# PJLab-ADG/neuralsim

Measured on AMD Instinct MI355X. Metric: training rays/sec (fwd+bwd) NeuS 800x800, higher is better.
Workload: dtype fp16

## Files before the change

### include/nsim.h

```cpp
#ifndef NSIM_H
#define NSIM_H
#include <stdint.h>

#ifdef __cplusplus
extern "C" {
#endif

#define NSIM_MAX_LEVELS 32
#define NSIM_LOTD_DENSE 0
#define NSIM_LOTD_HASH 1

typedef struct NsimLotdMeta {
  int32_t num_levels;
  int32_t n_feats;
  int32_t n_active_levels;
  int32_t res[NSIM_MAX_LEVELS][3];
  int32_t type[NSIM_MAX_LEVELS];
  uint32_t size[NSIM_MAX_LEVELS];
  int64_t offset[NSIM_MAX_LEVELS];
  float x_scale[3];
  float x_shift[3];
} NsimLotdMeta;

typedef struct NsimOccMeta {
  float aabb_min[3];
  float aabb_max[3];
  float scale[3];
  int32_t res[3];
} NsimOccMeta;

const char* nsim_strerror(int code);
int nsim_version(void);

int nsim_pack_infos_from_n(const int64_t* n, int64_t P, int64_t* pack_infos, int64_t* total, int64_t cap,
                           void* stream);
int nsim_pack_infos_from_n_notify(const int64_t* n, int64_t P, int64_t* pack_infos, int64_t* total, int64_t cap,
                                  int64_t* notify, int64_t seq, void* stream);
int nsim_live_rank(const int64_t* n, int64_t R, int C, int nf0, int nf1, int nf2, int nf3, int64_t* live_rank,
                   int64_t* live_idx, int64_t* cnts, int64_t* notify, int64_t seq, int64_t* pack_infos, int64_t* total,
                   int64_t cap, int64_t* notify_total, int64_t seq_total, void* stream);
int nsim_packed_sum(const float* x, int C, const int64_t* pack_infos, int64_t P, float* out, void* stream);
int nsim_packed_binary(const float* x, int C, const float* per_pack, int Cp, const int64_t* pack_infos,
                       int64_t P, int op, float* out, void* stream);
int nsim_packed_cmp(const float* x, const float* per_pack, const int64_t* pack_infos, int64_t P, int op,
                    uint8_t* out, void* stream);
int nsim_packed_matmul3(const float* x, const float* rot, const int64_t* pack_infos, int64_t P,
                        int transpose, float* out, void* stream);
int nsim_packed_sort(const float* x, const int64_t* pack_infos, int64_t P, float* sorted,
                     int64_t* indices, void* stream);
typedef struct NsimComposeSrc {
  const float* t;
  const int64_t* rays_inds;
  const int64_t* pack_infos;
  int64_t P;
  int64_t* dst;
} NsimComposeSrc;
int nsim_compose_collect_sort(const NsimComposeSrc* src, int32_t K, const int64_t* total_pack_infos, int64_t N,
                              float* t_sorted, void* stream);
int nsim_interleave_linstep(const int64_t* start, const int64_t* pack_infos, int64_t P, int64_t step,
                            int64_t* out, void* stream);
int nsim_merge_two_packs(const float* va, const int64_t* pia, const int64_t* slot_a, int64_t Pa,
                         const float* vb, const int64_t* pib, const int64_t* slot_b, int64_t Pb,
                         const int64_t* pack_infos_out, int64_t U, int64_t* pidx_a, int64_t* pidx_b,
                         void* stream);

int nsim_alpha_to_vw_fwd(const float* alpha, const int64_t* pack_infos, int64_t P, float* vw, float* trans,
                         void* stream);
int nsim_alpha_to_vw_bwd(const float* alpha, const float* trans, const float* vw, const float* dvw,
                         const int64_t* pack_infos, int64_t P, float* dalpha, void* stream);
int nsim_render_head(const float* sdf, const float* ln_inv_s, float ln_inv_s_factor, float forward_inv_s, const float* t,
                     const float* rgb, const float* nablas, const int64_t* pack_infos, int64_t P, int normalized_depth,
                     const float* gt, int64_t N, int64_t S, int64_t M, float w_eikonal, const int64_t* out_idx, float* alpha,
                     float* vw, float* trans, float* mask, float* depth, float* rgb_out, float* nrm_out, float* acc,
                     float* dalpha, float* dsdf, float* drgb, float* dnablas, float* d_ln_inv_s, void* stream);
int nsim_composite_fwd(const float* alpha, const float* t, const float* rgb, const float* nrm,
                       const int64_t* pack_infos, int64_t P, int normalized_depth, float* vw, float* trans,
                       float* mask, float* depth, float* rgb_out, float* nrm_out, const int64_t* out_idx,
                       void* stream);
int nsim_composite_bwd(const float* alpha, const float* trans, const float* vw, const float* t,
                       const float* rgb, const float* nrm, const int64_t* pack_infos, int64_t P,
                       int normalized_depth, const float* mask, const float* depth, const float* dmask,
                       const float* ddepth, const float* drgb_out, const float* dnrm_out,
                       const float* dvw_ext, float* dalpha, float* drgb, float* dnrm, const int64_t* out_idx,
                       void* stream);
int nsim_neus_alpha_fwd(const float* sdf, const int64_t* pack_infos, int64_t P, const float* ln_inv_s,
                        float ln_inv_s_factor, float forward_inv_s, float* alpha, void* stream);
int nsim_neus_alpha_bwd(const float* sdf, const float* dalpha, const int64_t* pack_infos, int64_t P,
                        const float* ln_inv_s, float ln_inv_s_factor, float forward_inv_s, float* dsdf,
                        float* d_ln_inv_s, void* stream);
int nsim_neus_composite_fwd(const float* sdf, const float* ln_inv_s, float ln_inv_s_factor, float forward_inv_s,
                            const float* t, const float* rgb, const float* nrm, const int64_t* pack_infos, int64_t P,
                            int normalized_depth, float* alpha, float* vw, float* trans, float* mask, float* depth,
                            float* rgb_out, float* nrm_out, const int64_t* out_idx, void* stream);

int nsim_raygen_pinhole(const float* xy, const int64_t* fidx, const float* intr ,
                        const float* c2w , const int64_t* WH , int64_t N, int snap,
                        float* rays_o, float* rays_d, void* stream);
int nsim_raygen_pinhole_bwd(const float* xy, const int64_t* fidx, const float* intr, const float* c2w,
                            const int64_t* WH, int64_t N, int snap, const float* d_rays_o, const float* d_rays_d,
                            float* d_c2w, void* stream);
int nsim_raygen_opencv(const float* xy, const int64_t* fidx, const float* intr, const float* distortion ,
                       int n_iters, const float* c2w, const int64_t* WH, int64_t N, int snap, float* rays_o,
                       float* rays_d, void* stream);
int nsim_raygen_opencv_bwd(const float* xy, const int64_t* fidx, const float* intr, const float* distortion, int n_iters,
                           const float* c2w, const int64_t* WH, int64_t N, int snap, const float* d_rays_o,
                           const float* d_rays_d, float* d_c2w, void* stream);
int nsim_raygen_fisheye(const float* xy, const int64_t* fidx, const float* intr, const float* distortion ,
                        int n_iters, const float* c2w, const int64_t* WH, int64_t N, int snap, float* rays_o,
                        float* rays_d, void* stream);
int nsim_raygen_fisheye_bwd(const float* xy, const int64_t* fidx, const float* intr, const float* distortion, int n_iters,
                            const float* c2w, const int64_t* WH, int64_t N, int snap, const float* d_rays_o,
                            const float* d_rays_d, float* d_c2w, void* stream);
int nsim_aabb_ray_test(const float* rays_o, const float* rays_d, int64_t N, const NsimOccMeta* meta,
                       float near, float far, float* near_out, float* far_out, uint8_t* hit, void* stream);

int nsim_occ_decay(float* val, int64_t nvox, float decay, void* stream);
int nsim_occ_update(float* val, const float* pts, const float* sdf, int64_t n, const NsimOccMeta* meta,
                    float inv_s, void* stream);
int nsim_occ_pack_bits(const float* val, int64_t nvox, float thre, uint32_t* bits, void* stream);
int nsim_occ_collect(float* val, const float* pts, const float* sdf, int64_t n, const int64_t* n_dev, int64_t n_add,
                     const NsimOccMeta* meta, float inv_s, void* stream);
int nsim_march_count(const float* rays_o, const float* rays_d, const float* near, const float* far,
                     const float* jitter, int64_t R, const uint32_t* bits, const int64_t* ray_word_off,
                     const NsimOccMeta* meta, float step, int max_steps, int64_t* counts, void* stream);
int nsim_march_emit(const float* rays_o, const float* rays_d, const float* near, const float* far,
                    const float* jitter, int64_t R, const uint32_t* bits, const int64_t* ray_word_off,
                    const NsimOccMeta* meta, float step, int max_steps, const int64_t* pack_infos, float* t_out,
                    void* stream);
int nsim_coarse_depths(const float* near, const float* far, const float* jitter_c, int64_t R, int C,
                       float* out, const int64_t* live_rank, void* stream);
int nsim_upsample_stage(const float* t, const float* sdf, const int64_t* pack_infos, int64_t R, float inv_s,
                        int n_fine, int use_estimate_alpha, float* scratch, float* t_new, const float* rays_o,
                        const float* rays_d, float* x_new, const int64_t* live_rank, void* stream);
int nsim_merge_sorted(const float* t_a, const float* v_a, const int64_t* pack_infos_a, const float* t_b,
                      const float* v_b, int64_t R, int nb, float* t_out, float* v_out,
                      int64_t* pack_infos_out, int64_t* ridx_out, const float* rays_o, const float* rays_d,
                      float* x_out, const int64_t* live_rank, void* stream);
int nsim_merge_upsample(const float* t_a, const float* v_a, const int64_t* pack_infos_a, const float* t_b, const float* v_b,
                        int64_t R, int nb, float* t_out, float* v_out, int64_t* pack_infos_out, int64_t* ridx_out, float inv_s,
                        int n_fine, int use_estimate_alpha, float* scratch, float* t_new, const float* rays_o,
                        const float* rays_d, float* x_new, const int64_t* live_rank, void* stream);

int nsim_compress_count(const float* sdf, const int64_t* pack_infos, int64_t R, const float* ln_inv_s,
                        float ln_inv_s_factor, float forward_inv_s, float thre, int64_t* counts, void* stream);
int nsim_compress_emit(const float* sdf, const float* t, const int64_t* pack_infos, int64_t R, const float* ln_inv_s,
                       float ln_inv_s_factor, float forward_inv_s, float thre, const int64_t* pack_infos_out,
                       float* t_out, int64_t* ridx_out, int64_t tail_n, void* stream);

int nsim_lotd_fwd(const float* x, const void* grid_f16, const NsimLotdMeta* meta, int64_t S, float* out,
                  float* dydx, void* stream);
int nsim_lotd_bwd(const float* x, const float* dL_dout, const float* dL_ddydx, const NsimLotdMeta* meta,
                  int64_t S, float* dgrid, void* stream);

typedef struct NsimPermutoMeta {
  int32_t in_dim;
  int32_t num_levels;
  int32_t n_feats;
  uint32_t hashmap_size;
  float scale[NSIM_MAX_LEVELS][8];
  float shift[NSIM_MAX_LEVELS][8];
} NsimPermutoMeta;
int nsim_permuto_fwd(const NsimPermutoMeta* meta, const void* grid_f16, const float* x, int64_t S, float* out, float* dydx,
                     void* stream);
int nsim_permuto_bwd(const NsimPermutoMeta* meta, const float* x, int64_t S, const float* dL_dout, float* dgrid,
                     void* stream);
int nsim_permuto_gather(const NsimPermutoMeta* meta, const void* grid_f16, const float* x, const float* rays_o,
                        const float* rays_d, const float* t, const int64_t* ridx, const float* z, int64_t S,
                        const int64_t* n_dev, int64_t n_add, void* feat_planes, int feat_f32, float* h_planes,
                        void* J_planes, void* stream);
int nsim_permuto_scatter(const NsimPermutoMeta* meta, const float* x, const float* rays_o, const float* rays_d,
                         const float* t, const int64_t* ridx, const float* z, int64_t S, const float* dh_planes,
                         const float* g_planes, const float* gn, float* dgrid, void* stream);
int nsim_permuto_dz(const NsimPermutoMeta* meta, const void* grid_f16, const float* x, const float* rays_o,
                    const float* rays_d, const float* t, const int64_t* ridx, const float* z, int64_t S,
                    const float* dh_planes, float* dz, void* stream);

typedef struct NsimFieldMeta {
  NsimLotdMeta lotd;
  int32_t sdf_D;
  int32_t precision;
  float softplus_beta;
  int32_t embed_E;
} NsimFieldMeta;

int64_t nsim_field_wpack_bytes(const NsimFieldMeta* meta);
int nsim_field_pack_weights(const NsimFieldMeta* meta, const float* sdf_w, const float* sdf_b,
                            const float* rad_w, const float* rad_b, void* wpack, void* stream);
int nsim_field_pack_weights2(const NsimFieldMeta* meta_a, void* wpack_a, const NsimFieldMeta* meta_b, void* wpack_b,
                             const float* sdf_w, const float* sdf_b, const float* rad_w, const float* rad_b, void* stream);
int nsim_field_sdf(const NsimFieldMeta* meta, const void* grid_f16, const void* wpack, const float* x,
                   const float* rays_o, const float* rays_d, const float* t, const int64_t* ridx,
                   const int64_t* ray_goff, int64_t S, const int64_t* n_dev, int64_t n_add, float* sdf,
                   const void* feat_planes, float* occ_val, const NsimOccMeta* occ_meta, float occ_inv_s, void* stream);
int nsim_lotd_gather_lm(const NsimFieldMeta* meta, const void* grid_f16, const float* x, const float* rays_o,
                        const float* rays_d, const float* t, const int64_t* ridx, const int64_t* ray_goff, int64_t S,
                        const int64_t* n_dev, int64_t n_add, void* feat_planes, void* stream);
#define NSIM_PLANE_PITCH(S) ((((int64_t)(S)) + 31) & ~(int64_t)31)
int nsim_field_fwd(const NsimFieldMeta* meta, const void* grid_f16, const void* wpack, const float* x,
                   const float* rays_o, const float* rays_d, const float* t, const int64_t* ridx,
                   const int64_t* ray_goff, const float* h_appear, int64_t S, float* sdf, float* nablas, float* rgb,
                   float* h_planes, void* J_planes, const int64_t* n_dev, int64_t n_add, void* stream);
int nsim_jplane_elem_bytes(const NsimFieldMeta* meta);
int nsim_set_grad_scratch(float* buf, int64_t floats, void* stream);
int nsim_field_bwd_rad(const NsimFieldMeta* meta, const void* wpack, const float* nablas_fwd, const float* rgb_fwd,
                       const float* x, const float* rays_o, const float* rays_d, const float* t, const int64_t* ridx,
                       const float* h_appear, int64_t S, const float* dnablas, const float* drgb, float* gn_out,
                       float* drad_w, float* drad_b, float* dh_appear, float* dx, float* dv, void* stream);
int nsim_field_bwd_sdf(const NsimFieldMeta* meta, const void* wpack, const float* h_planes, const void* J_planes,
                       int64_t S, const float* dsdf, const float* gn, float* dh_planes, float* g_planes,
                       float* dsdf_w, float* dsdf_b, float* dx, int64_t plane_pitch, void* stream);
int nsim_wide_sdf(const NsimFieldMeta* meta, int32_t n_freq, const float* sdf_w, const float* sdf_b, const float* x,
                  const float* rays_o, const float* rays_d, const float* t, const int64_t* ridx, int64_t S,
                  const int64_t* n_dev, int64_t n_add, const float* feat_planes, float* sdf, void* stream);
int nsim_wide_bwd_sdf(const NsimFieldMeta* meta, const void* wpack, const float* x, const float* rays_o,
                      const float* rays_d, const float* t, const int64_t* ridx, int64_t S, const float* h_planes,
                      const void* J_planes, int64_t plane_pitch, const float* dsdf, const float* gn, float* dh_planes,
                      float* g_planes, float* dsdf_w, float* dsdf_b, void* stream);
int nsim_lotd_scatter(const NsimLotdMeta* meta, const float* x, const float* rays_o, const float* rays_d,
                      const float* t, const int64_t* ridx, const int64_t* ray_goff, int64_t S,
                      const float* dh_planes, const float* g_planes, const float* gn, float* dgrid, int level_begin,
                      int level_count, void* stream);
int nsim_lotd_hess_dx(const NsimLotdMeta* meta, const void* grid_f16, const float* x, const float* rays_o,
                      const float* rays_d, const float* t, const int64_t* ridx, const int64_t* ray_goff, int64_t S,
                      const float* g_planes, const float* gn, float* dx, void* stream);
int nsim_ray_grad_reduce(const float* dx, const float* dv, const float* t, const int64_t* ridx, int64_t S,
                         float* d_rays_o, float* d_rays_d, void* stream);

typedef struct NsimLotd4Meta {
  int32_t num_levels;
  int32_t res_xyz[16];
  int32_t res_w[16];
  int32_t type[16];
  uint32_t size[16];
  int64_t offset[16];
  int32_t res_y[16];
  int32_t res_z[16];
} NsimLotd4Meta;

typedef struct NsimDistantMeta {
  NsimLotd4Meta lotd;
  int32_t precision;
} NsimDistantMeta;

int64_t nsim_distant_wpack_bytes(const NsimDistantMeta* meta);
int nsim_distant_pack_weights(const NsimDistantMeta* meta, const float* den_w, const float* den_b, const float* rad_w,
                              const float* rad_b, void* wpack, void* stream);
int nsim_distant_shells(const float* rays_o, const float* rays_d, const float* near, const float* jitter, int64_t N,
                        int K, const float* aabb, float r_min, float r_max, float* t, float* u4, uint8_t* valid,
                        void* stream);
int nsim_density_alpha_fwd(const float* sigma, const float* t, const uint8_t* valid, int64_t N, int K,
                           int include_inf_distance, float* alpha, void* stream);
int nsim_density_alpha_bwd(const float* sigma, const float* t, const uint8_t* valid, const float* dalpha, int64_t N,
                           int K, int include_inf_distance, float* dsigma, void* stream);
int nsim_distant_fwd(const NsimDistantMeta* meta, const void* grid_f16, const void* wpack, const float* u4,
                     const float* rays_d, const float* h_appear, int64_t S, int K, float* sigma, float* rgb,
                     float* h_planes, void* stream);
int nsim_distant_bwd(const NsimDistantMeta* meta, const void* wpack, const float* h_planes, const float* sigma_fwd,
                     const float* rgb_fwd, const float* rays_d, const float* h_appear, const uint8_t* valid,
                     int64_t S, int K, const float* dsigma, const float* drgb, float* dh_planes, float* dden_w,
                     float* dden_b, float* drad_w, float* drad_b, float* dh_appear, void* stream);
int nsim_lotd4_scatter(const NsimLotd4Meta* meta, const float* u4, const uint8_t* valid, int64_t S,
                       const float* dh_planes, float* dgrid, void* stream);

typedef struct NsimSkyMeta {
  int32_t n_frequencies;
  int32_t n_appear;
  int32_t precision;
} NsimSkyMeta;

int64_t nsim_sky_wpack_bytes(const NsimSkyMeta* meta);
int64_t nsim_sky_plane_pitch(int64_t N);
int nsim_sky_pack_weights(const NsimSkyMeta* meta, const float* w, const float* b, void* wpack, void* stream);
int nsim_sky_fwd(const NsimSkyMeta* meta, const void* wpack, const float* v, const float* h_appear, int64_t N,
                 float* rgb, float* planes_fwd, void* stream);
int nsim_sky_bwd(const NsimSkyMeta* meta, const void* wpack, const float* rgb_fwd, const float* drgb, int64_t N,
                 const float* planes_fwd, float* planes_bwd, float* dw, float* db, float* dh_appear, void* stream);

int nsim_eikonal_loss_fwd(const float* nablas, int64_t S, float* out, void* stream);
int nsim_eikonal_loss_bwd(const float* nablas, int64_t S, const float* gout, float* dnablas, void* stream);
int nsim_mse_loss_fwd(const float* pred, const float* gt, int64_t n, float* out, void* stream);
int nsim_mse_loss_bwd(const float* pred, const float* gt, int64_t n, const float* gout, float* dpred, void* stream);
int nsim_rows_scatter_add(const float* g, const int64_t* idx, int64_t n, int C, int64_t rows, float* out, void* stream);
int nsim_rows_gather(const float* table, const int64_t* idx, int64_t n, int C, int64_t rows, int64_t tail, float* out,
                     void* stream);
int nsim_train_loss_head(const float* pred, const float* gt, int64_t n_img, const float* nablas, int64_t S, int64_t M,
                         float w_eikonal, float* acc, float* d_pred, float* d_nablas, void* stream);
int nsim_gather_rays(const float* rays_o, const float* rays_d, const float* near, const float* far, const int64_t* idx,
                     int64_t R, float* o_out, float* d_out, float* near_out, float* far_out, void* stream);
int nsim_sphere_image(const float* rays_o, const float* rays_d, int64_t N, float radius, float* rgb, void* stream);

int nsim_adam_step(float* p, void* p16, float* grad, float* m, float* v, int64_t n, float lr, float beta1,
                   float beta2, float eps, float bias1, float bias2, float grad_scale, int zero_grad,
                   void* stream);

#define NSIM_ADAM_MULTI_MAX 12
typedef struct {
  float* p;
  void* p16;
  float* grad;
  float* m;
  float* v;
  int64_t n;
  float beta1, beta2, bias1, bias2, lr_scale;
} NsimAdamTensor;
int nsim_adam_multi(const NsimAdamTensor* tensors, int n_tensors, float lr, float eps, float grad_scale, int zero_grad,
                    void* stream);

int nsim_mc_count(const float* lat, int64_t nx, int64_t ny, int64_t nzs, float level, int32_t* cnt_v, int32_t* cnt_t,
                  void* stream);
int nsim_mc_scan(int32_t* cnt_v, int32_t* cnt_t, int64_t nx, int64_t ny, int64_t nzs, int32_t* totals, void* stream);
int nsim_mc_emit_verts(const float* lat, const float* below, const float* above, int64_t nx, int64_t ny, int64_t nzs,
                       float level, float bx, float by, float bz, float h, int64_t k0, int64_t vbase, int emit_top,
                       const int32_t* off_v, int32_t* vid, float* verts, float* normals, void* stream);
int nsim_mc_emit_tris(const float* lat, int64_t nx, int64_t ny, int64_t nzs, float level, const int32_t* off_t,
                      const int32_t* vid, int32_t* faces, void* stream);

int nsim_nn_brute(const float* x, int64_t N, const float* y, int64_t M, const int32_t* qlist, const int32_t* nq, int64_t nsplit,
                  float* part_d2, int32_t* part_idx, float* d2, int32_t* idx, void* stream);
int nsim_nn_grid_count(const float* y, int64_t M, float target_occ, int64_t max_cells, int32_t* hdr, int32_t* cell_cnt,
                       int32_t* cell_of, int32_t* rank, void* stream);
int nsim_nn_grid_scan(const int32_t* hdr, int32_t* cell_cnt, void* stream);
int nsim_nn_grid_fill(const float* y, int64_t M, const int32_t* cell_off, const int32_t* cell_of, const int32_t* rank, float* rec,
                      void* stream);
int nsim_nn_grid_query(const float* x, int64_t N, const float* rec, const int32_t* cell_off, int32_t* hdr, int max_rings, float* d2,
                       int32_t* idx, int32_t* left_list, void* stream);

int nsim_selftest_mfma(const float* a, const float* b, float* d, int use_f32, void* stream);

#ifdef __cplusplus
}
#endif
#endif
```

### neuralsim_amd/_lib.py

```python
import ctypes as C
import os
from pathlib import Path

import torch

NSIM_MAX_LEVELS = 32
_HERE = Path(__file__).resolve().parent
LIB_PATH = _HERE / "csrc" / "libnsim_hip.so"


class LotdMeta(C.Structure):
    _fields_ = [("num_levels", C.c_int32), ("n_feats", C.c_int32), ("n_active_levels", C.c_int32),
                ("res", (C.c_int32 * 3) * NSIM_MAX_LEVELS),
                ("type", C.c_int32 * NSIM_MAX_LEVELS), ("size", C.c_uint32 * NSIM_MAX_LEVELS),
                ("offset", C.c_int64 * NSIM_MAX_LEVELS), ("x_scale", C.c_float * 3), ("x_shift", C.c_float * 3)]


class OccMeta(C.Structure):
    _fields_ = [("aabb_min", C.c_float * 3), ("aabb_max", C.c_float * 3), ("scale", C.c_float * 3),
                ("res", C.c_int32 * 3)]


class Lotd4Meta(C.Structure):
    _fields_ = [("num_levels", C.c_int32), ("res_xyz", C.c_int32 * 16), ("res_w", C.c_int32 * 16),
                ("type", C.c_int32 * 16), ("size", C.c_uint32 * 16), ("offset", C.c_int64 * 16),
                ("res_y", C.c_int32 * 16), ("res_z", C.c_int32 * 16)]


class PermutoMeta(C.Structure):
    _fields_ = [("in_dim", C.c_int32), ("num_levels", C.c_int32), ("n_feats", C.c_int32), ("hashmap_size", C.c_uint32),
                ("scale", (C.c_float * 8) * NSIM_MAX_LEVELS), ("shift", (C.c_float * 8) * NSIM_MAX_LEVELS)]


class DistantMeta(C.Structure):
    _fields_ = [("lotd", Lotd4Meta), ("precision", C.c_int32)]


class SkyMeta(C.Structure):
    _fields_ = [("n_frequencies", C.c_int32), ("n_appear", C.c_int32), ("precision", C.c_int32)]


class AdamTensor(C.Structure):
    _fields_ = [("p", C.c_void_p), ("p16", C.c_void_p), ("grad", C.c_void_p), ("m", C.c_void_p), ("v", C.c_void_p),
                ("n", C.c_int64), ("beta1", C.c_float), ("beta2", C.c_float), ("bias1", C.c_float), ("bias2", C.c_float),
                ("lr_scale", C.c_float)]


ADAM_MULTI_MAX = 12


def plane_pitch(S: int) -> int:
    return (int(S) + 31) & ~31


def jplane_dtype(fm):
    import torch
    return torch.float16 if int(get_lib().nsim_jplane_elem_bytes(fm)) == 2 else torch.float32


class FieldMeta(C.Structure):
    _fields_ = [("lotd", LotdMeta), ("sdf_D", C.c_int32), ("precision", C.c_int32), ("softplus_beta", C.c_float),
                ("embed_E", C.c_int32)]


class ComposeSrc(C.Structure):
    _fields_ = [("t", C.c_void_p), ("rays_inds", C.c_void_p), ("pack_infos", C.c_void_p), ("P", C.c_int64), ("dst", C.c_void_p)]


_P = C.c_void_p
_I64 = C.c_int64
_I = C.c_int
_F = C.c_float

SIGNATURES = {
    "nsim_pack_infos_from_n": [_P, _I64, _P, _P, _I64],
    "nsim_pack_infos_from_n_notify": [_P, _I64, _P, _P, _I64, _P, _I64],
    "nsim_live_rank": [_P, _I64, _I, _I, _I, _I, _I, _P, _P, _P, _P, _I64, _P, _P, _I64, _P, _I64],
    "nsim_packed_sum": [_P, _I, _P, _I64, _P],
    "nsim_packed_binary": [_P, _I, _P, _I, _P, _I64, _I, _P],
    "nsim_packed_cmp": [_P, _P, _P, _I64, _I, _P],
    "nsim_packed_matmul3": [_P, _P, _P, _I64, _I, _P],
    "nsim_packed_sort": [_P, _P, _I64, _P, _P],
    "nsim_interleave_linstep": [_P, _P, _I64, _I64, _P],
    "nsim_merge_two_packs": [_P, _P, _P, _I64, _P, _P, _P, _I64, _P, _I64, _P, _P],
    "nsim_alpha_to_vw_fwd": [_P, _P, _I64, _P, _P],
    "nsim_alpha_to_vw_bwd": [_P, _P, _P, _P, _P, _I64, _P],
    "nsim_composite_fwd": [_P, _P, _P, _P, _P, _I64, _I, _P, _P, _P, _P, _P, _P, _P],
    "nsim_neus_composite_fwd": [_P, _P, _F, _F, _P, _P, _P, _P, _I64, _I, _P, _P, _P, _P, _P, _P, _P, _P],
    "nsim_render_head": [_P, _P, _F, _F, _P, _P, _P, _P, _I64, _I, _P, _I64, _I64, _I64, _F, _P] + [_P] * 13,
    "nsim_composite_bwd": [_P, _P, _P, _P, _P, _P, _P, _I64, _I, _P, _P, _P, _P, _P, _P, _P, _P, _P, _P, _P],
    "nsim_neus_alpha_fwd": [_P, _P, _I64, _P, _F, _F, _P],
    "nsim_neus_alpha_bwd": [_P, _P, _P, _I64, _P, _F, _F, _P, _P],
    "nsim_raygen_pinhole": [_P, _P, _P, _P, _P, _I64, _I, _P, _P],
    "nsim_raygen_pinhole_bwd": [_P, _P, _P, _P, _P, _I64, _I, _P, _P, _P],
    "nsim_raygen_opencv": [_P, _P, _P, _P, _I, _P, _P, _I64, _I, _P, _P],
    "nsim_raygen_opencv_bwd": [_P, _P, _P, _P, _I, _P, _P, _I64, _I, _P, _P, _P],
    "nsim_raygen_fisheye": [_P, _P, _P, _P, _I, _P, _P, _I64, _I, _P, _P],
    "nsim_raygen_fisheye_bwd": [_P, _P, _P, _P, _I, _P, _P, _I64, _I, _P, _P, _P],
    "nsim_aabb_ray_test": [_P, _P, _I64, C.POINTER(OccMeta), _F, _F, _P, _P, _P],
    "nsim_occ_decay": [_P, _I64, _F],
    "nsim_occ_update": [_P, _P, _P, _I64, C.POINTER(OccMeta), _F],
    "nsim_occ_pack_bits": [_P, _I64, _F, _P],
    "nsim_occ_collect": [_P, _P, _P, _I64, _P, _I64, C.POINTER(OccMeta), _F],
    "nsim_march_count": [_P, _P, _P, _P, _P, _I64, _P, _P, C.POINTER(OccMeta), _F, _I, _P],
    "nsim_march_emit": [_P, _P, _P, _P, _P, _I64, _P, _P, C.POINTER(OccMeta), _F, _I, _P, _P],
    "nsim_coarse_depths": [_P, _P, _P, _I64, _I, _P, _P],
    "nsim_upsample_stage": [_P, _P, _P, _I64, _F, _I, _I, _P, _P, _P, _P, _P, _P],
    "nsim_merge_sorted": [_P, _P, _P, _P, _P, _I64, _I, _P, _P, _P, _P, _P, _P, _P, _P],
    "nsim_merge_upsample": [_P, _P, _P, _P, _P, _I64, _I, _P, _P, _P, _P, _F, _I, _I, _P, _P, _P, _P, _P, _P],
    "nsim_compress_count": [_P, _P, _I64, _P, _F, _F, _F, _P],
    "nsim_compress_emit": [_P, _P, _P, _I64, _P, _F, _F, _F, _P, _P, _P, _I64],
    "nsim_lotd_fwd": [_P, _P, C.POINTER(LotdMeta), _I64, _P, _P],
    "nsim_lotd_bwd": [_P, _P, _P, C.POINTER(LotdMeta), _I64, _P],
    "nsim_field_pack_weights": [C.POINTER(FieldMeta), _P, _P, _P, _P, _P],
    "nsim_field_sdf": [C.POINTER(FieldMeta), _P, _P, _P, _P, _P, _P, _P, _P, _I64, _P, _I64, _P, _P, _P, C.POINTER(OccMeta), _F],
    "nsim_lotd_gather_lm": [C.POINTER(FieldMeta), _P, _P, _P, _P, _P, _P, _P, _I64, _P, _I64, _P],
    "nsim_field_fwd": [C.POINTER(FieldMeta), _P, _P, _P, _P, _P, _P, _P, _P, _P, _I64, _P, _P, _P, _P, _P, _P, _I64],
    "nsim_compose_collect_sort": [_P, _I, _P, _I64, _P],
    "nsim_wide_sdf": [C.POINTER(FieldMeta), _I, _P, _P, _P, _P, _P, _P, _P, _I64, _P, _I64, _P, _P],
    "nsim_wide_bwd_sdf": [C.POINTER(FieldMeta), _P, _P, _P, _P, _P, _P, _I64, _P, _P, _I64, _P, _P, _P, _P, _P, _P],
    "nsim_set_grad_scratch": [_P, _I64],
    "nsim_permuto_fwd": [C.POINTER(PermutoMeta), _P, _P, _I64, _P, _P],
    "nsim_permuto_bwd": [C.POINTER(PermutoMeta), _P, _I64, _P, _P],
    "nsim_permuto_gather": [C.POINTER(PermutoMeta), _P, _P, _P, _P, _P, _P, _P, _I64, _P, _I64, _P, _I, _P, _P],
    "nsim_permuto_scatter": [C.POINTER(PermutoMeta), _P, _P, _P, _P, _P, _P, _I64, _P, _P, _P, _P],
    "nsim_permuto_dz": [C.POINTER(PermutoMeta), _P, _P, _P, _P, _P, _P, _P, _I64, _P, _P],
    "nsim_field_bwd_rad": [C.POINTER(FieldMeta), _P, _P, _P, _P, _P, _P, _P, _P, _P, _I64, _P, _P, _P, _P, _P, _P, _P, _P],
    "nsim_field_bwd_sdf": [C.POINTER(FieldMeta), _P, _P, _P, _I64, _P, _P, _P, _P, _P, _P, _P, _I64],
    "nsim_lotd_hess_dx": [C.POINTER(LotdMeta), _P, _P, _P, _P, _P, _P, _P, _I64, _P, _P, _P],
    "nsim_ray_grad_reduce": [_P, _P, _P, _P, _I64, _P, _P],
    "nsim_lotd_scatter": [C.POINTER(LotdMeta), _P, _P, _P, _P, _P, _P, _I64, _P, _P, _P, _P, _I, _I],
    "nsim_distant_pack_weights": [C.POINTER(DistantMeta), _P, _P, _P, _P, _P],
    "nsim_distant_shells": [_P, _P, _P, _P, _I64, _I, C.POINTER(C.c_float * 6), _F, _F, _P, _P, _P],
    "nsim_density_alpha_fwd": [_P, _P, _P, _I64, _I, _I, _P],
    "nsim_density_alpha_bwd": [_P, _P, _P, _P, _I64, _I, _I, _P],
    "nsim_distant_fwd": [C.POINTER(DistantMeta), _P, _P, _P, _P, _P, _I64, _I, _P, _P, _P],
    "nsim_distant_bwd": [C.POINTER(DistantMeta), _P, _P, _P, _P, _P, _P, _P, _I64, _I, _P, _P, _P, _P, _P, _P, _P, _P],
    "nsim_lotd4_scatter": [C.POINTER(Lotd4Meta), _P, _P, _I64, _P, _P],
    "nsim_sky_pack_weights": [C.POINTER(SkyMeta), _P, _P, _P],
    "nsim_sky_fwd": [C.POINTER(SkyMeta), _P, _P, _P, _I64, _P, _P],
    "nsim_sky_bwd": [C.POINTER(SkyMeta), _P, _P, _P, _I64, _P, _P, _P, _P, _P],
    "nsim_eikonal_loss_fwd": [_P, _I64, _P],
    "nsim_eikonal_loss_bwd": [_P, _I64, _P, _P],
    "nsim_mse_loss_fwd": [_P, _P, _I64, _P],
    "nsim_train_loss_head": [_P, _P, _I64, _P, _I64, _I64, _F, _P, _P, _P],
    "nsim_mse_loss_bwd": [_P, _P, _I64, _P, _P],
    "nsim_rows_scatter_add": [_P, _P, _I64, _I, _I64, _P],
    "nsim_rows_gather": [_P, _P, _I64, _I, _I64, _I64, _P],
    "nsim_field_pack_weights2": [C.POINTER(FieldMeta), _P, C.POINTER(FieldMeta), _P, _P, _P, _P, _P],
    "nsim_gather_rays": [_P, _P, _P, _P, _P, _I64, _P, _P, _P, _P],
    "nsim_sphere_image": [_P, _P, _I64, _F, _P],
    "nsim_adam_step": [_P, _P, _P, _P, _P, _I64, _F, _F, _F, _F, _F, _F, _F, _I],
    "nsim_adam_multi": [C.POINTER(AdamTensor), _I, _F, _F, _F, _I],
    "nsim_selftest_mfma": [_P, _P, _P, _I],
    "nsim_mc_count": [_P, _I64, _I64, _I64, _F, _P, _P],
    "nsim_mc_scan": [_P, _P, _I64, _I64, _I64, _P],
    "nsim_mc_emit_verts": [_P, _P, _P, _I64, _I64, _I64, _F, _F, _F, _F, _F, _I64, _I64, _I, _P, _P, _P, _P],
    "nsim_mc_emit_tris": [_P, _I64, _I64, _I64, _F, _P, _P, _P],
    "nsim_nn_brute": [_P, _I64, _P, _I64, _P, _P, _I64, _P, _P, _P, _P],
    "nsim_nn_grid_count": [_P, _I64, _F, _I64, _P, _P, _P, _P],
    "nsim_nn_grid_scan": [_P, _P],
    "nsim_nn_grid_fill": [_P, _I64, _P, _P, _P, _P],
    "nsim_nn_grid_query": [_P, _I64, _P, _P, _P, _I, _P, _P, _P],
}
NOSTREAM = {
    "nsim_strerror": ([_I], C.c_char_p),
    "nsim_version": ([], _I),
    "nsim_field_wpack_bytes": ([C.POINTER(FieldMeta)], _I64),
    "nsim_jplane_elem_bytes": ([C.POINTER(FieldMeta)], _I),
    "nsim_distant_wpack_bytes": ([C.POINTER(DistantMeta)], _I64),
    "nsim_sky_wpack_bytes": ([C.POINTER(SkyMeta)], _I64),
    "nsim_sky_plane_pitch": ([_I64], _I64),
}


def bind(cdll):
    for name, args in SIGNATURES.items():
        fn = getattr(cdll, name)
        fn.argtypes = list(args) + [_P]
        fn.restype = _I
    for name, (args, res) in NOSTREAM.items():
        fn = getattr(cdll, name)
        fn.argtypes = list(args)
        fn.restype = res
    return cdll


_LIB = None


def get_lib():
    global _LIB
    if _LIB is None:
        if not LIB_PATH.exists():
            raise RuntimeError(
                f"neuralsim_amd: {LIB_PATH} is missing. This package has no CPU fallback -- build the HIP "
                f"extension with `python -m neuralsim_amd.csrc.build` (needs hipcc, --offload-arch=gfx950).")
        _LIB = bind(C.CDLL(str(LIB_PATH)))
    return _LIB


def stream_handle() -> int:
    return torch._C._cuda_getCurrentRawStream(torch._C._cuda_getDevice())


def require_device(t: torch.Tensor, name: str = "tensor"):
    if not t.is_cuda:
        raise RuntimeError(f"neuralsim_amd: {name} must live on a HIP device (got {t.device}); there is no CPU path")


def ptr(t, dtype=None, name="tensor"):
    if t is not None and dtype is not None and t.dtype != dtype:
        raise TypeError(f"neuralsim_amd: {name} must be {dtype}, got {t.dtype}")
    return t


class HostNotify:

    def __init__(self, slots: int = 2):
        buf = torch.zeros([slots, 2], dtype=torch.long)
        self.buf = buf.pin_memory() if torch.cuda.is_available() else buf
        self.view = self.buf.numpy()
        self.seq = 0

    def __deepcopy__(self, memo):
        return HostNotify(self.buf.shape[0])

    def __reduce__(self):
        return (HostNotify, (self.buf.shape[0],))

    def arm(self, slot: int):
        self.seq += 1
        return self.buf.data_ptr() + 16 * slot, self.seq

    def wait(self, slot: int, seq: int, timeout_s: float = 10.0):
        v = self.view
        n = 0
        t0 = None
        while int(v[slot, 1]) != seq:
            n += 1
            if n & 1023 == 0:
                import time
                now = time.perf_counter()
                t0 = now if t0 is None else t0
                if now - t0 > timeout_s:
                    return None
        return int(v[slot, 0])


class KernelTimer:

    def __init__(self, only=None):
        self.events = {}
        self.units = {}
        self.only = set(only) if only is not None else None

    def note_units(self, name, n):
        self.units[name] = self.units.get(name, 0) + int(n)

    def summary(self):
        torch.cuda.synchronize()
        out = {}
        for name, evs in self.events.items():
            ms = [a.elapsed_time(b) for a, b in evs]
            out[name] = dict(calls=len(ms), total_ms=sum(ms), avg_ms=sum(ms) / max(1, len(ms)),
                             units=self.units.get(name, 0))
        return out


TIMER = None


_Tensor = torch.Tensor


def _marshal(args):
    out = []
    ap = out.append
    for a in args:
        if isinstance(a, _Tensor):
            if not a.is_cuda:
                require_device(a)
            if not a.is_contiguous():
                raise ValueError("neuralsim_amd: tensor arguments must be contiguous")
            ap(a.data_ptr())
        else:
            ap(a)
    return out


_GRAD_SCRATCH = {}
_GRAD_SCRATCH_USERS = ("nsim_field_bwd_rad", "nsim_field_bwd_sdf")
GRAD_SCRATCH_FLOATS = 16 * 8448


def ensure_grad_scratch(device):
    key = (str(device), stream_handle())
    if key not in _GRAD_SCRATCH:
        buf = torch.zeros([GRAD_SCRATCH_FLOATS], dtype=torch.float32, device=device)
        _GRAD_SCRATCH[key] = buf
        call("nsim_set_grad_scratch", buf, buf.numel())
    return _GRAD_SCRATCH[key]


CALL_COUNT = None
class _Arena:
    __slots__ = ("buf", "off", "cap", "demand", "device", "stream")


_ARENA = None
_ARENA_DEMAND = {}


def arena_begin(device):
    global _ARENA
    if os.environ.get("NSIM_ZERO_ARENA", "0") != "1":
        _ARENA = None
        return
    a = _Arena()
    a.device, a.off, a.demand = device, 0, 0
    want = _ARENA_DEMAND.get(str(device), 0)
    a.cap = (int(want * 1.125) + 1024) if want else 0
    a.buf = torch.zeros([a.cap], dtype=torch.float32, device=device) if a.cap else None
    a.stream = stream_handle() if device.type == "cuda" else 0
    _ARENA = a


def arena_end():
    global _ARENA
    a = _ARENA
    if a is not None:
        _ARENA_DEMAND[str(a.device)] = a.demand
    _ARENA = None


def zeros(shape, dtype=torch.float32, device=None):
    a = _ARENA
    if a is None or dtype != torch.float32 or device != a.device:
        return torch.zeros(shape, dtype=dtype, device=device)
    n = 1
    for d_ in shape:
        n *= int(d_)
    pad = (n + 3) & ~3
    a.demand += pad
    if a.off + pad > a.cap or (a.device.type == "cuda" and stream_handle() != a.stream):
        return torch.zeros(shape, dtype=dtype, device=device)
    v = a.buf[a.off:a.off + n].view(shape)
    a.off += pad
    return v


HOST_WAIT = None


def call(name: str, *args):
    global CALL_COUNT
    if CALL_COUNT is not None:
        CALL_COUNT += 1
    lib = get_lib()
    if name in _GRAD_SCRATCH_USERS:
        for a_ in args:
            if isinstance(a_, _Tensor):
                ensure_grad_scratch(a_.device)
                break
    cargs = _marshal(args)
    if TIMER is not None and (TIMER.only is None or name in TIMER.only):
        e0, e1 = torch.cuda.Event(enable_timing=True), torch.cuda.Event(enable_timing=True)
        e0.record()
        rc = getattr(lib, name)(*cargs, stream_handle())
        e1.record()
        TIMER.events.setdefault(name, []).append((e0, e1))
    else:
        rc = getattr(lib, name)(*cargs, stream_handle())
    if rc != 0:
        msg = lib.nsim_strerror(rc)
        raise RuntimeError(f"{name} failed with code {rc}: {msg.decode() if msg else '?'}")
```

### neuralsim_amd/csrc/build.py

```python
import hashlib
import os
import subprocess
import sys
from pathlib import Path

HERE = Path(__file__).resolve().parent
SOURCES = ["pack_ops.hip", "sampling.hip", "lotd.hip", "field.hip", "wide_field.hip", "permuto.hip", "nerf_field.hip", "sky.hip", "loss_ops.hip", "optim.hip", "misc.hip"]
HEADERS = ["nsim_common.h", "nsim_prims.h", "lotd_dev.h", "mfma_mlp.h", "occ_dev.h", "../../include/nsim.h"]
LIB = HERE / "libnsim_hip.so"
BUILD = HERE / "_build"

HIPCC_FLAGS = ["--offload-arch=gfx950", "-O3", "-std=c++17", "-fPIC", "-ffp-contract=off", f"-I{HERE}",
               "-munsafe-fp-atomics", "-Wno-unused-result"] + os.environ.get("NSIM_EXTRA_HIPCC_FLAGS", "").split()


def _hipcc():
    for c in (os.environ.get("HIPCC"), "/opt/rocm/bin/hipcc", "hipcc"):
        if c and (os.path.isabs(c) and os.path.exists(c) or not os.path.isabs(c)):
            return c
    raise RuntimeError("hipcc not found")


def _digest():
    h = hashlib.sha256()
    for f in SOURCES + HEADERS:
        h.update((HERE / f).read_bytes())
    h.update(" ".join(HIPCC_FLAGS).encode())
    return h.hexdigest()


def build(force: bool = False, verbose: bool = True) -> Path:
    BUILD.mkdir(exist_ok=True)
    stamp = BUILD / "stamp"
    dig = _digest()
    if not force and LIB.exists() and stamp.exists() and stamp.read_text() == dig:
        return LIB
    hipcc = _hipcc()
    procs = []
    objs = []
    for src in SOURCES:
        obj = BUILD / (src + ".o")
        objs.append(str(obj))
        cmd = [hipcc, *HIPCC_FLAGS, "-c", str(HERE / src), "-o", str(obj)]
        if verbose:
            print("[nsim build]", " ".join(cmd), flush=True)
        procs.append((src, subprocess.Popen(cmd, stdout=subprocess.PIPE, stderr=subprocess.STDOUT, text=True)))
    failed = False
    for src, p in procs:
        out, _ = p.communicate()
        if p.returncode != 0:
            failed = True
            sys.stderr.write(f"[nsim build] FAILED {src}\n{out}\n")
        elif verbose and out.strip():
            print(out)
    if failed:
        raise RuntimeError("hipcc failed")
    cmd = [hipcc, "--offload-arch=gfx950", "-shared", "-fPIC", *objs, "-o", str(LIB)]
    if verbose:
        print("[nsim build]", " ".join(cmd), flush=True)
    subprocess.check_call(cmd)
    stamp.write_text(dig)
    return LIB


if __name__ == "__main__":
    build(force="--force" in sys.argv)
    print(LIB)
```

### neuralsim_amd/csrc/pack_ops.hip

```cpp
#include "nsim_common.h"

#define PACK_WAVES_PER_BLOCK 4
#define PACK_BLOCK (64 * PACK_WAVES_PER_BLOCK)

__device__ __forceinline__ int64_t pack_wave_id() {
  return (int64_t)blockIdx.x * PACK_WAVES_PER_BLOCK + (threadIdx.x >> 6);
}
static inline dim3 pack_grid(int64_t P) { return dim3(nsim_blocks(P, PACK_WAVES_PER_BLOCK)); }

#define PI_THREADS 1024
#define PI_PER 8
__global__ void __launch_bounds__(PI_THREADS) k_pack_infos_from_n(const int64_t* __restrict__ n, int64_t P,
                                                                    int64_t* __restrict__ pi,
                                                                    int64_t* __restrict__ total, int64_t cap,
                                                                    int64_t* notify, int64_t seq) {
  __shared__ int64_t wtot[PI_THREADS / 64];
  const int tid = threadIdx.x, lane = nsim_lane(), wave = tid >> 6;
  int64_t carry = 0;
  for (int64_t base = 0; base < P; base += (int64_t)PI_THREADS * PI_PER) {
    const int64_t i0 = base + (int64_t)tid * PI_PER;
    int64_t v[PI_PER];
    int64_t mine = 0;
#pragma unroll
    for (int k = 0; k < PI_PER; ++k) {
      v[k] = (i0 + k) < P ? n[i0 + k] : 0;
      mine += v[k];
    }
    const int64_t incl = wave_incl_sum(mine);
    if (lane == 63) wtot[wave] = incl;
    __syncthreads();
    int64_t before = 0, chunk = 0;
#pragma unroll
    for (int w = 0; w < PI_THREADS / 64; ++w) {
      const int64_t x = wtot[w];
      before += (w < wave) ? x : 0;
      chunk += x;
    }
    int64_t run = carry + before + incl - mine;
#pragma unroll
    for (int k = 0; k < PI_PER; ++k) {
      const int64_t i = i0 + k;
      if (i < P) {
        const bool over = cap >= 0 && run + v[k] > cap;
        pi[2 * i] = (cap >= 0 && run > cap) ? cap : run;
        pi[2 * i + 1] = over ? 0 : v[k];
      }
      run += v[k];
    }
    carry += chunk;
    __syncthreads();
  }
  if (tid == 0 && total) total[0] = carry;
  if (tid == 0 && notify) {
    nsim_store_system(notify, carry, false);
    nsim_store_system(notify + 1, seq, true);
  }
}

struct LiveArgs {
  int C;
  int nf[4];
};
__global__ void __launch_bounds__(PI_THREADS) k_live_rank(const int64_t* __restrict__ n, int64_t R, LiveArgs la,
                                                           int64_t* __restrict__ live_rank, int64_t* __restrict__ live_idx,
                                                           int64_t* __restrict__ cnts, int64_t* notify, int64_t seq,
                                                           int64_t* __restrict__ pi, int64_t* __restrict__ total, int64_t cap,
                                                           int64_t* notify_total, int64_t seq_total) {
  __shared__ int64_t wtot[PI_THREADS / 64];
  __shared__ int wlive[PI_THREADS / 64];
  const int tid = threadIdx.x, lane = nsim_lane(), wave = tid >> 6;
  int64_t carry = 0, carry_live = 0;
  for (int64_t base = 0; base < R; base += (int64_t)PI_THREADS * PI_PER) {
    const int64_t i0 = base + (int64_t)tid * PI_PER;
    int64_t v[PI_PER];
    int64_t mine = 0;
    int mine_live = 0;
#pragma unroll
    for (int k = 0; k < PI_PER; ++k) {
      v[k] = (i0 + k) < R ? n[i0 + k] : 0;
      mine += v[k];
      mine_live += v[k] > 0 ? 1 : 0;
    }
    const int64_t incl = wave_incl_sum(mine);
    const int incl_live = wave_incl_sum(mine_live);
    if (lane == 63) {
      wtot[wave] = incl;
      wlive[wave] = incl_live;
    }
    __syncthreads();
    int64_t before = 0, chunk = 0;
    int before_live = 0, chunk_live = 0;
#pragma unroll
    for (int w = 0; w < PI_THREADS / 64; ++w) {
      const int64_t x = wtot[w];
      const int y = wlive[w];
      before += (w < wave) ? x : 0;
      chunk += x;
      before_live += (w < wave) ? y : 0;
      chunk_live += y;
    }
    int64_t run = carry + before + incl - mine;
    int64_t q = carry_live + before_live + incl_live - mine_live;
#pragma unroll
    for (int k = 0; k < PI_PER; ++k) {
      const int64_t i = i0 + k;
      if (i < R) {
        const bool live = v[k] > 0;
        live_rank[i] = live ? q : ~q;
        if (live && live_idx) live_idx[q] = i;
        if (pi) {
          const bool over = cap >= 0 && run + v[k] > cap;
          pi[2 * i] = (cap >= 0 && run > cap) ? cap : run;
          pi[2 * i + 1] = over ? 0 : v[k];
        }
        q += live ? 1 : 0;
      }
      run += v[k];
    }
    carry += chunk;
    carry_live += chunk_live;
    __syncthreads();
  }
  const int64_t Rl = carry_live, M = carry;
  if (live_idx)
    for (int64_t i = Rl + tid; i < R; i += PI_THREADS) live_idx[i] = 0;
  if (tid == 0) {
    cnts[0] = Rl;
    cnts[1] = M + Rl * la.C;
#pragma unroll
    for (int k = 0; k < 4; ++k) cnts[2 + k] = Rl * la.nf[k];
    cnts[6] = M;
    cnts[7] = 0;
    if (total) total[0] = M;
    if (notify) {
      nsim_store_system(notify, Rl, false);
      nsim_store_system(notify + 1, seq, true);
    }
    if (notify_total) {
      nsim_store_system(notify_total, M, false);
      nsim_store_system(notify_total + 1, seq_total, true);
    }
  }
}

__global__ void __launch_bounds__(PACK_BLOCK) k_packed_sum(const float* __restrict__ x, int C,
                                                             const int64_t* __restrict__ pi, int64_t P,
                                                             float* __restrict__ out) {
  const int64_t p = pack_wave_id();
  if (p >= P) return;
  const int lane = nsim_lane();
  const int64_t st = pi[2 * p], n = pi[2 * p + 1];
  for (int c = 0; c < C; ++c) {
    float acc = 0.f;
    for (int64_t i = lane; i < n; i += 64) acc += x[(st + i) * C + c];
    acc = wave_sum(acc);
    if (lane == 0) out[p * C + c] = acc;
  }
}

__global__ void __launch_bounds__(PACK_BLOCK) k_packed_binary(const float* __restrict__ x, int C,
                                                                const float* __restrict__ pp, int Cp,
                                                                const int64_t* __restrict__ pi, int64_t P,
                                                                int op, float* __restrict__ out) {
  const int64_t p = pack_wave_id();
  if (p >= P) return;
  const int lane = nsim_lane();
  const int64_t st = pi[2 * p], n = pi[2 * p + 1];
  const int64_t tot = n * C;
  for (int64_t j = lane; j < tot; j += 64) {
    const int c = (int)(j % C);
    const float b = pp[p * Cp + (Cp == 1 ? 0 : c)];
    const float a = x ? x[st * C + j] : 1.0f;
    float r;
    if (op == 0) r = a * b;
    else if (op == 1) r = a / b;
    else if (op == 2) r = a + b;
    else r = a - b;
    out[st * C + j] = r;
  }
}

__global__ void __launch_bounds__(PACK_BLOCK) k_packed_cmp(const float* __restrict__ x,
                                                             const float* __restrict__ pp,
                                                             const int64_t* __restrict__ pi, int64_t P, int op,
                                                             uint8_t* __restrict__ out) {
  const int64_t p = pack_wave_id();
  if (p >= P) return;
  const int lane = nsim_lane();
  const int64_t st = pi[2 * p], n = pi[2 * p + 1];
  const float b = pp[p];
  for (int64_t i = lane; i < n; i += 64) {
    const float a = x[st + i];
    bool r = (op == 0) ? (a >= b) : (op == 1) ? (a <= b) : (op == 2) ? (a < b) : (a > b);
    out[st + i] = r ? 1 : 0;
  }
}

__global__ void __launch_bounds__(PACK_BLOCK) k_packed_matmul3(const float* __restrict__ x,
                                                                 const float* __restrict__ rot,
                                                                 const int64_t* __restrict__ pi, int64_t P,
                                                                 int transpose, float* __restrict__ out) {
  const int64_t p = pack_wave_id();
  if (p >= P) return;
  const int lane = nsim_lane();
  const int64_t st = pi[2 * p], n = pi[2 * p + 1];
  float r[9];
  for (int k = 0; k < 9; ++k) r[k] = rot[p * 9 + k];
  for (int64_t i = lane; i < n; i += 64) {
    const float a = x[(st + i) * 3 + 0], b = x[(st + i) * 3 + 1], c = x[(st + i) * 3 + 2];
    float o0, o1, o2;
    if (!transpose) {
      o0 = r[0] * a + r[1] * b + r[2] * c;
      o1 = r[3] * a + r[4] * b + r[5] * c;
      o2 = r[6] * a + r[7] * b + r[8] * c;
    } else {
      o0 = r[0] * a + r[3] * b + r[6] * c;
      o1 = r[1] * a + r[4] * b + r[7] * c;
      o2 = r[2] * a + r[5] * b + r[8] * c;
    }
    out[(st + i) * 3 + 0] = o0;
    out[(st + i) * 3 + 1] = o1;
    out[(st + i) * 3 + 2] = o2;
  }
}

__global__ void __launch_bounds__(PACK_BLOCK) k_interleave_linstep(const int64_t* __restrict__ start,
                                                                     const int64_t* __restrict__ pi,
                                                                     int64_t P, int64_t step,
                                                                     int64_t* __restrict__ out) {
  const int64_t p = pack_wave_id();
  if (p >= P) return;
  const int lane = nsim_lane();
  const int64_t st = pi[2 * p], n = pi[2 * p + 1], s0 = start[p];
  for (int64_t i = lane; i < n; i += 64) out[st + i] = s0 + i * step;
}

#define PSORT_CAP 1024
#define PSORT_RUNS 16
__device__ __forceinline__ int lds_upper_bound(const float* a, int n, float v) {
  int lo = 0, hi = n;
  while (lo < hi) {
    const int mid = (lo + hi) >> 1;
    if (a[mid] <= v) lo = mid + 1; else hi = mid;
  }
  return lo;
}
__device__ __forceinline__ int lds_lower_bound(const float* a, int n, float v) {
  int lo = 0, hi = n;
  while (lo < hi) {
    const int mid = (lo + hi) >> 1;
    if (a[mid] < v) lo = mid + 1; else hi = mid;
  }
  return lo;
}
template <class Emit>
__device__ __forceinline__ void psort_staged(const float* sx, int* srun, int nn, int lane, Emit emit) {
  int nrun = 0;
  for (int i0 = 0; i0 < nn; i0 += 64) {
    const int i = i0 + lane;
    const bool head = i < nn && (i == 0 || sx[i] < sx[i - 1]);
    const unsigned long long m = wave_ballot(head);
    if (head) {
      const int pos = nrun + __popcll(m & ((1ull << lane) - 1ull));
      if (pos < PSORT_RUNS) srun[pos] = i;
    }
    nrun += __popcll(m);
  }
  if (nrun <= 1) {
    for (int i = lane; i < nn; i += 64) emit(i, i, sx[i]);
    return;
  }
  if (nrun <= PSORT_RUNS) {
    if (lane == 0) srun[nrun] = nn;
    wave_sync_lds();
    for (int i = lane; i < nn; i += 64) {
      const float xi = sx[i];
      int rank = 0;
      for (int r = 0; r < nrun; ++r) {
        const int b = srun[r], e = srun[r + 1];
        if (e <= i) rank += lds_upper_bound(&sx[b], e - b, xi);
        else if (b > i) rank += lds_lower_bound(&sx[b], e - b, xi);
        else rank += i - b;
      }
      emit(i, rank, xi);
    }
    return;
  }
  for (int i0 = 0; i0 < nn; i0 += 256) {
    float xi[4];
    int ii[4], rank[4];
#pragma unroll
    for (int k = 0; k < 4; ++k) {
      ii[k] = i0 + lane + 64 * k;
      xi[k] = ii[k] < nn ? sx[ii[k]] : 0.f;
      rank[k] = 0;
    }
    for (int j = 0; j < nn; ++j) {
      const float xj = sx[j];
#pragma unroll
      for (int k = 0; k < 4; ++k) rank[k] += (xj < xi[k] || (xj == xi[k] && j < ii[k])) ? 1 : 0;
    }
#pragma unroll
    for (int k = 0; k < 4; ++k)
      if (ii[k] < nn) emit(ii[k], rank[k], xi[k]);
  }
}

__global__ void __launch_bounds__(PACK_BLOCK) k_packed_sort(const float* __restrict__ x,
                                                              const int64_t* __restrict__ pi, int64_t P,
                                                              float* __restrict__ sorted,
                                                              int64_t* __restrict__ indices) {
  __shared__ float sx[PACK_WAVES_PER_BLOCK][PSORT_CAP];
  __shared__ int srun[PACK_WAVES_PER_BLOCK][PSORT_RUNS + 1];
  const int64_t p = pack_wave_id();
  if (p >= P) return;
  const int lane = nsim_lane();
  const int w = (int)(threadIdx.x >> 6);
  const int64_t st = pi[2 * p], n = pi[2 * p + 1];
  if (n <= PSORT_CAP) {
    for (int64_t i = lane; i < n; i += 64) sx[w][i] = x[st + i];
    wave_sync_lds();
    psort_staged(sx[w], srun[w], (int)n, lane, [&](int i, int rank, float xi) {
      sorted[st + rank] = xi;
      indices[st + rank] = st + i;
    });
    return;
  }
  for (int64_t i = lane; i < n; i += 64) {
    const float xi = x[st + i];
    int64_t rank = 0;
    for (int64_t j = 0; j < n; ++j) {
      const float xj = x[st + j];
      rank += (xj < xi || (xj == xi && j < i)) ? 1 : 0;
    }
    sorted[st + rank] = xi;
    indices[st + rank] = st + i;
  }
}

#define COMPOSE_MAX_SRC 64
struct ComposeSrcDev {
  const float* t;
  const int64_t *ric, *pi;
  int64_t P;
  int64_t* dst;
};
struct ComposeArgs {
  int K;
  ComposeSrcDev src[COMPOSE_MAX_SRC];
  const int64_t* total_pi;
  int64_t N;
  float* t_sorted;
};

__global__ void __launch_bounds__(PACK_BLOCK) k_compose_collect_sort(ComposeArgs a) {
  __shared__ float sx[PACK_WAVES_PER_BLOCK][PSORT_CAP];
  __shared__ int srun[PACK_WAVES_PER_BLOCK][PSORT_RUNS + 1];
  __shared__ int s_off[PACK_WAVES_PER_BLOCK][COMPOSE_MAX_SRC + 1];
  __shared__ int64_t s_stg[PACK_WAVES_PER_BLOCK][COMPOSE_MAX_SRC];
  const int64_t r = pack_wave_id();
  if (r >= a.N) return;
  const int lane = nsim_lane();
  const int w = (int)(threadIdx.x >> 6);
  const int64_t st = a.total_pi[2 * r], n = a.total_pi[2 * r + 1];
  if (n <= 0) return;
  int64_t my_st = 0;
  int my_n = 0;
  if (lane < a.K) {
    const ComposeSrcDev& sk = a.src[lane];
    int64_t lo = 0, hi = sk.P;
    while (lo < hi) {
      const int64_t mid = (lo + hi) >> 1;
      if (sk.ric[mid] < r) lo = mid + 1; else hi = mid;
    }
    if (lo < sk.P && sk.ric[lo] == r) {
      my_st = sk.pi[2 * lo];
      my_n = (int)sk.pi[2 * lo + 1];
    }
  }
  const int incl = wave_incl_sum(my_n);
  s_off[w][lane] = incl - my_n;
  if (lane == 63) s_off[w][64] = incl;
  s_stg[w][lane] = my_st;
  wave_sync_lds();
  const int K = a.K;
  auto source_of = [&](int j) -> int {
    int lo = 0, hi = K - 1;
    while (lo < hi) {
      const int mid = (lo + hi + 1) >> 1;
      if (s_off[w][mid] <= j) lo = mid; else hi = mid - 1;
    }
    return lo;
  };
  if (n <= PSORT_CAP) {
    for (int k = 0; k < K; ++k) {
      const int ok = s_off[w][k], nk = s_off[w][k + 1] - ok;
      const float* tk = a.src[k].t + s_stg[w][k];
      for (int i = lane; i < nk; i += 64) sx[w][ok + i] = tk[i];
    }
    wave_sync_lds();
    psort_staged(sx[w], srun[w], (int)n, lane, [&](int i, int rank, float xi) {
      a.t_sorted[st + rank] = xi;
      const int k = source_of(i);
      a.src[k].dst[s_stg[w][k] + (i - s_off[w][k])] = st + rank;
    });
    return;
  }
  for (int64_t i = lane; i < n; i += 64) {
    const int ki = source_of((int)i);
    const float xi = a.src[ki].t[s_stg[w][ki] + (i - s_off[w][ki])];
    int64_t rank = 0;
    for (int k = 0; k < K; ++k) {
      const int ok = s_off[w][k], nk = s_off[w][k + 1] - ok;
      const float* tk = a.src[k].t + s_stg[w][k];
      for (int jj = 0; jj < nk; ++jj) {
        const float xj = tk[jj];
        const int64_t j = ok + jj;
        rank += (xj < xi || (xj == xi && j < i)) ? 1 : 0;
      }
    }
    a.t_sorted[st + rank] = xi;
    a.src[ki].dst[s_stg[w][ki] + (i - s_off[w][ki])] = st + rank;
  }
}

__device__ __forceinline__ int64_t seg_lower_bound(const float* a, int64_t n, float v) {
  int64_t lo = 0, hi = n;
  while (lo < hi) {
    const int64_t mid = (lo + hi) >> 1;
    if (a[mid] < v) lo = mid + 1; else hi = mid;
  }
  return lo;
}
__device__ __forceinline__ int64_t seg_upper_bound(const float* a, int64_t n, float v) {
  int64_t lo = 0, hi = n;
  while (lo < hi) {
    const int64_t mid = (lo + hi) >> 1;
    if (a[mid] <= v) lo = mid + 1; else hi = mid;
  }
  return lo;
}

__global__ void __launch_bounds__(PACK_BLOCK) k_merge_two_packs(
    const float* __restrict__ vs, const int64_t* __restrict__ pis, const int64_t* __restrict__ slot_s,
    int64_t Ps, const float* __restrict__ vo, const int64_t* __restrict__ pio,
// ... 711 lines not shown
```

### neuralsim_amd/csrc/sampling.hip

```cpp
#include "nsim_common.h"
#include "occ_dev.h"

#define SMP_WAVES_PER_BLOCK 4
#define SMP_BLOCK (64 * SMP_WAVES_PER_BLOCK)
#define SMP_LDS_FLOATS 512

__device__ __forceinline__ int64_t smp_wave_id() {
  return (int64_t)blockIdx.x * SMP_WAVES_PER_BLOCK + (threadIdx.x >> 6);
}
static inline dim3 smp_grid(int64_t R) { return dim3(nsim_blocks(R, SMP_WAVES_PER_BLOCK)); }

__device__ __forceinline__ bool smp_live(const int64_t* __restrict__ live_rank, int64_t r, int64_t& q) {
  if (!live_rank) {
    q = r;
    return true;
  }
  const int64_t e = live_rank[r];
  q = e >= 0 ? e : ~e;
  return e >= 0;
}

__device__ __forceinline__ void raygen_lift_fisheye(const float* K, const float* dist, int n_iters, float w, float h, float l[3]) {
  const float xd = (w - K[2]) / K[0], yd = (h - K[5]) / K[4];
  const float td = sqrtf(xd * xd + yd * yd);
  const float k1 = dist[0], k2 = dist[1], k3 = dist[2], k4 = dist[3];
  float th = td;
  for (int it = 0; it < n_iters; ++it) {
    const float t2 = th * th;
    const float f = th * (1.0f + (((k4 * t2 + k3) * t2 + k2) * t2 + k1) * t2) - td;
    const float fp = 1.0f + (((9.0f * k4 * t2 + 7.0f * k3) * t2 + 5.0f * k2) * t2 + 3.0f * k1) * t2;
    th = th - f / fp;
  }
  const float sc = td > 1e-8f ? sinf(th) / td : 1.0f;
  l[0] = xd * sc;
  l[1] = yd * sc;
  l[2] = cosf(th);
}

__device__ __forceinline__ void raygen_lift(const float* K, const float* dist, int n_iters, float w, float h, float l[3]) {
  if (n_iters < 0) {
    raygen_lift_fisheye(K, dist, -n_iters, w, h, l);
    return;
  }
  const float x0 = (w - K[2]) / K[0], y0 = (h - K[5]) / K[4];
  float x = x0, y = y0;
  if (dist) {
    const float k1 = dist[0], k2 = dist[1], p1 = dist[2], p2 = dist[3], k3 = dist[4];
    for (int it = 0; it < n_iters; ++it) {
      const float r2 = x * x + y * y;
      const float icd = 1.0f / (1.0f + ((k3 * r2 + k2) * r2 + k1) * r2);
      const float dx = 2.0f * p1 * x * y + p2 * (r2 + 2.0f * x * x);
      const float dy = p1 * (r2 + 2.0f * y * y) + 2.0f * p2 * x * y;
      x = (x0 - dx) * icd;
      y = (y0 - dy) * icd;
    }
  }
  l[0] = x;
  l[1] = y;
  l[2] = 1.0f;
}

__global__ void __launch_bounds__(256) k_raygen_pinhole(const float* __restrict__ xy,
                                                         const int64_t* __restrict__ fidx,
                                                         const float* __restrict__ intr,
                                                         const float* __restrict__ c2w,
                                                         const int64_t* __restrict__ WH, int64_t N, int snap,
                                                         float* __restrict__ rays_o, float* __restrict__ rays_d,
                                                         const float* __restrict__ dist, int n_iters) {
  const int64_t i = (int64_t)blockIdx.x * blockDim.x + threadIdx.x;
  if (i >= N) return;
  const int64_t f = fidx[i];
  const float W = (float)WH[2 * f], H = (float)WH[2 * f + 1];
  float w = xy[2 * i] * W, h = xy[2 * i + 1] * H;
  if (snap) {
    float wi = truncf(w), hi = truncf(h);
    wi = fminf(fmaxf(wi, 0.f), W - 1.f);
    hi = fminf(fmaxf(hi, 0.f), H - 1.f);
    w = wi + 0.5f;
    h = hi + 0.5f;
  }
  float l[3];
  raygen_lift(intr + f * 9, dist ? dist + f * (n_iters < 0 ? 4 : 5) : nullptr, n_iters, w, h, l);
  const float dx = l[0], dy = l[1], dz = l[2];
  const float* M = c2w + f * 16;
  float d0 = M[0] * dx + M[1] * dy + M[2] * dz;
  float d1 = M[4] * dx + M[5] * dy + M[6] * dz;
  float d2 = M[8] * dx + M[9] * dy + M[10] * dz;
  const float nrm = fmaxf(sqrtf(d0 * d0 + d1 * d1 + d2 * d2), 1e-12f);
  rays_d[3 * i + 0] = d0 / nrm;
  rays_d[3 * i + 1] = d1 / nrm;
  rays_d[3 * i + 2] = d2 / nrm;
  rays_o[3 * i + 0] = M[3];
  rays_o[3 * i + 1] = M[7];
  rays_o[3 * i + 2] = M[11];
}

__global__ void __launch_bounds__(256) k_raygen_pinhole_bwd(const float* __restrict__ xy,
                                                             const int64_t* __restrict__ fidx,
                                                             const float* __restrict__ intr,
                                                             const float* __restrict__ c2w,
                                                             const int64_t* __restrict__ WH, int64_t N, int snap,
                                                             const float* __restrict__ d_o,
                                                             const float* __restrict__ d_d,
                                                             float* __restrict__ d_c2w,
                                                             const float* __restrict__ dist, int n_iters) {
  const int64_t i = (int64_t)blockIdx.x * blockDim.x + threadIdx.x;
  if (i >= N) return;
  const int64_t f = fidx[i];
  const float W = (float)WH[2 * f], H = (float)WH[2 * f + 1];
  float w = xy[2 * i] * W, h = xy[2 * i + 1] * H;
  if (snap) {
    float wi = truncf(w), hi = truncf(h);
    wi = fminf(fmaxf(wi, 0.f), W - 1.f);
    hi = fminf(fmaxf(hi, 0.f), H - 1.f);
    w = wi + 0.5f;
    h = hi + 0.5f;
  }
  float l[3];
  raygen_lift(intr + f * 9, dist ? dist + f * (n_iters < 0 ? 4 : 5) : nullptr, n_iters, w, h, l);
  const float* M = c2w + f * 16;
  float dw[3];
#pragma unroll
  for (int r = 0; r < 3; ++r) dw[r] = M[4 * r] * l[0] + M[4 * r + 1] * l[1] + M[4 * r + 2] * l[2];
  const float nrm = fmaxf(sqrtf(dw[0] * dw[0] + dw[1] * dw[1] + dw[2] * dw[2]), 1e-12f);
  float* G = d_c2w + f * 16;
  if (d_d) {
    const float u[3] = {dw[0] / nrm, dw[1] / nrm, dw[2] / nrm};
    const float g[3] = {d_d[3 * i], d_d[3 * i + 1], d_d[3 * i + 2]};
    const float dot = g[0] * u[0] + g[1] * u[1] + g[2] * u[2];
#pragma unroll
    for (int r = 0; r < 3; ++r) {
      const float gr = (g[r] - dot * u[r]) / nrm;
#pragma unroll
      for (int c = 0; c < 3; ++c) atomicAdd(&G[4 * r + c], gr * l[c]);
    }
  }
  if (d_o) {
#pragma unroll
    for (int r = 0; r < 3; ++r) atomicAdd(&G[4 * r + 3], d_o[3 * i + r]);
  }
}

__global__ void __launch_bounds__(256) k_aabb_ray_test(const float* __restrict__ rays_o,
                                                        const float* __restrict__ rays_d, int64_t N, OccDev m,
                                                        float near, float far, float* __restrict__ near_out,
                                                        float* __restrict__ far_out, uint8_t* __restrict__ hit) {
  const int64_t i = (int64_t)blockIdx.x * blockDim.x + threadIdx.x;
  if (i >= N) return;
  float tmin = -INFINITY, tmax = INFINITY;
#pragma unroll
  for (int a = 0; a < 3; ++a) {
    const float o = rays_o[3 * i + a];
    float d = rays_d[3 * i + a];
    if (fabsf(d) < 1e-12f) d = (d < 0.f) ? -1e-12f : 1e-12f;
    const float inv = 1.0f / d;
    const float t1 = (m.mn[a] - o) * inv, t2 = (m.mx[a] - o) * inv;
    tmin = fmaxf(tmin, fminf(t1, t2));
    tmax = fminf(tmax, fmaxf(t1, t2));
  }
  const float n = fmaxf(tmin, near);
  const float f = (far >= 0.f) ? fminf(tmax, far) : tmax;
  near_out[i] = n;
  far_out[i] = f;
  hit[i] = (f > n) ? 1 : 0;
}

__global__ void __launch_bounds__(256) k_occ_decay(float* __restrict__ val, int64_t n, float decay) {
  const int64_t i = (int64_t)blockIdx.x * blockDim.x + threadIdx.x;
  if (i < n) val[i] = val[i] * decay;
}

__global__ void __launch_bounds__(256) k_occ_update(float* __restrict__ val, const float* __restrict__ pts,
                                                     const float* __restrict__ sdf, int64_t n, OccDev m,
                                                     float inv_s, const int64_t* __restrict__ n_dev, int64_t n_add) {
  const int64_t i = (int64_t)blockIdx.x * blockDim.x + threadIdx.x;
  if (n_dev) {
    const int64_t nd = n_dev[0] + n_add;
    n = nd <= n ? nd : 0;
  }
  const bool ok = i < n;
  occ_collect_wave(val, m, ok, ok ? pts[3 * i] : 0.f, ok ? pts[3 * i + 1] : 0.f, ok ? pts[3 * i + 2] : 0.f, ok ? sdf[i] : 0.f,
                   inv_s);
}

__global__ void __launch_bounds__(256) k_occ_pack_bits(const float* __restrict__ val, int64_t nvox, float thre,
                                                        uint32_t* __restrict__ bits) {
  const int64_t w = (int64_t)blockIdx.x * blockDim.x + threadIdx.x;
  const int64_t nwords = (nvox + 31) / 32;
  if (w >= nwords) return;
  uint32_t b = 0;
  for (int k = 0; k < 32; ++k) {
    const int64_t v = w * 32 + k;
    if (v < nvox && val[v] > thre) b |= (1u << k);
  }
  bits[w] = b;
}

struct MarchRay {
  float o[3], d[3], near, far, jit;
  int K;
};

__device__ __forceinline__ MarchRay march_load(const float* rays_o, const float* rays_d, const float* near,
                                               const float* far, const float* jitter, int64_t r, float step,
                                               int max_steps) {
  MarchRay m;
  for (int a = 0; a < 3; ++a) {
    m.o[a] = rays_o[3 * r + a];
    m.d[a] = rays_d[3 * r + a];
  }
  m.near = near[r];
  m.far = far[r];
  m.jit = jitter ? jitter[r] : 0.5f;
  float kf = ceilf((m.far - m.near) / step);
  kf = fminf(fmaxf(kf, 0.f), (float)max_steps);
  m.K = (int)kf;
  return m;
}

__device__ __forceinline__ bool march_test(const MarchRay& m, const OccDev& occ, const uint32_t* bits, int k,
                                           float step, float& t) {
  t = m.near + ((float)k + m.jit) * step;
  if (k >= m.K || !(t < m.far)) return false;
  const float px = m.o[0] + t * m.d[0], py = m.o[1] + t * m.d[1], pz = m.o[2] + t * m.d[2];
  int64_t flat;
  if (!occ_voxel(occ, px, py, pz, flat)) return false;
  return (bits[flat >> 5] >> (flat & 31)) & 1u;
}

__global__ void __launch_bounds__(SMP_BLOCK) k_march_count(
    const float* __restrict__ rays_o, const float* __restrict__ rays_d, const float* __restrict__ near,
    const float* __restrict__ far, const float* __restrict__ jitter, int64_t R, const uint32_t* __restrict__ bits,
    const int64_t* __restrict__ ray_word_off, OccDev occ, float step, int max_steps, int64_t* __restrict__ counts) {
  const int64_t r = smp_wave_id();
  if (r >= R) return;
  const int lane = nsim_lane();
  if (ray_word_off) bits += ray_word_off[r];
  const MarchRay m = march_load(rays_o, rays_d, near, far, jitter, r, step, max_steps);
  int cnt = 0;
  for (int base = 0; base < m.K; base += 64) {
    float t;
    const bool hit = march_test(m, occ, bits, base + lane, step, t);
    cnt += __popcll(wave_ballot(hit));
  }
  if (lane == 0) counts[r] = cnt;
}

__global__ void __launch_bounds__(SMP_BLOCK) k_march_emit(
    const float* __restrict__ rays_o, const float* __restrict__ rays_d, const float* __restrict__ near,
    const float* __restrict__ far, const float* __restrict__ jitter, int64_t R, const uint32_t* __restrict__ bits,
    const int64_t* __restrict__ ray_word_off, OccDev occ, float step, int max_steps, const int64_t* __restrict__ pi,
    float* __restrict__ t_out) {
  const int64_t r = smp_wave_id();
  if (r >= R) return;
  const int lane = nsim_lane();
  if (ray_word_off) bits += ray_word_off[r];
  if (pi[2 * r + 1] == 0) return;
  const MarchRay m = march_load(rays_o, rays_d, near, far, jitter, r, step, max_steps);
  const int64_t st = pi[2 * r];
  int cnt = 0;
  for (int base = 0; base < m.K; base += 64) {
    float t;
    const bool hit = march_test(m, occ, bits, base + lane, step, t);
    const unsigned long long mask = wave_ballot(hit);
    if (hit) {
      const int before = __popcll(mask & ((1ull << lane) - 1ull));
      t_out[st + cnt + before] = t;
    }
    cnt += __popcll(mask);
  }
}

__global__ void __launch_bounds__(256) k_coarse_depths(const float* __restrict__ near, const float* __restrict__ far,
                                                        const float* __restrict__ jc, int64_t R, int C,
                                                        float* __restrict__ out, const int64_t* __restrict__ live_rank) {
  const int64_t j = (int64_t)blockIdx.x * blockDim.x + threadIdx.x;
  if (j >= R * C) return;
  const int64_t r = j / C;
  const int i = (int)(j % C);
  int64_t q;
  if (!smp_live(live_rank, r, q)) return;
  const float u = jc ? jc[j] : 0.5f;
  out[q * C + i] = near[r] + (far[r] - near[r]) * (((float)i + u) / (float)C);
}

__device__ __forceinline__ float smp_sigmoid(float x) { return 1.0f / (1.0f + expf(-x)); }

__device__ __forceinline__ float upsample_alpha(const float* t, const float* sdf, int64_t i, float inv_s,
                                                int use_est) {
  const float s0 = sdf[i], s1 = sdf[i + 1];
  if (use_est) {
    const float t0 = t[i], t1 = t[i + 1];
    const float dist = t1 - t0;
    float cs = (s1 - s0) / (dist + 1e-5f);
    float prev = 0.f;
    if (i > 0) prev = (s0 - sdf[i - 1]) / ((t0 - t[i - 1]) + 1e-5f);
    cs = fminf(prev, cs);
    cs = fminf(fmaxf(cs, -1e3f), 0.f);
    const float mid = (s0 + s1) * 0.5f;
    const float half = cs * dist * 0.5f;
    const float pc = smp_sigmoid((mid - half) * inv_s), nc = smp_sigmoid((mid + half) * inv_s);
    return (pc - nc + 1e-5f) / (pc + 1e-5f);
  } else {
    const float c0 = smp_sigmoid(s0 * inv_s), c1 = smp_sigmoid(s1 * inv_s);
    const float a = (c0 - c1 + 1e-5f) / (c0 + 1e-5f);
    return fminf(fmaxf(a, 0.f), 1.f);
  }
}

__device__ __forceinline__ void upsample_ray(const float* tt, const float* ss, int64_t n, int64_t r, int64_t q, float inv_s, int n_fine,
                                             int use_est, float* lds, float* cs_glob, float* __restrict__ t_new,
                                             const float* __restrict__ rays_o, const float* __restrict__ rays_d,
                                             float* __restrict__ x_new) {
  const int lane = nsim_lane();
  const int64_t ni = n - 1;
  float ro[3] = {0.f, 0.f, 0.f}, rd[3] = {0.f, 0.f, 0.f};
  if (x_new) {
#pragma unroll
    for (int c = 0; c < 3; ++c) {
      ro[c] = rays_o[3 * r + c];
      rd[c] = rays_d[3 * r + c];
    }
  }
  auto body = [&](auto cs) {
    float carry_T = 1.0f, carry_S = 0.f;
    for (int64_t base = 0; base < ni; base += 64) {
      const int64_t i = base + lane;
      const bool valid = i < ni;
      const float a = valid ? upsample_alpha(tt, ss, i, inv_s, use_est) : 0.f;
      const float f = valid ? (1.0f - a + 1e-7f) : 1.0f;
      const float incl = wave_incl_prod(f);
      float excl = wave_shfl(incl, lane - 1);
      if (lane == 0) excl = 1.0f;
      const float T = carry_T * excl;
      carry_T = carry_T * wave_shfl(incl, 63);
      const float w = valid ? (a * T + 1e-5f) : 0.f;
      const float ws = wave_incl_sum(w);
      if (valid) cs[i] = carry_S + ws;
      carry_S = carry_S + wave_shfl(ws, 63);
    }
    nsim_wave_fence();
    const float wsum = carry_S;
    for (int kb = 0; kb < n_fine; kb += 64) {
      const int k = kb + lane;
      if (k >= n_fine) continue;
      float tn = (n > 0) ? tt[0] : 0.f;
      if (ni > 0) {
        const float u = ((float)k + 0.5f) / (float)n_fine;
        int64_t lo = 0, hi = ni;
        while (lo < hi) {
          const int64_t mid = (lo + hi) >> 1;
          if (cs[mid] / wsum <= u) lo = mid + 1; else hi = mid;
        }
        if (lo > ni - 1) lo = ni - 1;
        const float c_lo = (lo == 0) ? 0.f : cs[lo - 1] / wsum;
        const float c_hi = cs[lo] / wsum;
        float den = c_hi - c_lo;
        if (den < 1e-5f) den = 1.0f;
        float frac = (u - c_lo) / den;
        frac = fminf(fmaxf(frac, 0.f), 1.f);
        const float b_lo = tt[lo], b_hi = tt[lo + 1];
        tn = b_lo + frac * (b_hi - b_lo);
      }
      t_new[q * n_fine + k] = tn;
      if (x_new) {
#pragma unroll
        for (int c = 0; c < 3; ++c) x_new[(q * n_fine + k) * 3 + c] = ro[c] + tn * rd[c];
      }
    }
  };
  if (ni <= SMP_LDS_FLOATS) body(lds);
  else body(cs_glob);
}

__global__ void __launch_bounds__(SMP_BLOCK) k_upsample_stage(const float* __restrict__ t,
                                                                const float* __restrict__ sdf,
                                                                const int64_t* __restrict__ pi, int64_t R,
                                                                float inv_s, int n_fine, int use_est,
                                                                float* __restrict__ csum,
                                                                float* __restrict__ t_new,
                                                                const float* __restrict__ rays_o,
                                                                const float* __restrict__ rays_d,
                                                                float* __restrict__ x_new,
                                                                const int64_t* __restrict__ live_rank) {
  __shared__ float smp_lds[SMP_WAVES_PER_BLOCK][SMP_LDS_FLOATS];
  const int64_t r = smp_wave_id();
  if (r >= R) return;
  int64_t q;
  if (!smp_live(live_rank, r, q)) return;
  const int64_t st = pi[2 * r], n = pi[2 * r + 1];
  upsample_ray(t + st, sdf + st, n, r, q, inv_s, n_fine, use_est, &smp_lds[threadIdx.x >> 6][0], csum + st, t_new, rays_o, rays_d,
               x_new);
}

__device__ __forceinline__ int64_t smp_lower_bound(const float* a, int64_t n, float v) {
  int64_t lo = 0, hi = n;
  while (lo < hi) {
    const int64_t mid = (lo + hi) >> 1;
    if (a[mid] < v) lo = mid + 1; else hi = mid;
  }
  return lo;
}
__device__ __forceinline__ int64_t smp_upper_bound(const float* a, int64_t n, float v) {
  int64_t lo = 0, hi = n;
  while (lo < hi) {
    const int64_t mid = (lo + hi) >> 1;
    if (a[mid] <= v) lo = mid + 1; else hi = mid;
  }
  return lo;
}

__device__ __forceinline__ void merge_ray(const float* __restrict__ t_a, const float* __restrict__ v_a, int64_t sa, int64_t na,
                                          const float* __restrict__ t_b, const float* __restrict__ v_b, int64_t r, int64_t q, int nb,
                                          int64_t so, float* lds, float* __restrict__ t_out, float* __restrict__ v_out,
                                          int64_t* __restrict__ ridx_out, const float* __restrict__ rays_o,
                                          const float* __restrict__ rays_d, float* __restrict__ x_out) {
  const int lane = nsim_lane();
  float ro[3] = {0.f, 0.f, 0.f}, rd[3] = {0.f, 0.f, 0.f};
  if (x_out) {
#pragma unroll
    for (int c = 0; c < 3; ++c) {
      ro[c] = rays_o[3 * r + c];
      rd[c] = rays_d[3 * r + c];
    }
  }
  const bool in_lds = na + nb <= SMP_LDS_FLOATS;
  float* la = lds;
  float* lb = la + na;
  if (in_lds) {
    for (int64_t i = lane; i < na; i += 64) la[i] = t_a[sa + i];
    for (int64_t j = lane; j < nb; j += 64) lb[j] = t_b[q * (int64_t)nb + j];
    nsim_wave_fence();
  }
  auto body = [&](auto a, auto b) {
    for (int64_t i = lane; i < na; i += 64) {
      const float v = a[i];
      const int64_t pos = i + smp_lower_bound(b, nb, v);
      t_out[so + pos] = v;
      if (v_out) v_out[so + pos] = v_a ? v_a[sa + i] : 0.f;
      if (ridx_out) ridx_out[so + pos] = r;
      if (x_out) {
#pragma unroll
        for (int c = 0; c < 3; ++c) x_out[(so + pos) * 3 + c] = ro[c] + v * rd[c];
      }
    }
    for (int64_t j = lane; j < nb; j += 64) {
      const float v = b[j];
      const int64_t pos = j + smp_upper_bound(a, na, v);
      t_out[so + pos] = v;
      if (v_out) v_out[so + pos] = v_b ? v_b[q * (int64_t)nb + j] : 0.f;
      if (ridx_out) ridx_out[so + pos] = r;
      if (x_out) {
#pragma unroll
        for (int c = 0; c < 3; ++c) x_out[(so + pos) * 3 + c] = ro[c] + v * rd[c];
      }
    }
  };
  if (in_lds) body((const float*)la, (const float*)lb);
  else body(t_a + sa, t_b + q * (int64_t)nb);
}

__global__ void __launch_bounds__(SMP_BLOCK) k_merge_sorted(const float* __restrict__ t_a,
                                                              const float* __restrict__ v_a,
                                                              const int64_t* __restrict__ pia,
                                                              const float* __restrict__ t_b,
                                                              const float* __restrict__ v_b, int64_t R, int nb,
                                                              float* __restrict__ t_out, float* __restrict__ v_out,
                                                              int64_t* __restrict__ pio, int64_t* __restrict__ ridx_out,
                                                              const float* __restrict__ rays_o,
                                                              const float* __restrict__ rays_d,
                                                              float* __restrict__ x_out,
                                                              const int64_t* __restrict__ live_rank) {
  __shared__ float smp_lds[SMP_WAVES_PER_BLOCK][SMP_LDS_FLOATS];
  const int64_t r = smp_wave_id();
  if (r >= R) return;
  int64_t q;
  const bool live = smp_live(live_rank, r, q);
  const int64_t sa = pia[2 * r], na = live ? pia[2 * r + 1] : 0;
  const int64_t so = sa + q * (int64_t)nb;
  const int nb_r = live ? nb : 0;
  if (nsim_lane() == 0) {
    pio[2 * r] = so;
    pio[2 * r + 1] = na + nb_r;
  }
  if (!live) return;
  merge_ray(t_a, v_a, sa, na, t_b, v_b, r, q, nb, so, &smp_lds[threadIdx.x >> 6][0], t_out, v_out, ridx_out, rays_o, rays_d, x_out);
}

__global__ void __launch_bounds__(SMP_BLOCK) k_merge_upsample(const float* __restrict__ t_a, const float* __restrict__ v_a,
                                                                const int64_t* __restrict__ pia, const float* __restrict__ t_b,
                                                                const float* __restrict__ v_b, int64_t R, int nb,
                                                                float* __restrict__ t_out, float* __restrict__ v_out,
                                                                int64_t* __restrict__ pio, int64_t* __restrict__ ridx_out,
                                                                float inv_s, int n_fine, int use_est, float* __restrict__ csum,
                                                                float* __restrict__ t_new, const float* __restrict__ rays_o,
                                                                const float* __restrict__ rays_d, float* __restrict__ x_new,
                                                                const int64_t* __restrict__ live_rank) {
  __shared__ float smp_lds[SMP_WAVES_PER_BLOCK][SMP_LDS_FLOATS];
  const int64_t r = smp_wave_id();
  if (r >= R) return;
  int64_t q;
  const bool live = smp_live(live_rank, r, q);
  const int64_t sa = pia[2 * r], na = live ? pia[2 * r + 1] : 0;
  const int64_t so = sa + q * (int64_t)nb;
  const int nb_r = live ? nb : 0;
  if (nsim_lane() == 0) {
    pio[2 * r] = so;
    pio[2 * r + 1] = na + nb_r;
  }
  if (!live) return;
  float* lds = &smp_lds[threadIdx.x >> 6][0];
  merge_ray(t_a, v_a, sa, na, t_b, v_b, r, q, nb, so, lds, t_out, v_out, ridx_out, nullptr, nullptr, nullptr);
  nsim_wave_fence();
  upsample_ray(t_out + so, v_out + so, na + nb, r, q, inv_s, n_fine, use_est, lds, csum + so, t_new, rays_o, rays_d, x_new);
}

__device__ __forceinline__ float compress_alpha(const float* sdf, int64_t i, int64_t n, float s) {
  if (i + 1 >= n) return 0.f;
  const float c0 = smp_sigmoid(sdf[i] * s), c1 = smp_sigmoid(sdf[i + 1] * s);
  const float a = (c0 - c1 + 1e-5f) / (c0 + 1e-5f);
  return fminf(fmaxf(a, 0.f), 1.f);
}

template <bool EMIT>
__global__ void __launch_bounds__(SMP_BLOCK) k_compress(const float* __restrict__ sdf, const float* __restrict__ t,
                                                         const int64_t* __restrict__ pi, int64_t R,
                                                         const float* __restrict__ ln_inv_s, float factor,
                                                         float forward_inv_s, float thre, int64_t* __restrict__ counts,
                                                         const int64_t* __restrict__ pi_out, float* __restrict__ t_out,
                                                         int64_t* __restrict__ ridx_out, int64_t tail_n) {
  const int64_t r = smp_wave_id();
  if (r >= R) return;
  const int lane = nsim_lane();
  if (EMIT && tail_n > 0) {
    const int64_t S = pi_out[2 * (R - 1)] + pi_out[2 * (R - 1) + 1];
    for (int64_t i = r * 64 + lane; i < tail_n; i += R * 64) {
      t_out[S + i] = 0.f;
      ridx_out[S + i] = R + i;
    }
  }
  const int64_t st = pi[2 * r], n = pi[2 * r + 1];
  const float s = forward_inv_s > 0.f ? forward_inv_s : expf(ln_inv_s[0] * factor);
  const float* ss = sdf + st;
  float carry = 1.0f;
  bool prev_sig = false;
  int cnt = 0;
  const int64_t ost = EMIT ? pi_out[2 * r] : 0;
  for (int64_t base = 0; base < n; base += 64) {
    const int64_t i = base + lane;
    const bool valid = i < n;
    const float a = valid ? compress_alpha(ss, i, n, s) : 0.f;
    const float f = valid ? (1.0f - a + 1e-10f) : 1.0f;
    const float incl = wave_incl_prod(f);
    float excl = wave_shfl(incl, lane - 1);
    if (lane == 0) excl = 1.0f;
    const float vw = a * (carry * excl);
    carry = carry * wave_shfl(incl, 63);
    const bool sig = valid && (vw > thre);
    int psig = wave_shfl((int)sig, lane - 1);
    if (lane == 0) psig = prev_sig ? 1 : 0;
    prev_sig = wave_shfl((int)sig, 63) != 0;
    const bool keep = valid && (sig || psig != 0);
    const unsigned long long m = wave_ballot(keep);
    if (EMIT && keep) {
      const int before = __popcll(m & ((1ull << lane) - 1ull));
      t_out[ost + cnt + before] = t[st + i];
      ridx_out[ost + cnt + before] = r;
    }
    cnt += __popcll(m);
  }
  if (!EMIT && lane == 0) counts[r] = cnt;
}

extern "C" {

int nsim_raygen_pinhole(const float* xy, const int64_t* fidx, const float* intr, const float* c2w,
                        const int64_t* WH, int64_t N, int snap, float* rays_o, float* rays_d, void* stream) {
  if (N <= 0) return 0;
  hipLaunchKernelGGL(k_raygen_pinhole, dim3(nsim_blocks(N, 256)), dim3(256), 0, (hipStream_t)stream, xy, fidx, intr, c2w,
                     WH, N, snap, rays_o, rays_d, (const float*)nullptr, 0);
  NSIM_CHECK_LAUNCH();
  return 0;
}

int nsim_raygen_opencv(const float* xy, const int64_t* fidx, const float* intr, const float* distortion, int n_iters,
                       const float* c2w, const int64_t* WH, int64_t N, int snap, float* rays_o, float* rays_d,
                       void* stream) {
  if (N <= 0) return 0;
  if (!distortion || n_iters < 0 || n_iters > 64) return 4;
  hipLaunchKernelGGL(k_raygen_pinhole, dim3(nsim_blocks(N, 256)), dim3(256), 0, (hipStream_t)stream, xy, fidx, intr, c2w,
                     WH, N, snap, rays_o, rays_d, distortion, n_iters);
  NSIM_CHECK_LAUNCH();
  return 0;
}

int nsim_raygen_fisheye(const float* xy, const int64_t* fidx, const float* intr, const float* distortion, int n_iters,
                        const float* c2w, const int64_t* WH, int64_t N, int snap, float* rays_o, float* rays_d,
                        void* stream) {
  if (N <= 0) return 0;
  if (!distortion || n_iters < 1 || n_iters > 64) return 4;
  hipLaunchKernelGGL(k_raygen_pinhole, dim3(nsim_blocks(N, 256)), dim3(256), 0, (hipStream_t)stream, xy, fidx, intr, c2w,
                     WH, N, snap, rays_o, rays_d, distortion, -n_iters);
  NSIM_CHECK_LAUNCH();
  return 0;
}

int nsim_raygen_fisheye_bwd(const float* xy, const int64_t* fidx, const float* intr, const float* distortion, int n_iters,
                            const float* c2w, const int64_t* WH, int64_t N, int snap, const float* d_rays_o,
                            const float* d_rays_d, float* d_c2w, void* stream) {
  if (N <= 0) return 0;
  if (!d_c2w || !distortion || n_iters < 1 || n_iters > 64) return 4;
  hipLaunchKernelGGL(k_raygen_pinhole_bwd, dim3(nsim_blocks(N, 256)), dim3(256), 0, (hipStream_t)stream, xy, fidx, intr,
                     c2w, WH, N, snap, d_rays_o, d_rays_d, d_c2w, distortion, -n_iters);
  NSIM_CHECK_LAUNCH();
  return 0;
}

int nsim_raygen_pinhole_bwd(const float* xy, const int64_t* fidx, const float* intr, const float* c2w,
                            const int64_t* WH, int64_t N, int snap, const float* d_rays_o, const float* d_rays_d,
                            float* d_c2w, void* stream) {
  if (N <= 0) return 0;
  if (!d_c2w) return 4;
  hipLaunchKernelGGL(k_raygen_pinhole_bwd, dim3(nsim_blocks(N, 256)), dim3(256), 0, (hipStream_t)stream, xy, fidx, intr,
                     c2w, WH, N, snap, d_rays_o, d_rays_d, d_c2w, (const float*)nullptr, 0);
  NSIM_CHECK_LAUNCH();
  return 0;
}

int nsim_raygen_opencv_bwd(const float* xy, const int64_t* fidx, const float* intr, const float* distortion, int n_iters,
                           const float* c2w, const int64_t* WH, int64_t N, int snap, const float* d_rays_o,
                           const float* d_rays_d, float* d_c2w, void* stream) {
  if (N <= 0) return 0;
  if (!d_c2w || !distortion || n_iters < 0 || n_iters > 64) return 4;
  hipLaunchKernelGGL(k_raygen_pinhole_bwd, dim3(nsim_blocks(N, 256)), dim3(256), 0, (hipStream_t)stream, xy, fidx, intr,
                     c2w, WH, N, snap, d_rays_o, d_rays_d, d_c2w, distortion, n_iters);
  NSIM_CHECK_LAUNCH();
  return 0;
}

int nsim_aabb_ray_test(const float* rays_o, const float* rays_d, int64_t N, const NsimOccMeta* meta, float near,
                       float far, float* near_out, float* far_out, uint8_t* hit, void* stream) {
  if (N <= 0) return 0;
  if (!meta) return 5;
  hipLaunchKernelGGL(k_aabb_ray_test, dim3(nsim_blocks(N, 256)), dim3(256), 0, (hipStream_t)stream, rays_o, rays_d, N,
                     occ_dev(meta), near, far, near_out, far_out, hit);
  NSIM_CHECK_LAUNCH();
  return 0;
}

int nsim_occ_decay(float* val, int64_t nvox, float decay, void* stream) {
  if (nvox <= 0) return 0;
  hipLaunchKernelGGL(k_occ_decay, dim3(nsim_blocks(nvox, 256)), dim3(256), 0, (hipStream_t)stream, val, nvox, decay);
  NSIM_CHECK_LAUNCH();
  return 0;
}

int nsim_occ_update(float* val, const float* pts, const float* sdf, int64_t n, const NsimOccMeta* meta,
                    float inv_s, void* stream) {
  if (n <= 0) return 0;
  if (!meta) return 5;
  hipLaunchKernelGGL(k_occ_update, dim3(nsim_blocks(n, 256)), dim3(256), 0, (hipStream_t)stream, val, pts, sdf, n,
                     occ_dev(meta), inv_s, (const int64_t*)nullptr, (int64_t)0);
  NSIM_CHECK_LAUNCH();
  return 0;
}

int nsim_occ_collect(float* val, const float* pts, const float* sdf, int64_t n, const int64_t* n_dev, int64_t n_add,
                     const NsimOccMeta* meta, float inv_s, void* stream) {
  if (n <= 0) return 0;
  if (!meta) return 5;
  hipLaunchKernelGGL(k_occ_update, dim3(nsim_blocks(n, 256)), dim3(256), 0, (hipStream_t)stream, val, pts, sdf, n,
                     occ_dev(meta), inv_s, n_dev, n_add);
  NSIM_CHECK_LAUNCH();
  return 0;
}

int nsim_occ_pack_bits(const float* val, int64_t nvox, float thre, uint32_t* bits, void* stream) {
  if (nvox <= 0) return 0;
  hipLaunchKernelGGL(k_occ_pack_bits, dim3(nsim_blocks((nvox + 31) / 32, 256)), dim3(256), 0, (hipStream_t)stream, val,
                     nvox, thre, bits);
  NSIM_CHECK_LAUNCH();
  return 0;
}

int nsim_march_count(const float* rays_o, const float* rays_d, const float* near, const float* far,
                     const float* jitter, int64_t R, const uint32_t* bits, const int64_t* ray_word_off,
                     const NsimOccMeta* meta, float step, int max_steps, int64_t* counts, void* stream) {
  if (R <= 0) return 0;
  if (!meta || !(step > 0.f)) return 5;
  hipLaunchKernelGGL(k_march_count, smp_grid(R), dim3(SMP_BLOCK), 0, (hipStream_t)stream, rays_o, rays_d, near, far,
                     jitter, R, bits, ray_word_off, occ_dev(meta), step, max_steps, counts);
  NSIM_CHECK_LAUNCH();
  return 0;
}

int nsim_march_emit(const float* rays_o, const float* rays_d, const float* near, const float* far,
                    const float* jitter, int64_t R, const uint32_t* bits, const int64_t* ray_word_off,
                    const NsimOccMeta* meta, float step, int max_steps, const int64_t* pack_infos, float* t_out,
                    void* stream) {
  if (R <= 0) return 0;
  if (!meta || !(step > 0.f)) return 5;
  hipLaunchKernelGGL(k_march_emit, smp_grid(R), dim3(SMP_BLOCK), 0, (hipStream_t)stream, rays_o, rays_d, near, far, jitter,
                     R, bits, ray_word_off, occ_dev(meta), step, max_steps, pack_infos, t_out);
  NSIM_CHECK_LAUNCH();
  return 0;
}

int nsim_coarse_depths(const float* near, const float* far, const float* jitter_c, int64_t R, int C, float* out,
                       const int64_t* live_rank, void* stream) {
  if (R <= 0 || C <= 0) return 0;
  hipLaunchKernelGGL(k_coarse_depths, dim3(nsim_blocks(R * C, 256)), dim3(256), 0, (hipStream_t)stream, near, far,
                     jitter_c, R, C, out, live_rank);
  NSIM_CHECK_LAUNCH();
  return 0;
}

int nsim_upsample_stage(const float* t, const float* sdf, const int64_t* pack_infos, int64_t R, float inv_s,
                        int n_fine, int use_estimate_alpha, float* scratch, float* t_new, const float* rays_o,
                        const float* rays_d, float* x_new, const int64_t* live_rank, void* stream) {
  if (R <= 0 || n_fine <= 0) return 0;
  if (x_new && !(rays_o && rays_d)) return 24;
  hipLaunchKernelGGL(k_upsample_stage, smp_grid(R), dim3(SMP_BLOCK), 0, (hipStream_t)stream, t, sdf, pack_infos, R, inv_s,
                     n_fine, use_estimate_alpha, scratch, t_new, rays_o, rays_d, x_new, live_rank);
  NSIM_CHECK_LAUNCH();
  return 0;
}

int nsim_merge_sorted(const float* t_a, const float* v_a, const int64_t* pack_infos_a, const float* t_b,
                      const float* v_b, int64_t R, int nb, float* t_out, float* v_out, int64_t* pack_infos_out,
                      int64_t* ridx_out, const float* rays_o, const float* rays_d, float* x_out, const int64_t* live_rank,
                      void* stream) {
  if (R <= 0) return 0;
  if (x_out && !(rays_o && rays_d)) return 24;
  hipLaunchKernelGGL(k_merge_sorted, smp_grid(R), dim3(SMP_BLOCK), 0, (hipStream_t)stream, t_a, v_a, pack_infos_a, t_b, v_b,
                     R, nb, t_out, v_out, pack_infos_out, ridx_out, rays_o, rays_d, x_out, live_rank);
  NSIM_CHECK_LAUNCH();
  return 0;
}

int nsim_merge_upsample(const float* t_a, const float* v_a, const int64_t* pack_infos_a, const float* t_b, const float* v_b,
                        int64_t R, int nb, float* t_out, float* v_out, int64_t* pack_infos_out, int64_t* ridx_out, float inv_s,
                        int n_fine, int use_estimate_alpha, float* scratch, float* t_new, const float* rays_o,
                        const float* rays_d, float* x_new, const int64_t* live_rank, void* stream) {
  if (R <= 0) return 0;
  if (n_fine <= 0 || !v_a || !v_b || !v_out || !scratch || !t_new) return 4;
  if (x_new && !(rays_o && rays_d)) return 24;
  hipLaunchKernelGGL(k_merge_upsample, smp_grid(R), dim3(SMP_BLOCK), 0, (hipStream_t)stream, t_a, v_a, pack_infos_a, t_b, v_b, R,
                     nb, t_out, v_out, pack_infos_out, ridx_out, inv_s, n_fine, use_estimate_alpha, scratch, t_new, rays_o,
                     rays_d, x_new, live_rank);
  NSIM_CHECK_LAUNCH();
  return 0;
}

int nsim_compress_count(const float* sdf, const int64_t* pack_infos, int64_t R, const float* ln_inv_s,
                        float ln_inv_s_factor, float forward_inv_s, float thre, int64_t* counts, void* stream) {
  if (R <= 0) return 0;
  hipLaunchKernelGGL((k_compress<false>), smp_grid(R), dim3(SMP_BLOCK), 0, (hipStream_t)stream, sdf, nullptr, pack_infos, R,
                     ln_inv_s, ln_inv_s_factor, forward_inv_s, thre, counts, nullptr, nullptr, nullptr, (int64_t)0);
  NSIM_CHECK_LAUNCH();
  return 0;
}

int nsim_compress_emit(const float* sdf, const float* t, const int64_t* pack_infos, int64_t R, const float* ln_inv_s,
                       float ln_inv_s_factor, float forward_inv_s, float thre, const int64_t* pack_infos_out,
                       float* t_out, int64_t* ridx_out, int64_t tail_n, void* stream) {
  if (R <= 0) return 0;
  hipLaunchKernelGGL((k_compress<true>), smp_grid(R), dim3(SMP_BLOCK), 0, (hipStream_t)stream, sdf, t, pack_infos, R,
                     ln_inv_s, ln_inv_s_factor, forward_inv_s, thre, nullptr, pack_infos_out, t_out, ridx_out, tail_n);
  NSIM_CHECK_LAUNCH();
  return 0;
}

}
```

### neuralsim_amd/fields/neus.py

```python
import ctypes
import math
import os
import time
from typing import Dict, Optional, Sequence

import torch
import torch.nn as nn

from .. import _lib
from ..grid_encodings.lotd import LoTDConfig, LoTDEncoding
from ..graphics import pack_ops as po
from ..model_base import ModelMixin
from ..spatial import AABBSpace, aabb_ray_test

def C_memmove(dst, src):
    ctypes.memmove(ctypes.byref(dst), ctypes.byref(src), ctypes.sizeof(src))


DEFAULT_LOD_RES = [16, 23, 31, 43, 59, 81, 112, 154, 213, 295, 407, 562, 777, 1073, 1483, 2048]
RAD_IN = 26


def _flat_sizes(D: int, L: int = 16, E: int = 0):
    n_sdf_w = 64 * (2 * L + E) + (64 * 64 if D == 2 else 0) + 64
    n_sdf_b = 64 * D + 1
    n_rad_w = 64 * RAD_IN + 64 * 64 + 3 * 64
    n_rad_b = 131
    return n_sdf_w, n_sdf_b, n_rad_w, n_rad_b


def append_extra_points(model, rays_o, rays_d, t, ridx, h_appear, extra_x):
    dev = rays_o.device
    R, M = rays_o.shape[0], extra_x.shape[0]
    xe = extra_x.detach().float().reshape(-1, 3)
    ck = (M, str(dev))
    cache = getattr(model, "_extra_cache", None)
    if cache is None or cache[0] != ck:
        ez = torch.zeros([M, 3], dtype=torch.float32, device=dev)
        ez[:, 2] = 1.0
        cache = model._extra_cache = (ck, ez, torch.zeros([M], dtype=torch.float32, device=dev),
                                      torch.zeros([M, 4], dtype=torch.float32, device=dev))
    _, ez, tz, hz = cache
    rays_o, rays_d = torch.cat([rays_o, xe]), torch.cat([rays_d, ez])
    t = torch.cat([t, tz])
    ridx = torch.cat([ridx, torch.arange(R, R + M, device=dev)])
    if h_appear is not None:
        hz = hz if h_appear.shape[1] == 4 else hz.new_zeros([M, h_appear.shape[1]])
        h_appear = torch.cat([h_appear.detach().float(), hz])
    return rays_o, rays_d, t, ridx, h_appear


def fine_list(qp: dict):
    nf = qp.get("num_fine", [8, 8, 32])
    if isinstance(nf, (list, tuple)):
        return [int(n) for n in nf]
    k = max(len(qp.get("upsample_inv_s_factors", [1, 4, 16])), 1)
    return [max(int(nf) // k, 1)] * k


def marched_only(qp: dict) -> bool:
    v = qp.get("upsample_on_marched_only", None)
    if v is None:
        return os.environ.get("NSIM_UPSAMPLE_ON_MARCHED_ONLY", "1") == "1"
    return bool(v)




_SPEC_FORWARD = os.environ.get("NSIM_SPEC_FORWARD", "1") == "1"
_EVAL_PLANES = os.environ.get("NSIM_EVAL_PLANES", "0") == "1"
_SDF_FUSED_BELOW = int(os.environ.get("NSIM_SDF_FUSED_BELOW", "0"))
_FUSE_MERGE_UPSAMPLE = os.environ.get("NSIM_FUSE_MERGE_UPSAMPLE", "1") == "1"


class _FieldFn(torch.autograd.Function):

    @staticmethod
    def forward(ctx, model, grid, sdf_w, sdf_b, rad_w, rad_b, h_appear, x, rays_o, rays_d, t, ridx, with_rgb,
                goff=None, extra_x=None, pre=None):
        dev = grid.device
        M = 0
        ctx.PS = 0
        if pre is not None:
            M = pre["M"]
            rays_o, rays_d, t, ridx, ha = pre["rays_o"], pre["rays_d"], pre["t"], pre["ridx"], pre["ha"]
            S = t.shape[0]
            sdf, nablas, rgb = pre["sdf"][:S], pre["nablas"][:S], (pre["rgb"][:S] if with_rgb else None)
            h_pl, J_pl, ctx.PS = pre["h_pl"], pre["J_pl"], pre["PS"]
            if _lib.TIMER is not None:
                _lib.TIMER.note_units("nsim_field_fwd", S)
            ctx.model, ctx.S, ctx.with_rgb, ctx.M = model, S, with_rgb, M
            ctx.enc_state = pre.get("enc_state")
            ctx.grid_numel = grid.numel()
            ctx.grid16 = None
            ctx.x_shape = None
            ctx.save_for_backward(None, rays_o, rays_d, t, ridx, ha, nablas, rgb, h_pl, J_pl)
            ctx.goff = None
            ctx.ha_shape = ha.shape if ha is not None else None
            ctx.set_materialize_grads(False)
            if M == 0:
                return (sdf, nablas, rgb) if with_rgb else (sdf, nablas)
            Sm = S - M
            return (sdf[:Sm], nablas[:Sm]) + ((rgb[:Sm],) if with_rgb else ()) + (sdf[Sm:], nablas[Sm:])
        if extra_x is not None:
            assert x is None and goff is None, "extra points ride on a ray-mode query of a single-instance model"
            M = extra_x.shape[0]
            rays_o, rays_d, t, ridx, h_appear = append_extra_points(model, rays_o, rays_d, t, ridx, h_appear, extra_x)
        S = x.shape[0] if x is not None else t.shape[0]
        grid16, wpack = model._shadow()
        sdf = torch.empty([S], dtype=torch.float32, device=dev)
        nablas = torch.empty([S, 3], dtype=torch.float32, device=dev)
        rgb = torch.empty([S, 3], dtype=torch.float32, device=dev) if with_rgb else None
        ha = h_appear.detach().float().contiguous() if h_appear is not None else None
        need_bwd = any(ctx.needs_input_grad)
        NLP = model.plane_levels
        need_pl = need_bwd or NLP > 16 or model.planes_always or _EVAL_PLANES
        PS = _lib.plane_pitch(S)
        h_pl = torch.empty([NLP, PS, 2], dtype=torch.float32, device=dev) if need_pl else None
        J_pl = torch.empty([NLP, PS, 2, 3], dtype=_lib.jplane_dtype(model.field_meta), device=dev) if need_pl else None
        ctx.enc_state = model._enc_field_fwd(grid16, wpack, x, rays_o, rays_d, t, ridx, goff, ha, S, sdf, nablas, rgb, h_pl, J_pl,
                                             None, 0)
        if _lib.TIMER is not None:
            _lib.TIMER.note_units("nsim_field_fwd", S)
        ctx.model, ctx.S, ctx.with_rgb, ctx.M = model, S, with_rgb, M
        ctx.grid_numel = grid.numel()
        ctx.grid16 = grid16
        ctx.x_shape = x.shape if x is not None else None
        ctx.save_for_backward(x, rays_o, rays_d, t, ridx, ha, nablas, rgb, h_pl, J_pl)
        ctx.goff = goff
        ctx.ha_shape = ha.shape if ha is not None else None
        ctx.set_materialize_grads(False)
        if M == 0:
            return (sdf, nablas, rgb) if with_rgb else (sdf, nablas)
        Sm = S - M
        outs = (sdf[:Sm], nablas[:Sm]) + ((rgb[:Sm],) if with_rgb else ()) + (sdf[Sm:], nablas[Sm:])
        return outs

    @staticmethod
    def backward(ctx, *grads):
        model = ctx.model
        x, rays_o, rays_d, t, ridx, ha, nab_fwd, rgb_fwd, h_pl, J_pl = ctx.saved_tensors
        S, M = ctx.S, ctx.M
        dev = nab_fwd.device
        g_sdf, g_nab = grads[0], grads[1]
        g_rgb = grads[2] if ctx.with_rgb else None
        if M > 0:
            Sm = S - M
            ge_s, ge_n = grads[-2], grads[-1]

            def join(a, b, tail):
                if a is None and b is None:
                    return None
                a = a.float() if a is not None else _lib.zeros([Sm, *tail], device=dev)
                b = b.float() if b is not None else _lib.zeros([M, *tail], device=dev)
                return torch.cat([a, b])
            g_sdf, g_nab = join(g_sdf, ge_s, ()), join(g_nab, ge_n, (3,))
            if g_rgb is not None:
                g_rgb = join(g_rgb, None, (3,))
        grid16 = ctx.grid16 if ctx.grid16 is not None else model._table16()
        wpack = model._weight_pack()
        n_sdf_w, n_sdf_b, n_rad_w, n_rad_b = _flat_sizes(model.sdf_D, model.encoding.cfg.num_levels, model.pos_embed_E)
        need = ctx.needs_input_grad
        dgrid = _lib.zeros([ctx.grid_numel], device=dev) if need[1] else None
        dsdf_w, dsdf_b, drad_w, drad_b = _lib.zeros([n_sdf_w + n_sdf_b + n_rad_w + n_rad_b],
                                                    device=dev).split([n_sdf_w, n_sdf_b, n_rad_w, n_rad_b])
        dha = _lib.zeros(list(ctx.ha_shape), device=dev) if (ha is not None and need[6]) else None
        gs = g_sdf.float().contiguous() if g_sdf is not None else None
        gn = g_nab.float().contiguous() if g_nab is not None else None
        gr = g_rgb.float().contiguous() if (ctx.with_rgb and g_rgb is not None) else None
        fm = model.field_meta
        gn_total = gn
        need_x, need_o, need_d = need[7] and x is not None, need[8] and x is None, need[9] and x is None
        need_dx = need_x or need_o or need_d
        dx = dv = None
        if need_dx:
            dx = (torch.empty if gr is not None else torch.zeros)([S, 3], dtype=torch.float32, device=dev)
            dv = torch.empty([S, 3], dtype=torch.float32, device=dev) if (gr is not None and need_d) else None
        if gr is not None:
            gn_total = torch.empty([S, 3], dtype=torch.float32, device=dev)
            _lib.call("nsim_field_bwd_rad", fm, _lib.ptr(wpack), _lib.ptr(nab_fwd.detach()), _lib.ptr(rgb_fwd.detach()),
                      _lib.ptr(x), _lib.ptr(rays_o), _lib.ptr(rays_d), _lib.ptr(t), _lib.ptr(ridx), _lib.ptr(ha), S,
                      _lib.ptr(gn), _lib.ptr(gr), _lib.ptr(gn_total), _lib.ptr(drad_w), _lib.ptr(drad_b), _lib.ptr(dha),
                      _lib.ptr(dx), _lib.ptr(dv))
        NLP = model.plane_levels
        need_pl = dgrid is not None or (need_dx and gn_total is not None)
        dh_pl = torch.empty([NLP, S, 2], dtype=torch.float32, device=dev) if need_pl else None
        g_pl = torch.empty([NLP, S, 2], dtype=torch.float32, device=dev) if need_pl else None
        if model.pos_embed_E:
            if need_dx:
                raise NotImplementedError("pose refinement through a model with extra_pos_embed_cfg (nsim_wide_bwd_sdf has no "
                                          "dL/dx output)")
            _lib.call("nsim_wide_bwd_sdf", fm, _lib.ptr(wpack), _lib.ptr(x), _lib.ptr(rays_o), _lib.ptr(rays_d), _lib.ptr(t),
                      _lib.ptr(ridx), S, _lib.ptr(h_pl), _lib.ptr(J_pl), int(ctx.PS), _lib.ptr(gs), _lib.ptr(gn_total),
                      _lib.ptr(dh_pl), _lib.ptr(g_pl), _lib.ptr(dsdf_w), _lib.ptr(dsdf_b))
        else:
            _lib.call("nsim_field_bwd_sdf", fm, _lib.ptr(wpack), _lib.ptr(h_pl), _lib.ptr(J_pl), S, _lib.ptr(gs),
                      _lib.ptr(gn_total), _lib.ptr(dh_pl), _lib.ptr(g_pl), _lib.ptr(dsdf_w), _lib.ptr(dsdf_b), _lib.ptr(dx),
                      int(ctx.PS))
        d_x = d_o = d_d = None
        if need_dx:
            if gn_total is not None:
                model._enc_hess_dx(grid16, x, rays_o, rays_d, t, ridx, ctx.goff, S, g_pl, gn_total, dx)
            if need_x:
                d_x = dx.reshape(ctx.x_shape)
            else:
                Rt = rays_o.shape[0]
                d_o = torch.zeros([Rt, 3], dtype=torch.float32, device=dev) if need_o else None
                d_d = torch.zeros([Rt, 3], dtype=torch.float32, device=dev) if need_d else None
                _lib.call("nsim_ray_grad_reduce", _lib.ptr(dx), _lib.ptr(dv), _lib.ptr(t), _lib.ptr(ridx), S,
                          _lib.ptr(d_o), _lib.ptr(d_d))
                if M > 0:
                    d_o = d_o[:Rt - M] if d_o is not None else None
                    d_d = d_d[:Rt - M] if d_d is not None else None
        if dgrid is not None:
            model._enc_scatter(x, rays_o, rays_d, t, ridx, ctx.goff, S, dh_pl, g_pl, gn_total, dgrid, enc_state=ctx.enc_state)
        if _lib.TIMER is not None:
            _lib.TIMER.note_units("nsim_field_bwd_sdf", S)
            if dgrid is not None:
                _lib.TIMER.note_units("nsim_lotd_scatter", S)
            if gr is not None:
                _lib.TIMER.note_units("nsim_field_bwd_rad", S)
        if model.sdf_scale != 1.0:
            dsdf_w[-64:] /= model.sdf_scale
            dsdf_b[-1:] /= model.sdf_scale
        if dha is not None and M > 0:
            dha = dha[:dha.shape[0] - M]
        if gr is None:
            drad_w = drad_b = dha = None
        return (None, dgrid, dsdf_w, dsdf_b, drad_w, drad_b, dha, d_x, d_o, d_d, None, None, None, None, None, None)


class _NeusAlphaFn(torch.autograd.Function):
    @staticmethod
    def forward(ctx, sdf, ln_inv_s, pack_infos, factor, forward_inv_s):
        sdf = sdf.float().contiguous()
        alpha = torch.empty_like(sdf)
        _lib.call("nsim_neus_alpha_fwd", _lib.ptr(sdf), _lib.ptr(pack_infos), pack_infos.shape[0], _lib.ptr(ln_inv_s),
                  float(factor), float(forward_inv_s), _lib.ptr(alpha))
        ctx.save_for_backward(sdf, ln_inv_s, pack_infos)
        ctx.factor, ctx.fis = float(factor), float(forward_inv_s)
        return alpha

    @staticmethod
    def backward(ctx, g):
        sdf, ln_inv_s, pack_infos = ctx.saved_tensors
        dsdf = torch.empty_like(sdf)
        dln = _lib.zeros(list(ln_inv_s.shape), device=ln_inv_s.device) if ln_inv_s.dtype == torch.float32 else torch.zeros_like(ln_inv_s)
        _lib.call("nsim_neus_alpha_bwd", _lib.ptr(sdf), _lib.ptr(g.float().contiguous()), _lib.ptr(pack_infos),
                  pack_infos.shape[0], _lib.ptr(ln_inv_s), ctx.factor, ctx.fis, _lib.ptr(dsdf), _lib.ptr(dln))
        return dsdf, dln, None, None, None


class _CompositeFn(torch.autograd.Function):

    @staticmethod
    def forward(ctx, alpha, t, rgb, nrm, pack_infos, normalized_depth, out_idx=None, N=None):
        alpha = alpha.float().contiguous()
        t = t.float().contiguous()
        rgbc = rgb.float().contiguous() if rgb is not None else None
        nrmc = nrm.float().contiguous() if nrm is not None else None
        P = pack_infos.shape[0]
        dev = alpha.device
        vw = torch.empty_like(alpha)
        trans = torch.empty_like(alpha)
        f32 = dict(dtype=torch.float32, device=dev)
        if out_idx is None:
            mask, depth = torch.empty([P], **f32), torch.empty([P], **f32)
            rgb_o = (torch.empty if rgbc is not None else torch.zeros)([P, 3], **f32)
            nrm_o = (torch.empty if nrmc is not None else torch.zeros)([P, 3], **f32)
        else:
            sc = _lib.zeros([2, N], device=dev)
            mask, depth = sc[0], sc[1]
            vec = _lib.zeros([2, N, 3], device=dev)
            rgb_o, nrm_o = vec[0], vec[1]
            out_idx = out_idx.contiguous()
        _lib.call("nsim_composite_fwd", _lib.ptr(alpha), _lib.ptr(t), _lib.ptr(rgbc), _lib.ptr(nrmc),
                  _lib.ptr(pack_infos), P, int(normalized_depth), _lib.ptr(vw), _lib.ptr(trans), _lib.ptr(mask),
                  _lib.ptr(depth), _lib.ptr(rgb_o), _lib.ptr(nrm_o), _lib.ptr(out_idx))
        ctx.save_for_backward(alpha, trans, vw, t, rgbc, nrmc, pack_infos, mask, depth, out_idx)
        ctx.nd = int(normalized_depth)
        ctx.mark_non_differentiable(trans)
        ctx.set_materialize_grads(False)
        return vw, mask, depth, rgb_o, nrm_o, trans

    @staticmethod
    def backward(ctx, g_vw, g_mask, g_depth, g_rgb, g_nrm, _g_trans):
        alpha, trans, vw, t, rgbc, nrmc, pack_infos, mask, depth, out_idx = ctx.saved_tensors
        P = pack_infos.shape[0]

        def c(g):
            return g.float().contiguous() if g is not None else None
        dalpha = torch.empty_like(alpha)
        drgb = torch.empty_like(rgbc) if rgbc is not None else None
        dnrm = torch.empty_like(nrmc) if nrmc is not None else None
        _lib.call("nsim_composite_bwd", _lib.ptr(alpha), _lib.ptr(trans), _lib.ptr(vw), _lib.ptr(t), _lib.ptr(rgbc),
                  _lib.ptr(nrmc), _lib.ptr(pack_infos), P, ctx.nd, _lib.ptr(mask), _lib.ptr(depth), _lib.ptr(c(g_mask)),
                  _lib.ptr(c(g_depth)), _lib.ptr(c(g_rgb)), _lib.ptr(c(g_nrm)), _lib.ptr(c(g_vw)), _lib.ptr(dalpha),
                  _lib.ptr(drgb), _lib.ptr(dnrm), _lib.ptr(out_idx))
        return dalpha, None, drgb, dnrm, None, None, None, None


def volume_integration(alpha, t, rgb, nablas, pack_infos, depth_use_normalized_vw=False, rays_inds=None,
                       num_rays: int = None) -> Dict[str, torch.Tensor]:
    vw, mask, depth, rgb_o, nrm_o, trans = _CompositeFn.apply(alpha, t, rgb, nablas, pack_infos, depth_use_normalized_vw,
                                                             rays_inds, num_rays)
    out = dict(vw=vw, mask_volume=mask, depth_volume=depth, trans=trans)
    if rgb is not None:
        out["rgb_volume"] = rgb_o
    if nablas is not None:
        out["normals_volume"] = nrm_o
    return out


class OccGridAccel(nn.Module):

    def __init__(self, aabb: torch.Tensor, resolution=(64, 64, 64), occ_thre=0.3, ema_decay=0.95, inv_s=256.0,
                 num_steps=4, num_pts=2 ** 20, n_steps_between_update=16, n_steps_warmup=256, device=None,
                 update_from_samples_cfg: Optional[dict] = None, init_cfg: Optional[dict] = None):
        super().__init__()
        self.init_cfg = dict(init_cfg or {})
        self.update_from_samples_cfg = None if update_from_samples_cfg is None else dict(update_from_samples_cfg)
        self.collect_armed = False
        self.sync_values = None
        self.resolution = [int(r) for r in resolution]
        self.occ_thre, self.ema_decay, self.inv_s = float(occ_thre), float(ema_decay), float(inv_s)
        self.num_steps, self.num_pts = int(num_steps), int(num_pts)
        self.n_steps_between_update, self.n_steps_warmup = n_steps_between_update, n_steps_warmup
        nvox = self.resolution[0] * self.resolution[1] * self.resolution[2]
        self.register_buffer("aabb", aabb.float().reshape(2, 3).clone())
        self.register_buffer("occ_val", torch.zeros(nvox, dtype=torch.float32))
        self.register_buffer("occ_bits", torch.full([(nvox + 31) // 32], -1, dtype=torch.int32))
        if device is not None:
            self.to(device)
        self.meta = self._make_meta()

    def _make_meta(self):
        m = _lib.OccMeta()
        a = self.aabb.detach().cpu()
        res = torch.tensor(self.resolution, dtype=torch.float32)
        scale = res / (a[1] - a[0])
        for i in range(3):
            m.aabb_min[i] = float(a[0, i])
            m.aabb_max[i] = float(a[1, i])
            m.scale[i] = float(scale[i])
            m.res[i] = self.resolution[i]
        return m

    @property
    def occ_grid(self) -> torch.Tensor:
        r = self.resolution
        return (self.occ_val > self.occ_thre).view(r[2], r[1], r[0]).permute(2, 1, 0)

    def frac_occupied(self) -> float:
        return float((self.occ_val > self.occ_thre).float().mean())

    def set_all_occupied(self):
        self.occ_val.fill_(1.0)
        self.pack_bits()

    def pack_bits(self):
        _lib.call("nsim_occ_pack_bits", _lib.ptr(self.occ_val), self.occ_val.shape[0], self.occ_thre,
                  _lib.ptr(self.occ_bits))

    @torch.no_grad()
    def draw_points(self, n: int, generator=None) -> torch.Tensor:
        dev = self.occ_val.device
        lo, hi = self.aabb[0], self.aabb[1]
        if os.environ.get("NSIM_OCC_IID", "0") == "1":
            return lo + torch.rand([n, 3], device=dev, generator=generator) * (hi - lo)
        rx, ry, rz = self.resolution
        nvox = rx * ry * rz
        sweep = getattr(self, "_sweep", 0) % nvox
        self._sweep = (sweep + n) % nvox
        key = (n, sweep, str(dev), self.aabb._version)
        cache = getattr(self, "_corner_cache", None)
# ... 361 lines not shown
            return
        C_memmove(fs, fm)
        fs.precision = code[sp]
        lib = _lib.get_lib()
        if a[1].numel() != int(lib.nsim_field_wpack_bytes(fm)) or b[1].numel() != int(lib.nsim_field_wpack_bytes(fs)):
            return
        _lib.call("nsim_field_pack_weights2", fm, _lib.ptr(a[1]), fs, _lib.ptr(b[1]), _lib.ptr(self.sdf_w.detach()),
                  _lib.ptr(self.sdf_b.detach()), _lib.ptr(self.rad_w.detach()), _lib.ptr(self.rad_b.detach()))
        object.__setattr__(self, "_wpack_slot", (va, a[1]))
        object.__setattr__(self, "_wpack_slot_s", (vb, b[1]))

    def _sampling_ctx(self):
        sp = self.sampling_precision
        fm = self.field_meta
        code = {"fp16": 0, "f32": 1, "split": 2}
        if sp is None or code[sp] == fm.precision or (sp == "split" and fm.precision == 1):
            return fm, self._shadow()[1]
        fs = getattr(self, "_field_meta_s", None)
        if fs is None:
            fs = _lib.FieldMeta()
            object.__setattr__(self, "_field_meta_s", fs)
        C_memmove(fs, fm)
        fs.precision = code[sp]
        self._shadow()
        return fs, self._pack_for(fs, "_wpack_slot_s")

    @torch.no_grad()
    def geometric_init_sphere(self, radius: float = 0.5, noise_scale: float = 0.25, inside_out: bool = None,
                              level: int = None):
        cfg = self.encoding.cfg
        lv = max(l for l, t in enumerate(cfg.lod_types) if t == "Dense") if level is None else int(level)
        assert cfg.lod_types[lv] == "Dense", "the sphere is written to a dense level"
        Rx, Ry, Rz = cfg.lod_res3[lv]
        zz, yy, xx = torch.meshgrid(torch.linspace(-1.0, 1.0, Rz), torch.linspace(-1.0, 1.0, Ry),
                                    torch.linspace(-1.0, 1.0, Rx), indexing="ij")
        sdf = (torch.sqrt(xx ** 2 + yy ** 2 + zz ** 2) - radius).reshape(-1)
        if self.inside_out if inside_out is None else inside_out:
            sdf = -sdf
        sdf = sdf * self.sdf_scale
        lvl = self.encoding.flattened_params.data[cfg.lod_offsets[lv]: cfg.lod_offsets[lv] + cfg.lod_sizes[lv] * 2].view(-1, 2)
        lvl[:, 0] = sdf.half().float().to(lvl.device)
        D = self.sdf_D
        F1 = 2 * cfg.num_levels + self.pos_embed_E
        w1 = self.sdf_w.data[:64 * F1].view(64, F1)
        w1.mul_(noise_scale)
        w1[0].zero_()
        w1[1].zero_()
        w1[0, 2 * lv], w1[1, 2 * lv] = 1.0, -1.0
        self.sdf_b.data[:64].mul_(noise_scale)
        self.sdf_b.data[0:2] = 0.0
        if D == 2:
            w2 = self.sdf_w.data[64 * F1:64 * F1 + 4096].view(64, 64)
            w2.mul_(noise_scale)
            w2[0].zero_()
            w2[1].zero_()
            w2[0, 0], w2[0, 1], w2[1, 0], w2[1, 1] = 1.0, -1.0, -1.0, 1.0
            self.sdf_b.data[64:128].mul_(noise_scale)
            self.sdf_b.data[64:66] = 0.0
        wh = self.sdf_w.data[-64:]
        wh.mul_(noise_scale * 0.05)
        wh[0], wh[1] = 1.0, -1.0
        self.sdf_b.data[-1] = 0.0
        self.encoding.flattened_params.add_(0)
        self.sdf_w.add_(0)
        return self

    @property
    def implicit_surface(self):
        return self

    @torch.no_grad()
    def geometric_init_fn(self, sdf_fn, noise_scale: float = 0.25, level: int = None):
        self.geometric_init_sphere(0.5, noise_scale=noise_scale, inside_out=False, level=level)
        cfg = self.encoding.cfg
        lv = max(l for l, t in enumerate(cfg.lod_types) if t == "Dense") if level is None else int(level)
        Rx, Ry, Rz = cfg.lod_res3[lv]
        zz, yy, xx = torch.meshgrid(torch.linspace(-1.0, 1.0, Rz), torch.linspace(-1.0, 1.0, Ry),
                                    torch.linspace(-1.0, 1.0, Rx), indexing="ij")
        a = self.accel.aabb.detach().cpu()
        xn = torch.stack([xx.reshape(-1), yy.reshape(-1), zz.reshape(-1)], dim=-1)
        x_obj = a[0] + (xn + 1.0) * 0.5 * (a[1] - a[0])
        sdf = sdf_fn(x_obj).reshape(-1).float() * self.sdf_scale
        lvl = self.encoding.flattened_params.data[cfg.lod_offsets[lv]: cfg.lod_offsets[lv] + cfg.lod_sizes[lv] * 2].view(-1, 2)
        lvl[:, 0] = sdf.half().float().to(lvl.device)
        self.encoding.flattened_params.add_(0)
        return self

    def set_var_ctrl(self, ctrl_type: Optional[str] = "mix_linear", start_it: int = 0, stop_it: int = 1,
                     final_inv_s: float = 2000.0):
        assert ctrl_type in (None, "mix_linear")
        self._var_ctrl = None if ctrl_type is None else dict(start_it=int(start_it), stop_it=int(stop_it),
                                                             final_inv_s=float(final_inv_s))
        self._ctrl_mix = 0.0

    def training_before_per_step(self, it: int, logger=None):
        if self.accel is not None and self.accel.update_from_samples_cfg is not None:
            self.accel.collect_armed = True
        vc = getattr(self, "_var_ctrl", None)
        if vc is not None:
            span = max(vc["stop_it"] - vc["start_it"], 1)
            self._ctrl_mix = min(max((int(it) - vc["start_it"]) / span, 0.0), 1.0)
        post = getattr(self, "_reference_post", None)
        if post is not None:
            if post.get("anneal") is not None:
                self.anneal_levels(int(it), **post["anneal"])
            self.accel.cur_batch__step(int(it), self.query_sdf, generator=getattr(self, "refresh_generator", None))

    def training_after_per_step(self, it: int, logger=None):
        """After ``optimizer.step`` (app/resources/asset_bank.py:300-308): nothing to do -- the fp16 table shadow and
        the packed MFMA weight fragments refresh lazily from the parameter versions."""

    def rendering_before_per_view(self, renderer=None, observer=None, per_frame_info: dict = None):
        """app/resources/asset_bank.py:310-318: no per-view state."""

    def model_setup(self):
        self._shadow()

    def _ln_inv_s_eff(self) -> torch.Tensor:
        a = getattr(self, "_ctrl_mix", 0.0)
        if a <= 0.0 or getattr(self, "_var_ctrl", None) is None:
            return self.ln_inv_s
        inv_s = (1.0 - a) * torch.exp(self.ln_inv_s * self.ln_inv_s_factor) + a * self._var_ctrl["final_inv_s"]
        return torch.log(inv_s) / self.ln_inv_s_factor

    def forward_inv_s(self) -> torch.Tensor:
        return torch.exp(self._ln_inv_s_eff() * self.ln_inv_s_factor)

    planes_always = False

    def _wide_weights(self):
        sw, sb = self.sdf_w.detach(), self.sdf_b.detach()
        if self.sdf_scale != 1.0:
            sw, sb = sw.clone(), sb.clone()
            sw[-64:] /= self.sdf_scale
            sb[-1:] /= self.sdf_scale
        return sw.contiguous(), sb.contiguous()

    def _enc_field_fwd(self, grid16, wpack, x, rays_o, rays_d, t, ridx, goff, ha, S, sdf, nablas, rgb, h_pl, J_pl, n_dev,
                       n_add):
        _lib.call("nsim_field_fwd", self.field_meta, _lib.ptr(grid16), _lib.ptr(wpack), _lib.ptr(x), _lib.ptr(rays_o),
                  _lib.ptr(rays_d), _lib.ptr(t), _lib.ptr(ridx), _lib.ptr(goff), _lib.ptr(ha), S, _lib.ptr(sdf),
                  _lib.ptr(nablas), _lib.ptr(rgb), _lib.ptr(h_pl), _lib.ptr(J_pl), _lib.ptr(n_dev), int(n_add))

    def _enc_gather_feat(self, fm, grid16, x, rays_o, rays_d, t, ridx, goff, S, n_dev, n_add, planes):
        _lib.call("nsim_lotd_gather_lm", fm, _lib.ptr(grid16), _lib.ptr(x), _lib.ptr(rays_o), _lib.ptr(rays_d),
                  _lib.ptr(t), _lib.ptr(ridx), _lib.ptr(goff), S, _lib.ptr(n_dev), int(n_add), _lib.ptr(planes))

    def _enc_scatter(self, x, rays_o, rays_d, t, ridx, goff, S, dh_pl, g_pl, gn_total, dgrid, enc_state=None):
        _lib.call("nsim_lotd_scatter", self.encoding.cfg.meta, _lib.ptr(x), _lib.ptr(rays_o), _lib.ptr(rays_d),
                  _lib.ptr(t), _lib.ptr(ridx), _lib.ptr(goff), S, _lib.ptr(dh_pl), _lib.ptr(g_pl),
                  _lib.ptr(gn_total), _lib.ptr(dgrid), 0, 0)

    def _enc_hess_dx(self, grid16, x, rays_o, rays_d, t, ridx, goff, S, g_pl, gn_total, dx):
        _lib.call("nsim_lotd_hess_dx", self.encoding.cfg.meta, _lib.ptr(grid16), _lib.ptr(x), _lib.ptr(rays_o),
                  _lib.ptr(rays_d), _lib.ptr(t), _lib.ptr(ridx), _lib.ptr(goff), S, _lib.ptr(g_pl),
                  _lib.ptr(gn_total), _lib.ptr(dx))

    def _sdf_query(self, grid16, wpack, x, rays_o, rays_d, t, ridx, S: int, dev, goff=None, n_dev=None,
                   n_add: int = 0, collect: bool = False, fm=None) -> torch.Tensor:
        sdf = torch.empty([S], dtype=torch.float32, device=dev)
        if S == 0:
            return sdf
        fm = self.field_meta if fm is None else fm
        if self.pos_embed_E:
            return self._sdf_query_wide(grid16, x, rays_o, rays_d, t, ridx, S, dev, goff, n_dev, n_add, collect, sdf)
        planes = None
        small = (_SDF_FUSED_BELOW > 0 and S <= _SDF_FUSED_BELOW and x is not None and goff is None and self.plane_levels == 16
                 and type(self)._enc_gather_feat is LoTDNeuSModel._enc_gather_feat)
        if not self._sdf_fused and not small:
            planes = torch.empty([self.plane_levels * _lib.plane_pitch(S) * (1 if fm.precision == 0 else 2)],
                                 dtype=torch.float32, device=dev)
            self._enc_gather_feat(fm, grid16, x, rays_o, rays_d, t, ridx, goff, S, n_dev, n_add, planes)
        acc = self.accel if collect else None
        _lib.call("nsim_field_sdf", fm, _lib.ptr(grid16), _lib.ptr(wpack), _lib.ptr(x), _lib.ptr(rays_o),
                  _lib.ptr(rays_d), _lib.ptr(t), _lib.ptr(ridx), _lib.ptr(goff), S, _lib.ptr(n_dev), int(n_add),
                  _lib.ptr(sdf), _lib.ptr(planes), _lib.ptr(acc.occ_val) if acc is not None else None,
                  acc.meta if acc is not None else None, float(acc.inv_s) if acc is not None else 0.0)
        if _lib.TIMER is not None and n_dev is None:
            _lib.TIMER.note_units("nsim_field_sdf", S)
            if planes is not None:
                _lib.TIMER.note_units("nsim_lotd_gather_lm", S)
        return sdf

    def _sdf_query_wide(self, grid16, x, rays_o, rays_d, t, ridx, S, dev, goff, n_dev, n_add, collect, sdf):
        fm32 = getattr(self, "_field_meta_f32", None)
        if fm32 is None:
            fm32 = _lib.FieldMeta()
            object.__setattr__(self, "_field_meta_f32", fm32)
        C_memmove(fm32, self.field_meta)
        fm32.precision = 1
        planes = torch.empty([self.plane_levels * _lib.plane_pitch(S) * 2], dtype=torch.float32, device=dev)
        self._enc_gather_feat(fm32, grid16, x, rays_o, rays_d, t, ridx, goff, S, n_dev, n_add, planes)
        sw, sb = self._wide_weights()
        _lib.call("nsim_wide_sdf", fm32, int(self.pos_embed_n), _lib.ptr(sw), _lib.ptr(sb), _lib.ptr(x), _lib.ptr(rays_o),
                  _lib.ptr(rays_d), _lib.ptr(t), _lib.ptr(ridx), S, _lib.ptr(n_dev), int(n_add), _lib.ptr(planes), _lib.ptr(sdf))
        if collect:
            pts = x if x is not None else torch.addcmul(rays_o[ridx], t.unsqueeze(-1), rays_d[ridx])
            self.accel.collect(pts.contiguous(), sdf, n_dev, n_add)
        return sdf

    @torch.no_grad()
    def query_sdf(self, x: torch.Tensor) -> torch.Tensor:
        shape = x.shape[:-1]
        x = x.detach().float().reshape(-1, 3).contiguous()
        grid16, wpack = self._shadow()
        sdf = self._sdf_query(grid16, wpack, x, None, None, None, None, x.shape[0], x.device)
        return sdf.reshape(shape)

    @torch.no_grad()
    def _query_sdf_rays(self, rays_o, rays_d, t, ridx, goff=None, n_dev=None, n_add=0):
        grid16, wpack = self._shadow()
        return self._sdf_query(grid16, wpack, None, rays_o, rays_d, t, ridx, t.shape[0], t.device, goff=goff,
                               n_dev=n_dev, n_add=n_add)

    def _object_coords(self, x: torch.Tensor, input_normalized: bool) -> torch.Tensor:
        return self.space.unnormalize_coords(x) if input_normalized else x

    def forward_sdf_nablas(self, x: torch.Tensor, nablas_has_grad: bool = True, *,
                           input_normalized: bool = False) -> Dict[str, torch.Tensor]:
        shape = x.shape[:-1]
        x = self._object_coords(x, input_normalized)
        xf = (x if x.requires_grad else x.detach()).float().reshape(-1, 3).contiguous()
        sdf, nablas = _FieldFn.apply(self, self._table(), self.sdf_w, self.sdf_b, self.rad_w,
                                     self.rad_b, None, xf, None, None, None, None, False)
        if not nablas_has_grad:
            nablas = nablas.detach()
        return dict(sdf=sdf.reshape(shape), nablas=nablas.reshape(*shape, 3))

    def forward_sdf(self, x: torch.Tensor, *, input_normalized: bool = False) -> Dict[str, torch.Tensor]:
        return dict(sdf=self.forward_sdf_nablas(self._object_coords(x, input_normalized), nablas_has_grad=False)["sdf"])

    def forward(self, x: torch.Tensor, v: torch.Tensor, *, with_rgb: bool = True, with_normal: bool = False,
                input_normalized: bool = False, h_appear: torch.Tensor = None) -> Dict[str, torch.Tensor]:
        shape = x.shape[:-1]
        o = self._object_coords(x, input_normalized).detach().float().reshape(-1, 3).contiguous()
        d = v.detach().float().reshape(-1, 3).contiguous()
        n = o.shape[0]
        t = torch.zeros([n], dtype=torch.float32, device=o.device)
        ridx = torch.arange(n, device=o.device)
        ha = h_appear.reshape(n, -1) if h_appear is not None else None
        outs = _FieldFn.apply(self, self._table(), self.sdf_w, self.sdf_b, self.rad_w, self.rad_b, ha, None, o, d, t, ridx,
                              bool(with_rgb))
        ret = dict(sdf=outs[0].reshape(shape))
        if with_rgb:
            ret["rgb"] = outs[2].reshape(*shape, 3)
        if with_normal:
            ret["nablas"] = outs[1].reshape(*shape, 3)
        return ret

    def sample_pts_uniform(self, num_pts: int, generator=None) -> Dict[str, torch.Tensor]:
        lo, hi = self.accel.aabb[0], self.accel.aabb[1]
        x = lo + torch.rand([num_pts, 3], device=self.device, generator=generator) * (hi - lo)
        ret = self.forward_sdf_nablas(x)
        ret["net_x"] = x
        return ret

    def sample_pts_in_occupied(self, num_pts: int, generator=None) -> Dict[str, torch.Tensor]:
        acc = self.accel
        occ_idx = (acc.occ_val > acc.occ_thre).nonzero()[:, 0]
        if occ_idx.numel() == 0:
            return self.sample_pts_uniform(num_pts, generator=generator)
        dev = self.device
        pick = occ_idx[torch.randint(0, occ_idx.numel(), [num_pts], device=dev, generator=generator)]
        rx, ry = acc.resolution[0], acc.resolution[1]
        vox = torch.stack([pick % rx, (pick // rx) % ry, pick // (rx * ry)], dim=-1).to(torch.float32)
        res = torch.tensor(acc.resolution, dtype=torch.float32, device=dev)
        lo, hi = acc.aabb[0], acc.aabb[1]
        x = lo + (vox + torch.rand([num_pts, 3], device=dev, generator=generator)) / res * (hi - lo)
        ret = self.forward_sdf_nablas(x)
        ret["net_x"] = x
        return ret

    @staticmethod
    def convert_rays_in_node(rays_o, rays_d, rotation: torch.Tensor, translation: torch.Tensor, scale=1.0):
        Rt = rotation.transpose(-1, -2)
        o = ((rays_o - translation).unsqueeze(-2) * Rt).sum(-1) / scale
        d = (rays_d.unsqueeze(-2) * Rt).sum(-1) / scale
        return o, d

    def ray_test(self, rays_o, rays_d, near=None, far=None, **extra) -> Dict:
        return aabb_ray_test(self.accel.aabb, self.accel.meta, rays_o, rays_d, near=near, far=far, **extra)

    def _arange_repeat(self, R: int, n: int, dev):
        key = (R, n, str(dev))
        c = getattr(self, "_ar_cache", None)
        if c is None:
            c = self._ar_cache = {}
        if key not in c:
            if len(c) > 16:
                c.clear()
            c[key] = torch.arange(R, device=dev).repeat_interleave(n)
        return c[key]

    def _sample(self, o, d, near, far, qp: dict, jitter, jitter_c, goff=None, woff=None, cap: Optional[int] = None,
                pre_sync_hook=None, need_ridx: bool = True):
        R = o.shape[0]
        dev = o.device
        f32 = dict(dtype=torch.float32, device=dev)
        march = qp.get("march_cfg", {})
        step, max_steps = float(march.get("step_size", 0.005)), int(march.get("max_steps", 4096))
        C = int(qp.get("num_coarse", 64))
        bits, occm = self.accel.occ_bits, self.accel.meta
        counts = torch.empty([R], dtype=torch.long, device=dev)
        _lib.call("nsim_march_count", _lib.ptr(o), _lib.ptr(d), _lib.ptr(near), _lib.ptr(far), _lib.ptr(jitter), R,
                  _lib.ptr(bits), _lib.ptr(woff), occm, step, max_steps, _lib.ptr(counts))
        nt = self._host_notify() if cap is not None else None
        self._notify_seq_m = None
        fine = fine_list(qp)
        mo = marched_only(qp)
        lr = live_idx = cnts = None
        self._live = None
        adr_m = None
        if nt is not None:
            adr_m, self._notify_seq_m = nt.arm(0)
        if mo:
            assert len(fine) <= 4, "upsample_on_marched_only: at most four up-sampling stages"
            lr = torch.empty([R], dtype=torch.long, device=dev)
            live_idx = torch.empty([R], dtype=torch.long, device=dev)
            cnts = torch.empty([8], dtype=torch.long, device=dev)
            pi_m = torch.empty([R, 2], dtype=torch.long, device=dev)
            total_m = torch.empty([1], dtype=torch.long, device=dev)
            adr_l, seq_l = nt.arm(2) if nt is not None else (None, 0)
            _lib.call("nsim_live_rank", _lib.ptr(counts), R, C, *((list(fine) + [0, 0, 0, 0])[:4]), _lib.ptr(lr), _lib.ptr(live_idx),
                      _lib.ptr(cnts), adr_l, seq_l, _lib.ptr(pi_m), _lib.ptr(total_m), -1 if cap is None else int(cap), adr_m,
                      self._notify_seq_m or 0)
            self._live = dict(rank=lr, idx=live_idx, cnts=cnts, seq=seq_l if nt is not None else None, n=None)
        elif nt is not None:
            pi_m, total_m = po.get_pack_infos_from_n(counts, return_total=True, cap=int(cap), notify=(adr_m, self._notify_seq_m))
        else:
            pi_m, total_m = po.get_pack_infos_from_n(counts, return_total=True, cap=-1 if cap is None else int(cap))
        Rl = R
        if cap is None:
            if pre_sync_hook is not None:
                pre_sync_hook()
            if mo:
                c_host = cnts.tolist()
                M, Rl = int(c_host[6]), int(c_host[0])
                self._live["n"] = Rl
                if Rl == 0:
                    self._last_S_q, self._S_per_live = 0, C + sum(int(n) for n in fine)
                    e = torch.empty([0], **f32)
                    return (e, e, torch.zeros([R, 2], dtype=torch.long, device=dev),
                            torch.empty([0], dtype=torch.long, device=dev) if need_ridx else None, counts, total_m)
            else:
                M = int(total_m.item())
            n_dev = None
        else:
            M, n_dev = int(cap), total_m

        def n_of(k):
            if n_dev is None:
                return None
            return cnts[1 + k:2 + k] if mo else (n_dev if k == 0 else None)
        t_m = torch.empty([max(M, 1)], **f32)
        _lib.call("nsim_march_emit", _lib.ptr(o), _lib.ptr(d), _lib.ptr(near), _lib.ptr(far), _lib.ptr(jitter), R,
                  _lib.ptr(bits), _lib.ptr(woff), occm, step, max_steps, _lib.ptr(pi_m), _lib.ptr(t_m))
        t_c = torch.empty([max(Rl, 1), C], **f32)
        _lib.call("nsim_coarse_depths", _lib.ptr(near), _lib.ptr(far), _lib.ptr(jitter_c), R, C, _lib.ptr(t_c), _lib.ptr(lr))
        S = M + Rl * C
        t = torch.empty([S], **f32)
        pi = torch.empty([R, 2], dtype=torch.long, device=dev)
        with_x = not self._sdf_fused
        per_ray = goff is not None or self._per_ray_condition()
        ridx_mid = (not with_x) or per_ray
        ridx = torch.empty([S], dtype=torch.long, device=dev) if (ridx_mid or (need_ridx and not fine)) else None
        xq = torch.empty([S, 3], **f32) if with_x else None
        _lib.call("nsim_merge_sorted", _lib.ptr(t_m), None, _lib.ptr(pi_m), _lib.ptr(t_c), None, R, C, _lib.ptr(t), None,
                  _lib.ptr(pi), _lib.ptr(ridx), _lib.ptr(o), _lib.ptr(d), _lib.ptr(xq), _lib.ptr(lr))
        grid16, wpack = self._shadow()
        fm_s = None
        if with_x:
            fm_s, wpack = self._sampling_ctx()
        collect = with_x and goff is None and self.accel.collect_armed
        n0, a0 = (n_of(0), 0) if mo else (n_dev, R * C)
        if with_x:
            sdf = self._sdf_query(grid16, wpack, xq, None, None, None, ridx if per_ray else None, S, dev,
                                  goff=goff, n_dev=n0, n_add=a0, collect=collect, fm=fm_s)
        else:
            sdf = self._query_sdf_rays(o, d, t, ridx, goff, n_dev=n0, n_add=a0)
        inv_s0 = float(qp.get("upsample_inv_s", 64.0))
        use_est = 1 if qp.get("upsample_use_estimate_alpha", True) else 0
        factors = list(qp.get("upsample_inv_s_factors", [1, 4, 16]))
        stages = list(zip(fine, factors))
        fuse = _FUSE_MERGE_UPSAMPLE
        t_new = x_new = None
        for k_stage, (nf, fac) in enumerate(stages):
            nf = int(nf)
            if t_new is None:
                t_new = torch.empty([max(Rl, 1), nf], **f32)
                scratch = torch.empty([S], **f32)
                x_new = torch.empty([max(Rl, 1) * nf, 3], **f32) if with_x else None
                _lib.call("nsim_upsample_stage", _lib.ptr(t), _lib.ptr(sdf), _lib.ptr(pi), R, inv_s0 * float(fac), nf, use_est,
                          _lib.ptr(scratch), _lib.ptr(t_new), _lib.ptr(o), _lib.ptr(d), _lib.ptr(x_new), _lib.ptr(lr))
            if not mo:
                ridx_new = self._arange_repeat(R, nf, dev)
            elif per_ray or not with_x:
                ridx_new = live_idx[:Rl].repeat_interleave(nf)
            else:
                ridx_new = None
            if with_x:
                sdf_new = self._sdf_query(grid16, wpack, x_new, None, None, None, ridx_new if per_ray else None,
                                          Rl * nf, dev, goff=goff, n_dev=n_of(1 + k_stage) if mo else None, collect=collect, fm=fm_s)
            else:
                sdf_new = self._query_sdf_rays(o, d, t_new.reshape(-1)[:Rl * nf], ridx_new, goff)
            S2 = S + Rl * nf
            t2 = torch.empty([S2], **f32)
            sdf2 = torch.empty([S2], **f32)
            pi2 = torch.empty([R, 2], dtype=torch.long, device=dev)
            last = k_stage == len(stages) - 1
            ridx = torch.empty([S2], dtype=torch.long, device=dev) if (ridx_mid or (need_ridx and last)) else None
            if fuse and not last:
                nf2, fac2 = int(stages[k_stage + 1][0]), stages[k_stage + 1][1]
                t_nx = torch.empty([max(Rl, 1), nf2], **f32)
                scratch = torch.empty([S2], **f32)
                x_nx = torch.empty([max(Rl, 1) * nf2, 3], **f32) if with_x else None
                _lib.call("nsim_merge_upsample", _lib.ptr(t), _lib.ptr(sdf), _lib.ptr(pi), _lib.ptr(t_new), _lib.ptr(sdf_new), R, nf,
                          _lib.ptr(t2), _lib.ptr(sdf2), _lib.ptr(pi2), _lib.ptr(ridx), inv_s0 * float(fac2), nf2, use_est,
                          _lib.ptr(scratch), _lib.ptr(t_nx), _lib.ptr(o), _lib.ptr(d), _lib.ptr(x_nx), _lib.ptr(lr))
                t_new, x_new = t_nx, x_nx
            else:
                _lib.call("nsim_merge_sorted", _lib.ptr(t), _lib.ptr(sdf), _lib.ptr(pi), _lib.ptr(t_new), _lib.ptr(sdf_new), R,
                          nf, _lib.ptr(t2), _lib.ptr(sdf2), _lib.ptr(pi2), _lib.ptr(ridx), None, None, None, _lib.ptr(lr))
                t_new = x_new = None
            t, sdf, pi, S = t2, sdf2, pi2, S2
        self._last_S_q = S
        self._S_per_live = C + sum(int(n) for n in fine)
        return t, sdf, pi, ridx, counts, total_m

    def _host_notify(self):
        nt = getattr(self, "_notify", None)
        if nt is None:
            nt = self._notify = _lib.HostNotify(3) if os.environ.get("NSIM_HOST_NOTIFY", "1") == "1" else False
        return nt or None

    def _compress(self, t, sdf, pi, forward_inv_s: float, thre: float, total_m=None, pre_sync_hook=None, tail: int = 0,
                  spec_launch=None):
        R = pi.shape[0]
        dev = t.device
        counts = torch.empty([R], dtype=torch.long, device=dev)
        ln_eff = self._ln_inv_s_eff().detach()
        _lib.call("nsim_compress_count", _lib.ptr(sdf), _lib.ptr(pi), R, _lib.ptr(ln_eff),
                  self.ln_inv_s_factor, forward_inv_s, thre, _lib.ptr(counts))
        nt = self._host_notify()
        self._spec_ok = False
        cap_k = self._keep_cap(R) if (spec_launch is not None and nt is not None) else None
        seq_k = None
        if nt is not None:
            adr, seq_k = nt.arm(1)
            pi_k, total = po.get_pack_infos_from_n(counts, return_total=True, notify=(adr, seq_k),
                                                   cap=-1 if cap_k is None else cap_k)
        else:
            pi_k, total = po.get_pack_infos_from_n(counts, return_total=True)

        def emit(n_out, tail_):
            t_o = torch.empty([n_out + tail_], dtype=torch.float32, device=dev)
            r_o = torch.empty([n_out + tail_], dtype=torch.long, device=dev)
            _lib.call("nsim_compress_emit", _lib.ptr(sdf), _lib.ptr(t), _lib.ptr(pi), R, _lib.ptr(ln_eff),
                      self.ln_inv_s_factor, forward_inv_s, thre, _lib.ptr(pi_k), _lib.ptr(t_o), _lib.ptr(r_o), tail_)
            return t_o, r_o
        if cap_k is not None:
            t_k, ridx_k = emit(cap_k, int(tail))
            spec_launch(t_k, ridx_k, pi_k, total, cap_k)
        if pre_sync_hook is not None:
            pre_sync_hook()
        Sk = M_true = None
        _w0 = time.perf_counter() if _lib.HOST_WAIT is not None else 0.0
        if nt is not None:
            Sk = nt.wait(1, seq_k)
            if Sk is not None and total_m is not None:
                M_true = nt.wait(0, self._notify_seq_m) if self._notify_seq_m is not None else None
                if M_true is None:
                    Sk = None
        if Sk is None:
            if total_m is None:
                Sk, M_true = int(total.item()), None
            else:
                Sk, M_true = torch.cat([total, total_m]).tolist()
            if nt is not None and int(nt.view[1, 1]) != seq_k:
                self._notify = False
        lv = getattr(self, "_live", None)
        if lv is not None and lv["n"] is None:
            n_l = nt.wait(2, lv["seq"]) if (nt is not None and self._notify and lv["seq"] is not None) else None
            lv["n"] = int(lv["cnts"][0].item()) if n_l is None else int(n_l)
        if _lib.HOST_WAIT is not None:
            _lib.HOST_WAIT += time.perf_counter() - _w0
        self._keep_stat = (R, Sk)
        if cap_k is not None and Sk <= cap_k and Sk > 0:
            self._spec_ok = True
            self._with_tail = (t_k[:Sk + int(tail)], ridx_k[:Sk + int(tail)]) if tail else None
            return t_k[:Sk], pi_k, ridx_k[:Sk], M_true
        if cap_k is not None:
            pi_k = po.get_pack_infos_from_n(counts)
        tail = int(tail) if Sk > 0 else 0
        if Sk > 0:
            t_k, ridx_k = emit(Sk, tail)
        else:
            t_k = torch.empty([0], dtype=torch.float32, device=dev)
            ridx_k = torch.empty([0], dtype=torch.long, device=dev)
        self._with_tail = (t_k, ridx_k) if tail else None
        return t_k[:Sk], pi_k, ridx_k[:Sk], M_true

    def _keep_cap(self, R: int) -> Optional[int]:
        st = getattr(self, "_keep_stat", None)
        if st is None or not self._speculate:
            return None
        R0, K0 = st
        if R0 <= 0 or K0 <= 0 or not (0.5 <= R / R0 <= 2.0):
            return None
        return ((int(1.3 * K0 * R / R0) + 4096) + 31) & ~31

    def _speculative_cap(self, R: int) -> Optional[int]:
        st = getattr(self, "_march_stat", None)
        if st is None or not self._speculate:
            return None
        R0, M0 = st
        if R0 <= 0 or not (0.5 <= R / R0 <= 2.0):
            return None
        return int(1.3 * M0 * R / R0) + 8192

    def _query_samples(self, ray_tested: dict, cfg: dict, qp: dict):
        R = ray_tested["num_rays"]
        self._last_R_tested = int(R)
        o = ray_tested["rays_o"].detach().float().contiguous()
        d = ray_tested["rays_d"].detach().float().contiguous()
        near, far = ray_tested["near"].contiguous(), ray_tested["far"].contiguous()
        dev = o.device
        perturb = cfg.get("perturb", False)
        jitter = cfg.get("_jitter", None)
        jitter_c = cfg.get("_jitter_c", None)
        if jitter is None and perturb:
            jitter = torch.rand([R], device=dev)
            jitter_c = torch.rand([R, int(qp.get("num_coarse", 64))], device=dev)
        if jitter is not None:
            jitter = jitter.float().contiguous()
        if jitter_c is not None:
            jitter_c = jitter_c.float().contiguous()
        fis = cfg.get("forward_inv_s", None)
        fis = float(fis) if fis else 0.0
        mode = cfg.get("query_mode", self.ray_query_cfg.get("query_mode", "march_occ_multi_upsample"))
        goff = ray_tested.get("rays_goff", None)
        woff = ray_tested.get("rays_word_off", None)
        with torch.no_grad():
            compressed = mode.endswith("_compressed")
            cap = self._speculative_cap(R) if compressed else None
            hook = cfg.get("_pre_sync_hook", None)
            t, sdf_ng, pi, ridx, march_counts, total_m = self._sample(o, d, near, far, qp, jitter, jitter_c, goff, woff,
                                                                      cap=cap, pre_sync_hook=hook if cap is None else None,
                                                                      need_ridx=not compressed)
            if compressed:
                thre = float(qp.get("compress_thre", 1e-4))
                tail = int(cfg.get("_tail_points", 0))
                t_k, pi_k, ridx_k, M_true = self._compress(t, sdf_ng, pi, fis, thre, total_m if cap is not None else None,
                                                           pre_sync_hook=hook if cap is not None else None, tail=tail,
                                                           spec_launch=cfg.get("_spec_launch") if cap is not None else None)
                if cap is not None and M_true > cap:
                    t, sdf_ng, pi, ridx, march_counts, total_m = self._sample(o, d, near, far, qp, jitter, jitter_c,
                                                                              goff, woff, cap=None, need_ridx=False)
                    t_k, pi_k, ridx_k, _ = self._compress(t, sdf_ng, pi, fis, thre, tail=tail)
                    M_true = int(total_m.item())
                lv = getattr(self, "_live", None)
                Rl = int(lv["n"]) if lv is not None else R
                per_live = int(qp.get("num_coarse", 64)) + sum(fine_list(qp))
                if M_true is None:
                    M_true = int(sdf_ng.shape[0]) - Rl * per_live
                self._march_stat = (R, M_true)
                self._last_S_q = M_true + Rl * per_live
                if _lib.TIMER is not None and cap is not None:
                    sizes = [M_true + Rl * int(qp.get("num_coarse", 64))]
                    if lv is not None:
                        sizes += [Rl * int(n) for n in fine_list(qp)]
                    for S0 in sizes:
                        _lib.TIMER.note_units("nsim_field_sdf", S0)
                        if not self._sdf_fused:
                            _lib.TIMER.note_units("nsim_lotd_gather_lm", S0)
                t, pi, ridx = t_k, pi_k, ridx_k
        self.accel.collect_armed = False
        return o, d, t, pi, ridx, sdf_ng, march_counts, goff, fis

    def ray_query(self, *, ray_input: dict = None, ray_tested: dict, config, return_buffer: bool = True,
                  return_details: bool = False, render_per_obj_individual: bool = False) -> Dict:
        cfg = dict(config)
        qp = dict(cfg.get("query_param", self.ray_query_cfg.get("query_param", {})))
        with_rgb = cfg.get("with_rgb", True)
        with_normal = cfg.get("with_normal", False)
        if cfg.get("with_feature_dim", 0):
            raise NotImplementedError("with_feature_dim > 0: the decoders of this model emit no extra feature channels")
        ret = dict()
        R = ray_tested["num_rays"]
        n_all = None
        if render_per_obj_individual and ray_input is not None and ray_input.get("rays_o") is not None:
            n_all = int(ray_input["rays_o"].shape[0])

        def empty_rendered():
            dev = ray_tested["rays_inds"].device
            z = lambda *sh: torch.zeros([n_all or 0, *sh], dtype=torch.float32, device=dev)
            r_ = dict(mask_volume=z(), depth_volume=z())
            if with_rgb:
                r_["rgb_volume"] = z(3)
            if with_normal:
                r_["normals_volume"] = z(3)
            return r_
        if R == 0:
            ret["volume_buffer"] = dict(type="empty")
            if render_per_obj_individual:
                ret["rendered"] = empty_rendered()
            if return_details:
                ret["details"] = dict()
            return ret
        h_appear = ray_tested.get("rays_h_appear", None)
        extra_x = cfg.get("_extra_pts", None)
        o_g, d_g = ray_tested["rays_o"], ray_tested["rays_d"]
        spec = None
        mode = cfg.get("query_mode", self.ray_query_cfg.get("query_mode", "march_occ_multi_upsample"))
        if (_SPEC_FORWARD and type(self) is LoTDNeuSModel and mode.endswith("_compressed") and torch.is_grad_enabled()
                and self.encoding.flattened_params.requires_grad and not (o_g.requires_grad or d_g.requires_grad)):
            M = int(extra_x.shape[0]) if extra_x is not None else 0
            o_a, d_a = o_g.detach().float().contiguous(), d_g.detach().float().contiguous()
            ha_a = h_appear.detach().float().contiguous() if (with_rgb and h_appear is not None) else None
            pre_od = cfg.get("_extra_pre", None)
            if M and pre_od is not None and pre_od[0].shape[0] == o_a.shape[0] + M:
                o_a, d_a = pre_od
                if ha_a is not None:
                    hz = getattr(self, "_extra_hz", None)
                    if hz is None or hz.shape != (M, ha_a.shape[1]) or hz.device != ha_a.device:
                        hz = self._extra_hz = torch.zeros([M, ha_a.shape[1]], dtype=torch.float32, device=ha_a.device)
                    ha_a = torch.cat([ha_a, hz])
            elif M:
                e = torch.empty([0], dtype=torch.float32, device=o_a.device)
                o_a, d_a, _, _, ha_a = append_extra_points(self, o_a, d_a, e, e.long(), ha_a, extra_x)
            spec = dict(M=M, rays_o=o_a, rays_d=d_a, ha=ha_a)

            def spec_launch(t_full, ridx_full, pi_k, total_dev, cap_k):
                dev_, NLP = t_full.device, self.plane_levels
                Sc = cap_k + M
                PSc = _lib.plane_pitch(Sc)
                f32 = dict(dtype=torch.float32, device=dev_)
                grid16, wpack = self._shadow()
                spec.update(sdf=torch.empty([Sc], **f32), nablas=torch.empty([Sc, 3], **f32),
                            rgb=torch.empty([Sc, 3], **f32) if with_rgb else None,
                            h_pl=torch.empty([NLP, PSc, 2], **f32),
                            J_pl=torch.empty([NLP, PSc, 2, 3], dtype=_lib.jplane_dtype(self.field_meta), device=dev_), PS=PSc)
                spec["enc_state"] = self._enc_field_fwd(grid16, wpack, None, o_a, d_a, t_full, ridx_full, None, ha_a, Sc, spec["sdf"],
                                                        spec["nablas"], spec["rgb"], spec["h_pl"], spec["J_pl"], total_dev, M)
            cfg["_spec_launch"], cfg["_tail_points"] = spec_launch, M
            self._with_tail = None
        o, d, t, pi, ridx, sdf_ng, march_counts, goff, fis = self._query_samples(ray_tested, cfg, qp)
        if t.shape[0] == 0:
            ret["volume_buffer"] = dict(type="empty")
            if render_per_obj_individual:
                ret["rendered"] = empty_rendered()
            if return_details:
                ret["details"] = dict(march_counts=march_counts)
            return ret
        pre = None
        if spec is not None and getattr(self, "_spec_ok", False) and "sdf" in spec:
            t_a, ridx_a = self._with_tail if spec["M"] else (t, ridx)
            pre = dict(spec, t=t_a, ridx=ridx_a)
        o_in = o_g.float().contiguous() if o_g.requires_grad else o
        d_in = d_g.float().contiguous() if d_g.requires_grad else d
        outs = _FieldFn.apply(self, self._table(), self.sdf_w, self.sdf_b, self.rad_w, self.rad_b,
                              h_appear if with_rgb else None, None, o_in, d_in, t, ridx, bool(with_rgb), goff, extra_x, pre)
        sdf, nablas = outs[0], outs[1]
        rgb = outs[2] if with_rgb else None
        if extra_x is not None:
            ret["extra_pts"] = dict(sdf=outs[-2], nablas=outs[-1], net_x=extra_x)
        if not qp.get("nablas_has_grad", True):
            nablas = nablas.detach()
        alpha = _NeusAlphaFn.apply(sdf, self._ln_inv_s_eff(), pi, self.ln_inv_s_factor, fis)
        rays_inds_hit, pi_hit = ray_tested["rays_inds"], pi
        self._rays_sel = None
        lv = getattr(self, "_live", None)
        if lv is not None and lv.get("n") is not None and int(lv["n"]) < R:
            self._rays_sel = lv["idx"][:int(lv["n"])]
            rays_inds_hit, pi_hit = rays_inds_hit[self._rays_sel], pi[self._rays_sel]
        vb = dict(type="packed", rays_inds_hit=rays_inds_hit, pack_infos_hit=pi_hit, t=t, opacity_alpha=alpha,
                  nablas=nablas, sdf=sdf)
        if with_rgb:
            vb["rgb"] = rgb
        ret["volume_buffer"] = vb
        if render_per_obj_individual or cfg.get("_render", False):
            ret["rendered"] = volume_integration(alpha, t, rgb, nablas if (with_normal or cfg.get("_render", False)) else None,
                                                 pi, cfg.get("depth_use_normalized_vw", True),
                                                 rays_inds=ray_tested["rays_inds"] if n_all is not None else None,
                                                 num_rays=n_all)
            ret["rendered"].pop("vw", None)
            ret["rendered"].pop("trans", None)
        if return_details:
            ret["details"] = dict(march_counts=march_counts, sdf_nograd=sdf_ng, ridx=ridx)
        if cfg.get("with_near_sdf", False):
            x_near = (o + ray_tested["near"].float()[:, None] * d).detach()
            ret.setdefault("details", {})["near_sdf"] = self.forward_sdf_nablas(x_near, nablas_has_grad=False)["sdf"]
        return ret
```

Baseline: 7.183 million.

## Fuse march emit, coarse depths and merge into one tail kernel; add fused count-scan

```diff
diff --git a/include/nsim.h b/include/nsim.h
--- a/include/nsim.h
+++ b/include/nsim.h
@@ -132,6 +132,15 @@
 int nsim_upsample_stage(const float* t, const float* sdf, const int64_t* pack_infos, int64_t R, float inv_s,
                         int n_fine, int use_estimate_alpha, float* scratch, float* t_new, const float* rays_o,
                         const float* rays_d, float* x_new, const int64_t* live_rank, void* stream);
+int nsim_march_count_rank(const float* rays_o, const float* rays_d, const float* near, const float* far, const float* jitter,
+                          int64_t R, const uint32_t* bits, const int64_t* ray_word_off, const NsimOccMeta* meta, float step,
+                          int max_steps, int64_t* counts, uint32_t* ticket, int C, int nf0, int nf1, int nf2, int nf3,
+                          int64_t* live_rank, int64_t* live_idx, int64_t* cnts, int64_t* notify, int64_t seq, int64_t* pack_infos,
+                          int64_t* total, int64_t cap, int64_t* notify_total, int64_t seq_total, void* stream);
+int nsim_march_tail(const float* rays_o, const float* rays_d, const float* near, const float* far, const float* jitter, int64_t R,
+                    const uint32_t* bits, const int64_t* ray_word_off, const NsimOccMeta* meta, float step, int max_steps,
+                    const int64_t* pack_infos_m, const float* jitter_c, int C, const int64_t* live_rank, float* t_out,
+                    int64_t* pack_infos_out, int64_t* ridx_out, float* x_out, void* stream);
 int nsim_merge_sorted(const float* t_a, const float* v_a, const int64_t* pack_infos_a, const float* t_b,
                       const float* v_b, int64_t R, int nb, float* t_out, float* v_out,
                       int64_t* pack_infos_out, int64_t* ridx_out, const float* rays_o, const float* rays_d,
@@ -143,6 +152,9 @@
 
 int nsim_compress_count(const float* sdf, const int64_t* pack_infos, int64_t R, const float* ln_inv_s,
                         float ln_inv_s_factor, float forward_inv_s, float thre, int64_t* counts, void* stream);
+int nsim_compress_count_pack(const float* sdf, const int64_t* pack_infos, int64_t R, const float* ln_inv_s, float ln_inv_s_factor,
+                             float forward_inv_s, float thre, int64_t* counts, uint32_t* ticket, int64_t* pack_infos_out,
+                             int64_t* total, int64_t cap, int64_t* notify, int64_t seq, void* stream);
 int nsim_compress_emit(const float* sdf, const float* t, const int64_t* pack_infos, int64_t R, const float* ln_inv_s,
                        float ln_inv_s_factor, float forward_inv_s, float thre, const int64_t* pack_infos_out,
                        float* t_out, int64_t* ridx_out, int64_t tail_n, void* stream);
diff --git a/neuralsim_amd/_lib.py b/neuralsim_amd/_lib.py
--- a/neuralsim_amd/_lib.py
+++ b/neuralsim_amd/_lib.py
@@ -103,12 +103,16 @@
     "nsim_occ_pack_bits": [_P, _I64, _F, _P],
     "nsim_occ_collect": [_P, _P, _P, _I64, _P, _I64, C.POINTER(OccMeta), _F],
     "nsim_march_count": [_P, _P, _P, _P, _P, _I64, _P, _P, C.POINTER(OccMeta), _F, _I, _P],
+    "nsim_march_count_rank": [_P, _P, _P, _P, _P, _I64, _P, _P, C.POINTER(OccMeta), _F, _I, _P, _P, _I, _I, _I, _I, _I, _P, _P, _P,
+                              _P, _I64, _P, _P, _I64, _P, _I64],
+    "nsim_march_tail": [_P, _P, _P, _P, _P, _I64, _P, _P, C.POINTER(OccMeta), _F, _I, _P, _P, _I, _P, _P, _P, _P, _P],
     "nsim_march_emit": [_P, _P, _P, _P, _P, _I64, _P, _P, C.POINTER(OccMeta), _F, _I, _P, _P],
     "nsim_coarse_depths": [_P, _P, _P, _I64, _I, _P, _P],
     "nsim_upsample_stage": [_P, _P, _P, _I64, _F, _I, _I, _P, _P, _P, _P, _P, _P],
     "nsim_merge_sorted": [_P, _P, _P, _P, _P, _I64, _I, _P, _P, _P, _P, _P, _P, _P, _P],
     "nsim_merge_upsample": [_P, _P, _P, _P, _P, _I64, _I, _P, _P, _P, _P, _F, _I, _I, _P, _P, _P, _P, _P, _P],
     "nsim_compress_count": [_P, _P, _I64, _P, _F, _F, _F, _P],
+    "nsim_compress_count_pack": [_P, _P, _I64, _P, _F, _F, _F, _P, _P, _P, _P, _I64, _P, _I64],
     "nsim_compress_emit": [_P, _P, _P, _I64, _P, _F, _F, _F, _P, _P, _P, _I64],
     "nsim_lotd_fwd": [_P, _P, C.POINTER(LotdMeta), _I64, _P, _P],
     "nsim_lotd_bwd": [_P, _P, _P, C.POINTER(LotdMeta), _I64, _P],
@@ -215,6 +219,17 @@
     return t
 
 
+_TICKETS = {}
+
+
+def ticket(device, slot: int) -> torch.Tensor:
+    key = (str(device), stream_handle(), slot)
+    t = _TICKETS.get(key)
+    if t is None:
+        t = _TICKETS[key] = torch.zeros([4], dtype=torch.int32, device=device)
+    return t
+
+
 class HostNotify:
 
     def __init__(self, slots: int = 2):
diff --git a/neuralsim_amd/csrc/build.py b/neuralsim_amd/csrc/build.py
--- a/neuralsim_amd/csrc/build.py
+++ b/neuralsim_amd/csrc/build.py
@@ -6,7 +6,7 @@
 
 HERE = Path(__file__).resolve().parent
 SOURCES = ["pack_ops.hip", "sampling.hip", "lotd.hip", "field.hip", "wide_field.hip", "permuto.hip", "nerf_field.hip", "sky.hip", "loss_ops.hip", "optim.hip", "misc.hip"]
-HEADERS = ["nsim_common.h", "nsim_prims.h", "lotd_dev.h", "mfma_mlp.h", "occ_dev.h", "../../include/nsim.h"]
+HEADERS = ["nsim_common.h", "nsim_prims.h", "lotd_dev.h", "mfma_mlp.h", "occ_dev.h", "pack_scan_dev.h", "../../include/nsim.h"]
 LIB = HERE / "libnsim_hip.so"
 BUILD = HERE / "_build"
 
diff --git a/neuralsim_amd/csrc/pack_ops.hip b/neuralsim_amd/csrc/pack_ops.hip
--- a/neuralsim_amd/csrc/pack_ops.hip
+++ b/neuralsim_amd/csrc/pack_ops.hip
@@ -1,4 +1,5 @@
 #include "nsim_common.h"
+#include "pack_scan_dev.h"
 
 #define PACK_WAVES_PER_BLOCK 4
 #define PACK_BLOCK (64 * PACK_WAVES_PER_BLOCK)
@@ -8,139 +9,19 @@
 }
 static inline dim3 pack_grid(int64_t P) { return dim3(nsim_blocks(P, PACK_WAVES_PER_BLOCK)); }
 
-#define PI_THREADS 1024
-#define PI_PER 8
 __global__ void __launch_bounds__(PI_THREADS) k_pack_infos_from_n(const int64_t* __restrict__ n, int64_t P,
                                                                     int64_t* __restrict__ pi,
                                                                     int64_t* __restrict__ total, int64_t cap,
                                                                     int64_t* notify, int64_t seq) {
-  __shared__ int64_t wtot[PI_THREADS / 64];
-  const int tid = threadIdx.x, lane = nsim_lane(), wave = tid >> 6;
-  int64_t carry = 0;
-  for (int64_t base = 0; base < P; base += (int64_t)PI_THREADS * PI_PER) {
-    const int64_t i0 = base + (int64_t)tid * PI_PER;
-    int64_t v[PI_PER];
-    int64_t mine = 0;
-#pragma unroll
-    for (int k = 0; k < PI_PER; ++k) {
-      v[k] = (i0 + k) < P ? n[i0 + k] : 0;
-      mine += v[k];
-    }
-    const int64_t incl = wave_incl_sum(mine);
-    if (lane == 63) wtot[wave] = incl;
-    __syncthreads();
-    int64_t before = 0, chunk = 0;
-#pragma unroll
-    for (int w = 0; w < PI_THREADS / 64; ++w) {
-      const int64_t x = wtot[w];
-      before += (w < wave) ? x : 0;
-      chunk += x;
-    }
-    int64_t run = carry + before + incl - mine;
-#pragma unroll
-    for (int k = 0; k < PI_PER; ++k) {
-      const int64_t i = i0 + k;
-      if (i < P) {
-        const bool over = cap >= 0 && run + v[k] > cap;
-        pi[2 * i] = (cap >= 0 && run > cap) ? cap : run;
-        pi[2 * i + 1] = over ? 0 : v[k];
-      }
-      run += v[k];
-    }
-    carry += chunk;
-    __syncthreads();
-  }
-  if (tid == 0 && total) total[0] = carry;
-  if (tid == 0 && notify) {
-    nsim_store_system(notify, carry, false);
-    nsim_store_system(notify + 1, seq, true);
-  }
-}
-
-struct LiveArgs {
-  int C;
-  int nf[4];
-};
+  pack_infos_scan(n, P, pi, total, cap, notify, seq);
+}
+
 __global__ void __launch_bounds__(PI_THREADS) k_live_rank(const int64_t* __restrict__ n, int64_t R, LiveArgs la,
                                                            int64_t* __restrict__ live_rank, int64_t* __restrict__ live_idx,
                                                            int64_t* __restrict__ cnts, int64_t* notify, int64_t seq,
                                                            int64_t* __restrict__ pi, int64_t* __restrict__ total, int64_t cap,
                                                            int64_t* notify_total, int64_t seq_total) {
-  __shared__ int64_t wtot[PI_THREADS / 64];
-  __shared__ int wlive[PI_THREADS / 64];
-  const int tid = threadIdx.x, lane = nsim_lane(), wave = tid >> 6;
-  int64_t carry = 0, carry_live = 0;
-  for (int64_t base = 0; base < R; base += (int64_t)PI_THREADS * PI_PER) {
-    const int64_t i0 = base + (int64_t)tid * PI_PER;
-    int64_t v[PI_PER];
-    int64_t mine = 0;
-    int mine_live = 0;
-#pragma unroll
-    for (int k = 0; k < PI_PER; ++k) {
-      v[k] = (i0 + k) < R ? n[i0 + k] : 0;
-      mine += v[k];
-      mine_live += v[k] > 0 ? 1 : 0;
-    }
-    const int64_t incl = wave_incl_sum(mine);
-    const int incl_live = wave_incl_sum(mine_live);
-    if (lane == 63) {
-      wtot[wave] = incl;
-      wlive[wave] = incl_live;
-    }
-    __syncthreads();
-    int64_t before = 0, chunk = 0;
-    int before_live = 0, chunk_live = 0;
-#pragma unroll
-    for (int w = 0; w < PI_THREADS / 64; ++w) {
-      const int64_t x = wtot[w];
-      const int y = wlive[w];
-      before += (w < wave) ? x : 0;
-      chunk += x;
-      before_live += (w < wave) ? y : 0;
-      chunk_live += y;
-    }
-    int64_t run = carry + before + incl - mine;
-    int64_t q = carry_live + before_live + incl_live - mine_live;
-#pragma unroll
-    for (int k = 0; k < PI_PER; ++k) {
-      const int64_t i = i0 + k;
-      if (i < R) {
-        const bool live = v[k] > 0;
-        live_rank[i] = live ? q : ~q;
-        if (live && live_idx) live_idx[q] = i;
-        if (pi) {
-          const bool over = cap >= 0 && run + v[k] > cap;
-          pi[2 * i] = (cap >= 0 && run > cap) ? cap : run;
-          pi[2 * i + 1] = over ? 0 : v[k];
-        }
-        q += live ? 1 : 0;
-      }
-      run += v[k];
-    }
-    carry += chunk;
-    carry_live += chunk_live;
-    __syncthreads();
-  }
-  const int64_t Rl = carry_live, M = carry;
-  if (live_idx)
-    for (int64_t i = Rl + tid; i < R; i += PI_THREADS) live_idx[i] = 0;
-  if (tid == 0) {
-    cnts[0] = Rl;
-    cnts[1] = M + Rl * la.C;
-#pragma unroll
-    for (int k = 0; k < 4; ++k) cnts[2 + k] = Rl * la.nf[k];
-    cnts[6] = M;
-    cnts[7] = 0;
-    if (total) total[0] = M;
-    if (notify) {
-      nsim_store_system(notify, Rl, false);
-      nsim_store_system(notify + 1, seq, true);
-    }
-    if (notify_total) {
-      nsim_store_system(notify_total, M, false);
-      nsim_store_system(notify_total + 1, seq_total, true);
-    }
-  }
+  live_rank_scan(n, R, la, live_rank, live_idx, cnts, notify, seq, pi, total, cap, notify_total, seq_total);
 }
 
 __global__ void __launch_bounds__(PACK_BLOCK) k_packed_sum(const float* __restrict__ x, int C,
diff --git a/neuralsim_amd/csrc/pack_scan_dev.h b/neuralsim_amd/csrc/pack_scan_dev.h
--- /dev/null
+++ b/neuralsim_amd/csrc/pack_scan_dev.h
@@ -0,0 +1,165 @@
+#pragma once
+#include "nsim_common.h"
+
+#define PI_THREADS 1024
+#define PI_PER 8
+
+__device__ __forceinline__ bool nsim_last_workgroup(unsigned* ticket) {
+  __shared__ int nsim_ticket_last;
+#ifdef __HIPCC__
+  asm volatile("s_waitcnt vmcnt(0)" ::: "memory");
+#endif
+  __syncthreads();
+  if (threadIdx.x == 0) {
+#ifdef __HIPCC__
+    __builtin_amdgcn_fence(__ATOMIC_RELEASE, "agent");
+    asm volatile("s_waitcnt vmcnt(0)" ::: "memory");
+    const unsigned prev = __hip_atomic_fetch_add(ticket, 1u, __ATOMIC_RELAXED, __HIP_MEMORY_SCOPE_AGENT);
+#else
+    const unsigned prev = atomicAdd(ticket, 1u);
+#endif
+    const int last = prev == gridDim.x - 1u ? 1 : 0;
+    if (last) {
+#ifdef __HIPCC__
+      __builtin_amdgcn_fence(__ATOMIC_ACQUIRE, "agent");
+      __hip_atomic_store(ticket, 0u, __ATOMIC_RELAXED, __HIP_MEMORY_SCOPE_AGENT);
+      asm volatile("s_waitcnt vmcnt(0)" ::: "memory");
+#else
+      *ticket = 0u;
+#endif
+    }
+    nsim_ticket_last = last;
+  }
+  __syncthreads();
+  return nsim_ticket_last != 0;
+}
+
+__device__ __forceinline__ void pack_infos_scan(const int64_t* n, int64_t P, int64_t* __restrict__ pi, int64_t* __restrict__ total,
+                                                int64_t cap, int64_t* notify, int64_t seq) {
+  __shared__ int64_t wtot[PI_THREADS / 64];
+  const int tid = threadIdx.x, lane = nsim_lane(), wave = tid >> 6;
+  int64_t carry = 0;
+  for (int64_t base = 0; base < P; base += (int64_t)PI_THREADS * PI_PER) {
+    const int64_t i0 = base + (int64_t)tid * PI_PER;
+    int64_t v[PI_PER];
+    int64_t mine = 0;
+#pragma unroll
+    for (int k = 0; k < PI_PER; ++k) {
+      v[k] = (i0 + k) < P ? n[i0 + k] : 0;
+      mine += v[k];
+    }
+    const int64_t incl = wave_incl_sum(mine);
+    if (lane == 63) wtot[wave] = incl;
+    __syncthreads();
+    int64_t before = 0, chunk = 0;
+#pragma unroll
+    for (int w = 0; w < PI_THREADS / 64; ++w) {
+      const int64_t x = wtot[w];
+      before += (w < wave) ? x : 0;
+      chunk += x;
+    }
+    int64_t run = carry + before + incl - mine;
+#pragma unroll
+    for (int k = 0; k < PI_PER; ++k) {
+      const int64_t i = i0 + k;
+      if (i < P) {
+        const bool over = cap >= 0 && run + v[k] > cap;
+        pi[2 * i] = (cap >= 0 && run > cap) ? cap : run;
+        pi[2 * i + 1] = over ? 0 : v[k];
+      }
+      run += v[k];
+    }
+    carry += chunk;
+    __syncthreads();
+  }
+  if (tid == 0 && total) total[0] = carry;
+  if (tid == 0 && notify) {
+    nsim_store_system(notify, carry, false);
+    nsim_store_system(notify + 1, seq, true);
+  }
+}
+
+struct LiveArgs {
+  int C;
+  int nf[4];
+};
+__device__ __forceinline__ void live_rank_scan(const int64_t* n, int64_t R, LiveArgs la, int64_t* __restrict__ live_rank,
+                                               int64_t* __restrict__ live_idx, int64_t* __restrict__ cnts, int64_t* notify,
+                                               int64_t seq, int64_t* __restrict__ pi, int64_t* __restrict__ total, int64_t cap,
+                                               int64_t* notify_total, int64_t seq_total) {
+  __shared__ int64_t wtot[PI_THREADS / 64];
+  __shared__ int wlive[PI_THREADS / 64];
+  const int tid = threadIdx.x, lane = nsim_lane(), wave = tid >> 6;
+  int64_t carry = 0, carry_live = 0;
+  for (int64_t base = 0; base < R; base += (int64_t)PI_THREADS * PI_PER) {
+    const int64_t i0 = base + (int64_t)tid * PI_PER;
+    int64_t v[PI_PER];
+    int64_t mine = 0;
+    int mine_live = 0;
+#pragma unroll
+    for (int k = 0; k < PI_PER; ++k) {
+      v[k] = (i0 + k) < R ? n[i0 + k] : 0;
+      mine += v[k];
+      mine_live += v[k] > 0 ? 1 : 0;
+    }
+    const int64_t incl = wave_incl_sum(mine);
+    const int incl_live = wave_incl_sum(mine_live);
+    if (lane == 63) {
+      wtot[wave] = incl;
+      wlive[wave] = incl_live;
+    }
+    __syncthreads();
+    int64_t before = 0, chunk = 0;
+    int before_live = 0, chunk_live = 0;
+#pragma unroll
+    for (int w = 0; w < PI_THREADS / 64; ++w) {
+      const int64_t x = wtot[w];
+      const int y = wlive[w];
+      before += (w < wave) ? x : 0;
+      chunk += x;
+      before_live += (w < wave) ? y : 0;
+      chunk_live += y;
+    }
+    int64_t run = carry + before + incl - mine;
+    int64_t q = carry_live + before_live + incl_live - mine_live;
+#pragma unroll
+    for (int k = 0; k < PI_PER; ++k) {
+      const int64_t i = i0 + k;
+      if (i < R) {
+        const bool live = v[k] > 0;
+        live_rank[i] = live ? q : ~q;
+        if (live && live_idx) live_idx[q] = i;
+        if (pi) {
+          const bool over = cap >= 0 && run + v[k] > cap;
+          pi[2 * i] = (cap >= 0 && run > cap) ? cap : run;
+          pi[2 * i + 1] = over ? 0 : v[k];
+        }
+        q += live ? 1 : 0;
+      }
+      run += v[k];
+    }
+    carry += chunk;
+    carry_live += chunk_live;
+    __syncthreads();
+  }
+  const int64_t Rl = carry_live, M = carry;
+  if (live_idx)
+    for (int64_t i = Rl + tid; i < R; i += PI_THREADS) live_idx[i] = 0;
+  if (tid == 0) {
+    cnts[0] = Rl;
+    cnts[1] = M + Rl * la.C;
+#pragma unroll
+    for (int k = 0; k < 4; ++k) cnts[2 + k] = Rl * la.nf[k];
+    cnts[6] = M;
+    cnts[7] = 0;
+    if (total) total[0] = M;
+    if (notify) {
+      nsim_store_system(notify, Rl, false);
+      nsim_store_system(notify + 1, seq, true);
+    }
+    if (notify_total) {
+      nsim_store_system(notify_total, M, false);
+      nsim_store_system(notify_total + 1, seq_total, true);
+    }
+  }
+}
diff --git a/neuralsim_amd/csrc/sampling.hip b/neuralsim_amd/csrc/sampling.hip
--- a/neuralsim_amd/csrc/sampling.hip
+++ b/neuralsim_amd/csrc/sampling.hip
@@ -1,5 +1,6 @@
 #include "nsim_common.h"
 #include "occ_dev.h"
+#include "pack_scan_dev.h"
 
 #define SMP_WAVES_PER_BLOCK 4
 #define SMP_BLOCK (64 * SMP_WAVES_PER_BLOCK)
@@ -228,12 +229,11 @@
   return (bits[flat >> 5] >> (flat & 31)) & 1u;
 }
 
-__global__ void __launch_bounds__(SMP_BLOCK) k_march_count(
-    const float* __restrict__ rays_o, const float* __restrict__ rays_d, const float* __restrict__ near,
-    const float* __restrict__ far, const float* __restrict__ jitter, int64_t R, const uint32_t* __restrict__ bits,
-    const int64_t* __restrict__ ray_word_off, OccDev occ, float step, int max_steps, int64_t* __restrict__ counts) {
-  const int64_t r = smp_wave_id();
-  if (r >= R) return;
+__device__ __forceinline__ int march_count_ray(const float* __restrict__ rays_o, const float* __restrict__ rays_d,
+                                               const float* __restrict__ near, const float* __restrict__ far,
+                                               const float* __restrict__ jitter, int64_t r, const uint32_t* __restrict__ bits,
+                                               const int64_t* __restrict__ ray_word_off, const OccDev& occ, float step,
+                                               int max_steps) {
   const int lane = nsim_lane();
   if (ray_word_off) bits += ray_word_off[r];
   const MarchRay m = march_load(rays_o, rays_d, near, far, jitter, r, step, max_steps);
@@ -243,7 +243,32 @@
     const bool hit = march_test(m, occ, bits, base + lane, step, t);
     cnt += __popcll(wave_ballot(hit));
   }
-  if (lane == 0) counts[r] = cnt;
+  return cnt;
+}
+
+__global__ void __launch_bounds__(SMP_BLOCK) k_march_count(
+    const float* __restrict__ rays_o, const float* __restrict__ rays_d, const float* __restrict__ near,
+    const float* __restrict__ far, const float* __restrict__ jitter, int64_t R, const uint32_t* __restrict__ bits,
+    const int64_t* __restrict__ ray_word_off, OccDev occ, float step, int max_steps, int64_t* __restrict__ counts) {
+  const int64_t r = smp_wave_id();
+  if (r >= R) return;
+  const int cnt = march_count_ray(rays_o, rays_d, near, far, jitter, r, bits, ray_word_off, occ, step, max_steps);
+  if (nsim_lane() == 0) counts[r] = cnt;
+}
+
+__global__ void __launch_bounds__(PI_THREADS) k_march_count_rank(
+    const float* __restrict__ rays_o, const float* __restrict__ rays_d, const float* __restrict__ near,
+    const float* __restrict__ far, const float* __restrict__ jitter, int64_t R, const uint32_t* __restrict__ bits,
+    const int64_t* __restrict__ ray_word_off, OccDev occ, float step, int max_steps, int64_t* counts, unsigned* ticket,
+    LiveArgs la, int64_t* __restrict__ live_rank, int64_t* __restrict__ live_idx, int64_t* __restrict__ cnts, int64_t* notify,
+    int64_t seq, int64_t* __restrict__ pi, int64_t* __restrict__ total, int64_t cap, int64_t* notify_total, int64_t seq_total) {
+  const int64_t r = (int64_t)blockIdx.x * (PI_THREADS / 64) + (threadIdx.x >> 6);
+  if (r < R) {
+    const int cnt = march_count_ray(rays_o, rays_d, near, far, jitter, r, bits, ray_word_off, occ, step, max_steps);
+    if (nsim_lane() == 0) counts[r] = cnt;
+  }
+  if (!nsim_last_workgroup(ticket)) return;
+  live_rank_scan(counts, R, la, live_rank, live_idx, cnts, notify, seq, pi, total, cap, notify_total, seq_total);
 }
 
 __global__ void __launch_bounds__(SMP_BLOCK) k_march_emit(
@@ -523,22 +548,11 @@
 }
 
 template <bool EMIT>
-__global__ void __launch_bounds__(SMP_BLOCK) k_compress(const float* __restrict__ sdf, const float* __restrict__ t,
-                                                         const int64_t* __restrict__ pi, int64_t R,
-                                                         const float* __restrict__ ln_inv_s, float factor,
-                                                         float forward_inv_s, float thre, int64_t* __restrict__ counts,
-                                                         const int64_t* __restrict__ pi_out, float* __restrict__ t_out,
-                                                         int64_t* __restrict__ ridx_out, int64_t tail_n) {
-  const int64_t r = smp_wave_id();
-  if (r >= R) return;
+__device__ __forceinline__ int compress_ray(const float* __restrict__ sdf, const float* __restrict__ t,
+                                            const int64_t* __restrict__ pi, int64_t r, const float* __restrict__ ln_inv_s,
+                                            float factor, float forward_inv_s, float thre, const int64_t* __restrict__ pi_out,
+                                            float* __restrict__ t_out, int64_t* __restrict__ ridx_out) {
   const int lane = nsim_lane();
-  if (EMIT && tail_n > 0) {
-    const int64_t S = pi_out[2 * (R - 1)] + pi_out[2 * (R - 1) + 1];
-    for (int64_t i = r * 64 + lane; i < tail_n; i += R * 64) {
-      t_out[S + i] = 0.f;
-      ridx_out[S + i] = R + i;
-    }
-  }
   const int64_t st = pi[2 * r], n = pi[2 * r + 1];
   const float s = forward_inv_s > 0.f ? forward_inv_s : expf(ln_inv_s[0] * factor);
   const float* ss = sdf + st;
@@ -569,7 +583,127 @@
     }
     cnt += __popcll(m);
   }
+  return cnt;
+}
+
+template <bool EMIT>
+__global__ void __launch_bounds__(SMP_BLOCK) k_compress(const float* __restrict__ sdf, const float* __restrict__ t,
+                                                         const int64_t* __restrict__ pi, int64_t R,
+                                                         const float* __restrict__ ln_inv_s, float factor,
+                                                         float forward_inv_s, float thre, int64_t* __restrict__ counts,
+                                                         const int64_t* __restrict__ pi_out, float* __restrict__ t_out,
+                                                         int64_t* __restrict__ ridx_out, int64_t tail_n) {
+  const int64_t r = smp_wave_id();
+  if (r >= R) return;
+  const int lane = nsim_lane();
+  if (EMIT && tail_n > 0) {
+    const int64_t S = pi_out[2 * (R - 1)] + pi_out[2 * (R - 1) + 1];
+    for (int64_t i = r * 64 + lane; i < tail_n; i += R * 64) {
+      t_out[S + i] = 0.f;
+      ridx_out[S + i] = R + i;
+    }
+  }
+  const int cnt = compress_ray<EMIT>(sdf, t, pi, r, ln_inv_s, factor, forward_inv_s, thre, pi_out, t_out, ridx_out);
   if (!EMIT && lane == 0) counts[r] = cnt;
+}
+
+__global__ void __launch_bounds__(PI_THREADS) k_compress_count_pack(const float* __restrict__ sdf, const int64_t* __restrict__ pi,
+                                                                      int64_t R, const float* __restrict__ ln_inv_s, float factor,
+                                                                      float forward_inv_s, float thre, int64_t* counts,
+                                                                      unsigned* ticket, int64_t* __restrict__ pi_out,
+                                                                      int64_t* __restrict__ total, int64_t cap, int64_t* notify,
+                                                                      int64_t seq) {
+  const int64_t r = (int64_t)blockIdx.x * (PI_THREADS / 64) + (threadIdx.x >> 6);
+  if (r < R) {
+    const int cnt = compress_ray<false>(sdf, nullptr, pi, r, ln_inv_s, factor, forward_inv_s, thre, nullptr, nullptr, nullptr);
+    if (nsim_lane() == 0) counts[r] = cnt;
+  }
+  if (!nsim_last_workgroup(ticket)) return;
+  pack_infos_scan(counts, R, pi_out, total, cap, notify, seq);
+}
+
+#define MT_MAX_C ((SMP_LDS_FLOATS - 1) / 2)
+__global__ void __launch_bounds__(SMP_BLOCK) k_march_tail(
+    const float* __restrict__ rays_o, const float* __restrict__ rays_d, const float* __restrict__ near,
+    const float* __restrict__ far, const float* __restrict__ jitter, int64_t R, const uint32_t* __restrict__ bits,
+    const int64_t* __restrict__ ray_word_off, OccDev occ, float step, int max_steps, const int64_t* __restrict__ pia,
+    const float* __restrict__ jc, int C, const int64_t* __restrict__ live_rank, float* __restrict__ t_out,
+    int64_t* __restrict__ pio, int64_t* __restrict__ ridx_out, float* __restrict__ x_out) {
+  __shared__ float smp_lds[SMP_WAVES_PER_BLOCK][SMP_LDS_FLOATS];
+  const int64_t r = smp_wave_id();
+  if (r >= R) return;
+  const int lane = nsim_lane();
+  int64_t q;
+  const bool live = smp_live(live_rank, r, q);
+  const int64_t sa = pia[2 * r], na = live ? pia[2 * r + 1] : 0;
+  const int64_t so = sa + q * (int64_t)C;
+  if (lane == 0) {
+    pio[2 * r] = so;
+    pio[2 * r + 1] = na + (live ? C : 0);
+  }
+  if (!live) return;
+  float* lb = &smp_lds[threadIdx.x >> 6][0];
+  int* hist = reinterpret_cast<int*>(lb + C);
+  const float nr = near[r], fr = far[r];
+  for (int j = lane; j < C; j += 64) {
+    const float u = jc ? jc[r * C + j] : 0.5f;
+    lb[j] = nr + (fr - nr) * (((float)j + u) / (float)C);
+  }
+  for (int j = lane; j <= C; j += 64) hist[j] = 0;
+  nsim_wave_fence();
+  float ro[3] = {0.f, 0.f, 0.f}, rd[3] = {0.f, 0.f, 0.f};
+  if (x_out) {
+#pragma unroll
+    for (int c = 0; c < 3; ++c) {
+      ro[c] = rays_o[3 * r + c];
+      rd[c] = rays_d[3 * r + c];
+    }
+  }
+  if (na > 0) {
+    if (ray_word_off) bits += ray_word_off[r];
+    const MarchRay m = march_load(rays_o, rays_d, near, far, jitter, r, step, max_steps);
+    int cnt = 0;
+    for (int base = 0; base < m.K; base += 64) {
+      float v;
+      const bool hit = march_test(m, occ, bits, base + lane, step, v);
+      const unsigned long long mask = wave_ballot(hit);
+      if (hit) {
+        const int i = cnt + __popcll(mask & ((1ull << lane) - 1ull));
+        int lo = 0, hi = C;
+        while (lo < hi) {
+          const int mid = (lo + hi) >> 1;
+          if (lb[mid] < v) lo = mid + 1; else hi = mid;
+        }
+        atomicAdd(&hist[lo], 1);
+        const int64_t pos = so + i + lo;
+        t_out[pos] = v;
+        if (ridx_out) ridx_out[pos] = r;
+        if (x_out) {
+#pragma unroll
+          for (int c = 0; c < 3; ++c) x_out[pos * 3 + c] = ro[c] + v * rd[c];
+        }
+      }
+      cnt += __popcll(mask);
+    }
+    nsim_wave_fence();
+  }
+  int carry = 0;
+  for (int base = 0; base < C; base += 64) {
+    const int j = base + lane;
+    const int h = j < C ? hist[j] : 0;
+    const int incl = wave_incl_sum(h);
+    if (j < C) {
+      const float v = lb[j];
+      const int64_t pos = so + j + carry + incl;
+      t_out[pos] = v;
+      if (ridx_out) ridx_out[pos] = r;
+      if (x_out) {
+#pragma unroll
+        for (int c = 0; c < 3; ++c) x_out[pos * 3 + c] = ro[c] + v * rd[c];
+      }
+    }
+    carry += wave_shfl(incl, 63);
+  }
 }
 
 extern "C" {
@@ -771,4 +905,49 @@
   return 0;
 }
 
-}
+int nsim_march_count_rank(const float* rays_o, const float* rays_d, const float* near, const float* far, const float* jitter,
+                          int64_t R, const uint32_t* bits, const int64_t* ray_word_off, const NsimOccMeta* meta, float step,
+                          int max_steps, int64_t* counts, uint32_t* ticket, int C, int nf0, int nf1, int nf2, int nf3,
+                          int64_t* live_rank, int64_t* live_idx, int64_t* cnts, int64_t* notify, int64_t seq, int64_t* pack_infos,
+                          int64_t* total, int64_t cap, int64_t* notify_total, int64_t seq_total, void* stream) {
+  if (R <= 0) return 2;
+  if (!meta || !(step > 0.f)) return 5;
+  if (!counts || !ticket || !live_rank || !cnts || C < 0) return 4;
+  LiveArgs la;
+  la.C = C;
+  la.nf[0] = nf0, la.nf[1] = nf1, la.nf[2] = nf2, la.nf[3] = nf3;
+  hipLaunchKernelGGL(k_march_count_rank, dim3(nsim_blocks(R, PI_THREADS / 64)), dim3(PI_THREADS), 0, (hipStream_t)stream, rays_o,
+                     rays_d, near, far, jitter, R, bits, ray_word_off, occ_dev(meta), step, max_steps, counts, (unsigned*)ticket, la,
+                     live_rank, live_idx, cnts, notify, seq, pack_infos, total, cap, notify_total, seq_total);
+  NSIM_CHECK_LAUNCH();
+  return 0;
+}
+
+int nsim_compress_count_pack(const float* sdf, const int64_t* pack_infos, int64_t R, const float* ln_inv_s, float ln_inv_s_factor,
+                             float forward_inv_s, float thre, int64_t* counts, uint32_t* ticket, int64_t* pack_infos_out,
+                             int64_t* total, int64_t cap, int64_t* notify, int64_t seq, void* stream) {
+  if (R <= 0) return 2;
+  if (!counts || !ticket || !pack_infos_out) return 4;
+  hipLaunchKernelGGL(k_compress_count_pack, dim3(nsim_blocks(R, PI_THREADS / 64)), dim3(PI_THREADS), 0, (hipStream_t)stream, sdf,
+                     pack_infos, R, ln_inv_s, ln_inv_s_factor, forward_inv_s, thre, counts, (unsigned*)ticket, pack_infos_out, total,
+                     cap, notify, seq);
+  NSIM_CHECK_LAUNCH();
+  return 0;
+}
+
+int nsim_march_tail(const float* rays_o, const float* rays_d, const float* near, const float* far, const float* jitter, int64_t R,
+                    const uint32_t* bits, const int64_t* ray_word_off, const NsimOccMeta* meta, float step, int max_steps,
+                    const int64_t* pack_infos_m, const float* jitter_c, int C, const int64_t* live_rank, float* t_out,
+                    int64_t* pack_infos_out, int64_t* ridx_out, float* x_out, void* stream) {
+  if (R <= 0) return 0;
+  if (!meta || !(step > 0.f)) return 5;
+  if (C <= 0 || C > MT_MAX_C || !pack_infos_m || !t_out || !pack_infos_out) return 4;
+  if (x_out && !(rays_o && rays_d)) return 24;
+  hipLaunchKernelGGL(k_march_tail, smp_grid(R), dim3(SMP_BLOCK), 0, (hipStream_t)stream, rays_o, rays_d, near, far, jitter, R, bits,
+                     ray_word_off, occ_dev(meta), step, max_steps, pack_infos_m, jitter_c, C, live_rank, t_out, pack_infos_out,
+                     ridx_out, x_out);
+  NSIM_CHECK_LAUNCH();
+  return 0;
+}
+
+}
diff --git a/neuralsim_amd/fields/neus.py b/neuralsim_amd/fields/neus.py
--- a/neuralsim_amd/fields/neus.py
+++ b/neuralsim_amd/fields/neus.py
@@ -71,6 +71,8 @@
 _EVAL_PLANES = os.environ.get("NSIM_EVAL_PLANES", "0") == "1"
 _SDF_FUSED_BELOW = int(os.environ.get("NSIM_SDF_FUSED_BELOW", "0"))
 _FUSE_MERGE_UPSAMPLE = os.environ.get("NSIM_FUSE_MERGE_UPSAMPLE", "1") == "1"
+_FUSE_MARCH_TAIL = os.environ.get("NSIM_FUSE_MARCH_TAIL", "1") == "1"
+_FUSE_COUNT_SCAN = os.environ.get("NSIM_FUSE_COUNT_SCAN", "0") == "1"
 
 
 class _FieldFn(torch.autograd.Function):
@@ -1038,12 +1040,15 @@
         C = int(qp.get("num_coarse", 64))
         bits, occm = self.accel.occ_bits, self.accel.meta
         counts = torch.empty([R], dtype=torch.long, device=dev)
-        _lib.call("nsim_march_count", _lib.ptr(o), _lib.ptr(d), _lib.ptr(near), _lib.ptr(far), _lib.ptr(jitter), R,
-                  _lib.ptr(bits), _lib.ptr(woff), occm, step, max_steps, _lib.ptr(counts))
+        march_args = (_lib.ptr(o), _lib.ptr(d), _lib.ptr(near), _lib.ptr(far), _lib.ptr(jitter), R, _lib.ptr(bits), _lib.ptr(woff),
+                      occm, step, max_steps)
+        mo = marched_only(qp)
+        fuse_scan = _FUSE_COUNT_SCAN and mo
+        if not fuse_scan:
+            _lib.call("nsim_march_count", *march_args, _lib.ptr(counts))
         nt = self._host_notify() if cap is not None else None
         self._notify_seq_m = None
         fine = fine_list(qp)
-        mo = marched_only(qp)
         lr = live_idx = cnts = None
         self._live = None
         adr_m = None
@@ -1057,9 +1062,12 @@
             pi_m = torch.empty([R, 2], dtype=torch.long, device=dev)
             total_m = torch.empty([1], dtype=torch.long, device=dev)
             adr_l, seq_l = nt.arm(2) if nt is not None else (None, 0)
-            _lib.call("nsim_live_rank", _lib.ptr(counts), R, C, *((list(fine) + [0, 0, 0, 0])[:4]), _lib.ptr(lr), _lib.ptr(live_idx),
-                      _lib.ptr(cnts), adr_l, seq_l, _lib.ptr(pi_m), _lib.ptr(total_m), -1 if cap is None else int(cap), adr_m,
-                      self._notify_seq_m or 0)
+            rank_args = (C, *((list(fine) + [0, 0, 0, 0])[:4]), _lib.ptr(lr), _lib.ptr(live_idx), _lib.ptr(cnts), adr_l, seq_l,
+                         _lib.ptr(pi_m), _lib.ptr(total_m), -1 if cap is None else int(cap), adr_m, self._notify_seq_m or 0)
+            if fuse_scan:
+                _lib.call("nsim_march_count_rank", *march_args, _lib.ptr(counts), _lib.ptr(_lib.ticket(dev, 0)), *rank_args)
+            else:
+                _lib.call("nsim_live_rank", _lib.ptr(counts), R, *rank_args)
             self._live = dict(rank=lr, idx=live_idx, cnts=cnts, seq=seq_l if nt is not None else None, n=None)
         elif nt is not None:
             pi_m, total_m = po.get_pack_infos_from_n(counts, return_total=True, cap=int(cap), notify=(adr_m, self._notify_seq_m))
@@ -1088,11 +1096,6 @@
             if n_dev is None:
                 return None
             return cnts[1 + k:2 + k] if mo else (n_dev if k == 0 else None)
-        t_m = torch.empty([max(M, 1)], **f32)
-        _lib.call("nsim_march_emit", _lib.ptr(o), _lib.ptr(d), _lib.ptr(near), _lib.ptr(far), _lib.ptr(jitter), R,
-                  _lib.ptr(bits), _lib.ptr(woff), occm, step, max_steps, _lib.ptr(pi_m), _lib.ptr(t_m))
-        t_c = torch.empty([max(Rl, 1), C], **f32)
-        _lib.call("nsim_coarse_depths", _lib.ptr(near), _lib.ptr(far), _lib.ptr(jitter_c), R, C, _lib.ptr(t_c), _lib.ptr(lr))
         S = M + Rl * C
         t = torch.empty([S], **f32)
         pi = torch.empty([R, 2], dtype=torch.long, device=dev)
@@ -1101,8 +1104,16 @@
         ridx_mid = (not with_x) or per_ray
         ridx = torch.empty([S], dtype=torch.long, device=dev) if (ridx_mid or (need_ridx and not fine)) else None
         xq = torch.empty([S, 3], **f32) if with_x else None
-        _lib.call("nsim_merge_sorted", _lib.ptr(t_m), None, _lib.ptr(pi_m), _lib.ptr(t_c), None, R, C, _lib.ptr(t), None,
-                  _lib.ptr(pi), _lib.ptr(ridx), _lib.ptr(o), _lib.ptr(d), _lib.ptr(xq), _lib.ptr(lr))
+        if _FUSE_MARCH_TAIL and 0 < C <= 255:
+            _lib.call("nsim_march_tail", *march_args, _lib.ptr(pi_m), _lib.ptr(jitter_c), C, _lib.ptr(lr), _lib.ptr(t), _lib.ptr(pi),
+                      _lib.ptr(ridx), _lib.ptr(xq))
+        else:
+            t_m = torch.empty([max(M, 1)], **f32)
+            _lib.call("nsim_march_emit", *march_args, _lib.ptr(pi_m), _lib.ptr(t_m))
+            t_c = torch.empty([max(Rl, 1), C], **f32)
+            _lib.call("nsim_coarse_depths", _lib.ptr(near), _lib.ptr(far), _lib.ptr(jitter_c), R, C, _lib.ptr(t_c), _lib.ptr(lr))
+            _lib.call("nsim_merge_sorted", _lib.ptr(t_m), None, _lib.ptr(pi_m), _lib.ptr(t_c), None, R, C, _lib.ptr(t), None,
+                      _lib.ptr(pi), _lib.ptr(ridx), _lib.ptr(o), _lib.ptr(d), _lib.ptr(xq), _lib.ptr(lr))
         grid16, wpack = self._shadow()
         fm_s = None
         if with_x:
@@ -1175,18 +1186,26 @@
         dev = t.device
         counts = torch.empty([R], dtype=torch.long, device=dev)
         ln_eff = self._ln_inv_s_eff().detach()
-        _lib.call("nsim_compress_count", _lib.ptr(sdf), _lib.ptr(pi), R, _lib.ptr(ln_eff),
-                  self.ln_inv_s_factor, forward_inv_s, thre, _lib.ptr(counts))
+        count_args = (_lib.ptr(sdf), _lib.ptr(pi), R, _lib.ptr(ln_eff), self.ln_inv_s_factor, forward_inv_s, thre, _lib.ptr(counts))
         nt = self._host_notify()
         self._spec_ok = False
         cap_k = self._keep_cap(R) if (spec_launch is not None and nt is not None) else None
         seq_k = None
+        adr = None
         if nt is not None:
             adr, seq_k = nt.arm(1)
-            pi_k, total = po.get_pack_infos_from_n(counts, return_total=True, notify=(adr, seq_k),
-                                                   cap=-1 if cap_k is None else cap_k)
+        if _FUSE_COUNT_SCAN and R > 0:
+            pi_k = torch.empty([R, 2], dtype=torch.long, device=dev)
+            total = torch.empty([1], dtype=torch.long, device=dev)
+            _lib.call("nsim_compress_count_pack", *count_args, _lib.ptr(_lib.ticket(dev, 1)), _lib.ptr(pi_k), _lib.ptr(total),
+                      -1 if cap_k is None else cap_k, adr, seq_k or 0)
         else:
-            pi_k, total = po.get_pack_infos_from_n(counts, return_total=True)
+            _lib.call("nsim_compress_count", *count_args)
+            if nt is not None:
+                pi_k, total = po.get_pack_infos_from_n(counts, return_total=True, notify=(adr, seq_k),
+                                                       cap=-1 if cap_k is None else cap_k)
+            else:
+                pi_k, total = po.get_pack_infos_from_n(counts, return_total=True)
 
         def emit(n_out, tail_):
             t_o = torch.empty([n_out + tail_], dtype=torch.float32, device=dev)
```

New measurement: 7.192 million, median of 5. No clear change (+0.1%).
